# chymaera96/NeuralSampleID

Measured on AMD Instinct MI355X. Metric: audio clips/sec (contrastive step, grafp encoder), higher is better.
Workload: dtype bf16; 1 GPU; B=256 bf16 k=3 hipGraph 2-stream: grafp.yaml GraphEncoder('t') full contrastive step (fwd x2 views + NT-Xent + bwd + clip + Adam), synthetic (64,128) log-mel clip pairs per GPU, random-init weights; global_batch=256, k=3, parallelism=dp1, collectives=none (single process), gemm_arithmetic=bf16 MFMA operands, fp32 accumulate, activation_storage=bf16, views=two HIP streams (parallel graph branches), hipgraph=True

## Files before the change

include/nsid.h:

```cpp
#ifndef NSID_H
#define NSID_H
#include <stddef.h>
#include <stdint.h>

#ifdef __cplusplus
extern "C" {
#endif

#define NSID_OK 0
#define NSID_EINVAL (-1)
#define NSID_ELAUNCH (-2)

#define NSID_ACT_NONE 0
#define NSID_ACT_RELU 1
#define NSID_ACT_LEAKY 2
#define NSID_ACT_ELU 3

#define NSID_ROW_TILE 128

#define NSID_F32 0
#define NSID_BF16 1

#define NSID_GEMM_FP32 0
#define NSID_GEMM_BF16 1

int nsid_version(void);
int nsid_debug_gemm_trace(void* device_buf);
int nsid_debug_knn_trace(void* device_buf);
int nsid_set_gemm_precision(int mode);
int nsid_get_gemm_precision(void);
int nsid_set_tuning(const char* key, long value);
int nsid_get_tuning(const char* key, long* value);
int nsid_reset_tuning(void);
int nsid_tuning_count(void);
const char* nsid_tuning_key(int i);
long nsid_debug_counter(const char* key);
int nsid_debug_counters_reset(void);
int nsid_debug_counter_count(void);
const char* nsid_debug_counter_key(int i);
long nsid_gemm_g256_launches(void);
int nsid_row_tiles(int M);
long nsid_workspace_bytes(const char* op, long rows, long cols);

int nsid_linear_fwd(const void* x, int ldx, const void* w, int w_dtype, const float* bias, void* out, int ldo, int M,
                    int Nout, int K, int groups, const float* in_scale, const float* in_shift, int act_in, int act_out,
                    float* stat, int ksplit, int act_dtype , void* stream);
int nsid_linear_fwd_res(const void* x, int ldx, const void* w, int w_dtype, const float* bias, const void* addend, int ldadd,
                        void* out, int ldo, int M, int Nout, int K, int groups, const float* in_scale,
                        const float* in_shift, int act_in, int act_dtype, void* stream);
int nsid_ffn_fused_fwd(const void* x, const void* w1, const float* b1, const void* w2, const float* b2, void* out, int M, int C,
                       int H, void* stream);
int nsid_mrconv_fused_fwd(const void* y, const int32_t* idx, int B, int N, int C, int k, const void* w, const float* bias, void* out,
                          void* stream);
int nsid_linear_bwd_data(const void* dout, int ldd, const void* w, int w_dtype, const void* addend, int ldadd,
                         void* din, int ldi, int M, int Nout, int K, int groups,
                         int act_dtype , void* stream);
int nsid_linear_bwd_data_bn(const void* dout, int ldd, const void* w, int w_dtype, const void* addend, int ldadd,
                            void* din, int ldi, int M, int Nout, int K, int groups, int act_dtype, const void* bn_r,
                            const float* bn_scale, const float* bn_shift, const float* bn_mean, const float* bn_invstd,
                            int bn_act, float* bn_partial, void* stream);
int nsid_linear_bwd_data_bnapply(const void* dy, const void* r, const float* coef4, int act, void* dr, const void* w, int w_dtype,
                                 const void* addend, int ldadd, void* din, int ldi, int M, int Nout, int K, int groups,
                                 int act_dtype, const void* bn_r, const float* bn_scale, const float* bn_shift,
                                 const float* bn_mean, const float* bn_invstd, int bn_act, float* bn_partial, void* stream);
int nsid_linear_bwd_weight(const void* dout, int ldd, const void* x, int ldx, float* dw, int M, int Nout, int K,
                           int groups, const float* in_scale, const float* in_shift, int act_in,
                           int act_dtype , void* stream);
typedef struct nsid_wgrad_problem {
  const void* dout[2];
  const void* x[2];
  const float* in_scale[2];
  const float* in_shift[2];
  float* dw;
  int ldd, ldx, M, Nout, K, groups, act_in;
  int ds_out_nodes;
} nsid_wgrad_problem;
int nsid_linear_bwd_weight_grouped(const nsid_wgrad_problem* problems, int n, int act_dtype,
                                   int max_workgroups ,
                                   void* stream);
int nsid_colsum_acc(const void* x, int ldx, int M, int C, float* out, int dtype, void* stream);

int nsid_bn_finalize(const float* stat, int tiles, int C, int M, const float* gamma, const float* beta,
                     float* running_mean, float* running_var, int64_t* num_batches_tracked, float momentum,
                     float eps, float* scale, float* shift, float* mean, float* invstd, void* stream);
int nsid_bn_finalize_deferred(const float* stat, int tiles, int C, int M, const float* gamma, const float* beta, float eps,
                              float* scale, float* shift, float* mean, float* invstd, float* uvar, void* stream);
int nsid_bn_running_update(int n, const int* C, float* const* running_mean, float* const* running_var,
                           int64_t* const* num_batches_tracked, const float* const* mean_a, const float* const* uvar_a,
                           const float* const* mean_b, const float* const* uvar_b, float momentum, void* stream);
int nsid_bn_eval_affine(const float* gamma, const float* beta, const float* running_mean, const float* running_var,
                        float eps, int C, float* scale, float* shift, void* stream);
int nsid_bn_apply(const void* r, const float* scale, const float* shift, int act, const void* residual,
                  void* out, int M, int C, int dtype, void* stream);
int nsid_bn_bwd_reduce(const void* dout, const void* r, int M, int C, const float* scale, const float* shift,
                       const float* mean, const float* invstd, int act, float* partial, int dtype, void* stream);
int nsid_bn_bwd_finalize(const float* partial, int tiles, int C, int M, float* dgamma, float* dbeta, float* coef,
                         void* stream);
int nsid_bn_bwd_finalize_fused(const float* partial, int tiles, int C, int M, float* dgamma, float* dbeta, float* coef,
                               const float* scale, const float* shift, const float* mean, const float* invstd, float* coef4,
                               void* stream);
int nsid_bn_bwd_apply(const void* dout, const void* r, int M, int C, const float* scale, const float* shift,
                      const float* mean, const float* invstd, int act, const float* coef, void* dr, int dtype,
                      void* stream);

int nsid_knn_graph(const void* r, int ldr, const float* scale, const float* shift, int B, int N, int C, int k,
                   int dilation, int32_t* idx, int dtype, void* stream);

int nsid_mr_aggregate_fwd(const void* r, int ldr, const float* scale, const float* shift, const int32_t* idx, int B,
                          int N, int C, int k, void* u, uint8_t* argmax, int dtype, void* stream);
int nsid_mr_aggregate_bwd(const void* du, const int32_t* idx, const uint8_t* argmax, int B, int N, int C, int k,
                          void* dy, int dtype, void* stream);
int nsid_mr_aggregate_bwd_bn(const void* du, const int32_t* idx, const uint8_t* argmax, int B, int N, int C, int k, void* dy,
                             const void* bn_r, int bn_ldr, const float* bn_scale, const float* bn_shift, const float* bn_mean,
                             const float* bn_invstd, int bn_act, float* partial, int dtype, void* stream);

int nsid_batched_index_select_fwd(const float* x, const int32_t* idx, int B, int C, int N, int Nq, int k, float* out,
                                  void* stream);
int nsid_batched_index_select_bwd(const float* dout, const int32_t* idx, int B, int C, int N, int Nq, int k,
                                  float* dx , void* stream);

int nsid_downsample3_fwd(const void* x, int B, int N, int C, const void* wp, int w_dtype, const float* bias, void* out,
                         int Cout, float* stat, int act_dtype, void* stream);
int nsid_downsample3_bwd_weight(const void* dout, const void* x, float* dwp , int B, int N, int C, int Cout,
                                int act_dtype, void* stream);
int nsid_downsample3_bwd_data(const void* dout, const void* wp, const void* w_odd, int w_dtype, void* dx, int B, int N,
                              int C, int Cout, int act_dtype, void* stream);
int nsid_pack_ds_weight_bwd(const float* w, int Cout, int Cin, float* w_odd, void* stream);
int nsid_im2col3_fwd(const void* x, int B, int N, int C, void* col, int dtype, void* stream);
int nsid_im2col3_bwd(const void* dcol, int B, int N, int C, void* dx, int dtype, void* stream);
int nsid_pack_ds_weight(const float* w, int Cout, int Cin, float* wp, void* stream);
int nsid_dsact_fwd(const void* x, int B, int N, int C, const float* in_scale, const float* in_shift, int act_in, const float* w,
                   const float* bias, void* out, int Cout, float* stat, const float* out_scale, const float* out_shift, int act_out,
                   int act_dtype, void* stream);
int nsid_dsact_bwd_weight(const void* dout, const void* x, const float* in_scale, const float* in_shift, int act_in,
                          float* dw , int B, int N, int C, int Cout, int act_dtype, void* stream);
int nsid_dsact_bwd_data(const void* dout, const float* w, void* dx, int B, int N, int C, int Cout, const void* r_prev,
                        const float* scale, const float* shift, const float* mean, const float* invstd, int act, float* partial,
                        int act_dtype, void* stream);
int nsid_dsact_part_rows(int B, int N);
int nsid_ds_prepack(int n, const float* const* w, void* const* wp16, void* const* wb16, float* const* dwp, const int* Cout,
                    const int* Cin, void* stream);
int nsid_unpack_ds_wgrad(const float* dwp, int Cout, int Cin, float* dw , void* stream);

int nsid_peak_patchify_fwd(const float* spec, const float* w, const float* bias, int B, int H, int W, int pb, int pf,
                           int F, void* out, int ldo, float* minmax, int out_dtype, void* stream);
int nsid_peak_patchify_bwd(const float* spec, const float* minmax, const void* out, const void* dout, int ldo,
                           int B, int H, int W, int pb, int pf, int F, float* dw , float* dbias ,
                           int out_dtype, void* stream);
int nsid_peak_patchify_bwd_ws(const float* spec, const float* minmax, const void* out, const void* dout, int ldo, int B, int H,
                              int W, int pb, int pf, int F, float* dw, float* dbias, float* ws, int out_dtype, void* stream);

int nsid_node_mean_fwd(const void* x, int B, int N, int C, float* out, int x_dtype, void* stream);
int nsid_node_mean_bwd(const float* dout, int B, int N, int C, void* dx, int dx_dtype, void* stream);
int nsid_elu_bwd(const float* dout, const float* out, long n, float* din, void* stream);
int nsid_l2norm_fwd(const float* p, int B, int d, float eps, float* z, float* norm, void* stream);
int nsid_l2norm_bwd(const float* dz, const float* z, const float* norm, int B, int d, float eps, float* dp,
                    void* stream);

int nsid_reflect_pad(const float* x, long L, int pad, float* out, void* stream);
int nsid_power_mel_db(const float* spec, long ld, int n_freq, const float* fb, const int* band, int n_mels, int T,
                      float* out, void* stream);
int nsid_unfold_segments(const float* logmel, int n_mels, int T, int n_frames, int step, int S, float* out, void* stream);
int nsid_logmel_fft(const float* wave, long in_stride, int B, long L, int n_fft, int hop, const float* window,
                    const float* twiddle, const float* fb, const int* band, int n_mels, float* out, long out_clip_stride,
                    long out_mel_stride, void* stream);

int nsid_f32_to_bf16(const float* src, void* dst, long n, void* stream);

size_t nsid_ntxent_ws_floats(int Bg);
int nsid_ntxent_fwd_bwd(const float* z_i, const float* z_j, int Bg, int d, float tau, int p0, int np, float* ws,
                        float* loss_out, float* dz_i, float* dz_j, void* stream);

int nsid_sumsq_blocks(long n);
int nsid_sumsq_partial(const float* g, long n, float* partial, void* stream);
int nsid_adam_step(float* p, const float* g, float* m, float* v, long n, const float* hyper, int64_t* step,
                   const float* partial, int nblocks, float* gnorm_out, void* stream);

int nsid_fill_zero(void* p, size_t bytes, void* stream);
int nsid_scale_f32(const float* x, const float* scale, long n, float* out, void* stream);

int nsid_bcn_to_rows(const float* x, int B, int C, int N, void* rows, int ld, int rows_dtype, void* stream);
int nsid_rows_to_bcn(const void* rows, int ld, int B, int C, int N, float* x, int rows_dtype, void* stream);

int nsid_row_sqnorm(const float* x, int ldx, int n, int d, float* out, void* stream);
int nsid_flat_l2_topk(const float* q, int ldq, int nq, const float* x, int ldx, int nx, const float* x_sqnorm, const float* q_sqnorm,
                      int d, int k, float* D, int64_t* I, void* ws, size_t ws_bytes, void* stream);
int nsid_seq_scores(const float* q, int ldq, const float* x, int ldx, int nx, int d, const int64_t* I, int k, const int* starts,
                    const int* lens, int npairs, float* out, int ldo, void* stream);

int nsid_clf_node_rows(const float* x, int S, int C, int N, const float* pos, float* rows, void* stream);
int nsid_clf_pair_scores(const float* q, int nq_seg, const float* kp, int nc_seg, int N, const int* groups, const int64_t* out_off,
                         const int* tile_off, int ngroups, int ntiles, const int* cidx, const float* tail, float* out,
                         int64_t out_len, void* stream);
int nsid_clf_pair_scores_c(const float* q, int nq_seg, const float* kp, int nc_seg, int C, int N, const int* groups,
                           const int64_t* out_off, const int* tile_off, int ngroups, int ntiles, const int* cidx, const float* tail,
                           float* out, int64_t out_len, void* stream);
int nsid_clf_node_rows_n(const float* x, int S, int C, int N, const float* pos, float* rows, void* stream);
int nsid_clf_pair_scores_n(const float* q, int nq_seg, const float* kp, int nc_seg, int C, int N, const int* groups,
                           const int64_t* out_off, const int* tile_off, int ngroups, int ntiles, const int* cidx, const float* tail,
                           float* out, int64_t out_len, void* stream);

int nsid_clf_mine_hard_negatives(const float* zq, int nq, const float* za, int na, int d, int k, int64_t* out, void* stream);
int nsid_clf_attn_fwd(const float* q, int nq_seg, const float* kv, int nc_seg, int N, const int* qi, const int* ci, int P, float* obar,
                      float* attn, float* abar, void* stream);
int nsid_clf_head_fwd(const float* hid, const float* keep, const float* w2, const float* b2, int P, float* s, void* stream);
int nsid_clf_head_bwd(const float* ds, const float* s, const float* hid, const float* keep, const float* w2, int P, float* dh, float* dz,
                      float* dw2, float* db2, void* stream);
int nsid_clf_attn_bwd(const float* dobar, const float* attn, const float* q, int nq_seg, const float* kv, int nc_seg, int N,
                      const int* qi, const int* ci, int P, float* dq, float* dk, void* stream);
int nsid_clf_seg_reduce(const float* dq, const float* dk, const float* abar, const float* dobar, const int* qi, const int* ci, int P,
                        int N, int nq_seg, int nc_seg, float* dq_seg, float* dkv_seg, void* stream);
int nsid_clf_attn_fwd_c(const float* q, int nq_seg, const float* kv, int nc_seg, int C, int N, const int* qi, const int* ci, int P,
                        float* obar, float* attn, float* abar, void* stream);
int nsid_clf_attn_bwd_c(const float* dobar, const float* attn, const float* q, int nq_seg, const float* kv, int nc_seg, int C, int N,
                        const int* qi, const int* ci, int P, float* dq, float* dk, void* stream);
int nsid_clf_seg_reduce_c(const float* dq, const float* dk, const float* abar, const float* dobar, const int* qi, const int* ci, int P,
                          int C, int N, int nq_seg, int nc_seg, float* dq_seg, float* dkv_seg, void* stream);

int nsid_conv2d_fwd(const void* x, int B, int H, int W, int C, const void* w, int w_dtype, const float* bias, const void* addend,
                    void* out, int Cout, int ksize, int stride, int act_out, int act_dtype, void* stream);
int nsid_ibn_relu_fwd(const void* x, int B, int HW, int C, const float* in_gamma, const float* in_beta, float eps,
                      const float* bn_scale, const float* bn_shift, void* out, int dtype, void* stream);
int nsid_stem7_pool_fwd(const float* x, int B, int H, int W, const float* w, const float* bias, void* out, int out_dtype,
                        void* stream);
int nsid_gem_pool_fwd(const void* x, int B, int HW, int C, const float* p, float eps, float* out, int x_dtype, void* stream);

#ifdef __cplusplus
}
#endif
#endif
```

neuralsampleid_amd/_lib.py:

```python
import ctypes
import os

import torch

_PKG = os.path.dirname(os.path.abspath(__file__))
LIB_PATH = os.environ.get("NSID_LIB") or os.path.join(_PKG, "libnsid_hip.so")

SIGNATURES = {
    "nsid_set_gemm_precision": "i",
    "nsid_linear_fwd": "pipippiiiiippiipiis",
    "nsid_linear_fwd_res": "pipippipiiiiippiis",
    "nsid_linear_bwd_data": "pipipipiiiiiis",
    "nsid_linear_bwd_data_bn": "pipipipiiiiiipppppips",
    "nsid_linear_bwd_weight": "pipipiiiippiis",
    "nsid_linear_bwd_weight_grouped": "piiis",
    "nsid_colsum_acc": "piiipis",
    "nsid_bn_finalize": "piiipppppffpppps",
    "nsid_bn_finalize_deferred": "piiippfppppps",
    "nsid_bn_running_update": "ippppppppfs",
    "nsid_bn_eval_affine": "ppppfipps",
    "nsid_bn_apply": "pppippiiis",
    "nsid_bn_bwd_reduce": "ppiippppipis",
    "nsid_bn_bwd_finalize": "piiippps",
    "nsid_bn_bwd_apply": "ppiippppippis",
    "nsid_bn_bwd_finalize_fused": "piiipppppppps",
    "nsid_knn_graph": "pippiiiiipis",
    "nsid_mr_aggregate_fwd": "pipppiiiippis",
    "nsid_mr_aggregate_bwd": "pppiiiipis",
    "nsid_im2col3_fwd": "piiipis",
    "nsid_im2col3_bwd": "piiipis",
    "nsid_pack_ds_weight": "piips",
    "nsid_dsact_fwd": "piiippipppipppiis",
    "nsid_dsact_bwd_weight": "ppppipiiiiis",
    "nsid_dsact_bwd_data": "pppiiiipppppipis",
    "nsid_pack_ds_weight_bwd": "piips",
    "nsid_downsample3_fwd": "piiipippipis",
    "nsid_downsample3_bwd_weight": "pppiiiiis",
    "nsid_downsample3_bwd_data": "pppipiiiiis",
    "nsid_unpack_ds_wgrad": "piips",
    "nsid_ds_prepack": "ipppppps",
    "nsid_peak_patchify_fwd": "pppiiiiiipipis",
    "nsid_peak_patchify_bwd": "ppppiiiiiiippis",
    "nsid_peak_patchify_bwd_ws": "ppppiiiiiiipppis",
    "nsid_node_mean_fwd": "piiipis",
    "nsid_node_mean_bwd": "piiipis",
    "nsid_elu_bwd": "pplps",
    "nsid_l2norm_fwd": "piifpps",
    "nsid_l2norm_bwd": "pppiifps",
    "nsid_ntxent_fwd_bwd": "ppiifiipppps",
    "nsid_sumsq_partial": "plps",
    "nsid_adam_step": "pppplpppips",
    "nsid_f32_to_bf16": "ppls",
    "nsid_reflect_pad": "plips",
    "nsid_power_mel_db": "plippiips",
    "nsid_unfold_segments": "piiiiips",
    "nsid_logmel_fft": "pliliippppiplls",
    "nsid_bcn_to_rows": "piiipiis",
    "nsid_rows_to_bcn": "piiiipis",
    "nsid_batched_index_select_fwd": "ppiiiiips",
    "nsid_batched_index_select_bwd": "ppiiiiips",
    "nsid_fill_zero": "pzs",
    "nsid_scale_f32": "pplps",
    "nsid_row_sqnorm": "piiips",
    "nsid_flat_l2_topk": "piipiippiipppzs",
    "nsid_seq_scores": "pipiiipippipis",
    "nsid_clf_node_rows": "piiipps",
    "nsid_clf_pair_scores": "pipiipppiipppls",
    "nsid_clf_pair_scores_c": "pipiiipppiipppls",
    "nsid_clf_node_rows_n": "piiipps",
    "nsid_clf_pair_scores_n": "pipiiipppiipppls",
    "nsid_clf_mine_hard_negatives": "pipiiips",
    "nsid_clf_attn_fwd": "pipiippippps",
    "nsid_clf_head_fwd": "ppppips",
    "nsid_clf_head_bwd": "pppppipppps",
    "nsid_clf_attn_bwd": "pppipiippipps",
    "nsid_clf_seg_reduce": "ppppppiiiipps",
    "nsid_clf_attn_fwd_c": "pipiiippippps",
    "nsid_clf_attn_bwd_c": "pppipiiippipps",
    "nsid_clf_seg_reduce_c": "ppppppiiiiipps",
    "nsid_conv2d_fwd": "piiiipipppiiiiis",
    "nsid_ibn_relu_fwd": "piiippfpppis",
    "nsid_stem7_pool_fwd": "piiipppis",
    "nsid_gem_pool_fwd": "piiipfpis",
}

class WgradProblem(ctypes.Structure):
    _fields_ = [("dout", ctypes.c_void_p * 2), ("x", ctypes.c_void_p * 2), ("in_scale", ctypes.c_void_p * 2),
                ("in_shift", ctypes.c_void_p * 2), ("dw", ctypes.c_void_p), ("ldd", ctypes.c_int), ("ldx", ctypes.c_int),
                ("M", ctypes.c_int), ("Nout", ctypes.c_int), ("K", ctypes.c_int), ("groups", ctypes.c_int), ("act_in", ctypes.c_int),
                ("ds_out_nodes", ctypes.c_int)]


_CT = {"p": ctypes.c_void_p, "i": ctypes.c_int, "l": ctypes.c_long, "f": ctypes.c_float, "s": ctypes.c_void_p,
       "z": ctypes.c_size_t}


def _load():
    if not os.path.exists(LIB_PATH):
        raise ImportError(
            f"{LIB_PATH} is missing: build it with `python -m neuralsampleid_amd.build` "
            "(hipcc --offload-arch=gfx950). There is no CPU fallback for the product path.")
    lib = ctypes.CDLL(LIB_PATH)
    for name, sig in SIGNATURES.items():
        fn = getattr(lib, name)
        fn.argtypes = [_CT[c] for c in sig]
        fn.restype = ctypes.c_int
    lib.nsid_version.restype = ctypes.c_int
    if lib.nsid_version() < 0:
        raise ImportError(f"{LIB_PATH} reports a negative version: not a product build of this tree; rebuild with "
                          "`python -m neuralsampleid_amd.build --force`")
    lib.nsid_debug_gemm_trace.argtypes = [ctypes.c_void_p]
    lib.nsid_debug_gemm_trace.restype = ctypes.c_int
    lib.nsid_debug_knn_trace.argtypes = [ctypes.c_void_p]
    lib.nsid_debug_knn_trace.restype = ctypes.c_int
    lib.nsid_get_gemm_precision.restype = ctypes.c_int
    lib.nsid_gemm_g256_launches.argtypes = []
    lib.nsid_gemm_g256_launches.restype = ctypes.c_long
    lib.nsid_set_tuning.argtypes = [ctypes.c_char_p, ctypes.c_long]
    lib.nsid_set_tuning.restype = ctypes.c_int
    lib.nsid_get_tuning.argtypes = [ctypes.c_char_p, ctypes.POINTER(ctypes.c_long)]
    lib.nsid_get_tuning.restype = ctypes.c_int
    lib.nsid_reset_tuning.argtypes = []
    lib.nsid_reset_tuning.restype = ctypes.c_int
    lib.nsid_workspace_bytes.argtypes = [ctypes.c_char_p, ctypes.c_long, ctypes.c_long]
    lib.nsid_workspace_bytes.restype = ctypes.c_long
    lib.nsid_tuning_count.argtypes = []
    lib.nsid_tuning_count.restype = ctypes.c_int
    lib.nsid_tuning_key.argtypes = [ctypes.c_int]
    lib.nsid_tuning_key.restype = ctypes.c_char_p
    lib.nsid_debug_counter.argtypes = [ctypes.c_char_p]
    lib.nsid_debug_counter.restype = ctypes.c_long
    lib.nsid_debug_counters_reset.argtypes = []
    lib.nsid_debug_counters_reset.restype = ctypes.c_int
    lib.nsid_debug_counter_count.argtypes = []
    lib.nsid_debug_counter_count.restype = ctypes.c_int
    lib.nsid_debug_counter_key.argtypes = [ctypes.c_int]
    lib.nsid_debug_counter_key.restype = ctypes.c_char_p
    lib.nsid_linear_bwd_data_bnapply.argtypes = [_CT[c] for c in "pppippipipiiiiiipppppips"]
    lib.nsid_linear_bwd_data_bnapply.restype = ctypes.c_int
    lib.nsid_mr_aggregate_bwd_bn.argtypes = [_CT[c] for c in "pppiiiippippppipis"]
    lib.nsid_mr_aggregate_bwd_bn.restype = ctypes.c_int
    lib.nsid_ffn_fused_fwd.argtypes = [_CT[c] for c in "ppppppiiis"]
    lib.nsid_ffn_fused_fwd.restype = ctypes.c_int
    lib.nsid_mrconv_fused_fwd.argtypes = [_CT[c] for c in "ppiiiippps"]
    lib.nsid_mrconv_fused_fwd.restype = ctypes.c_int
    lib.nsid_row_tiles.argtypes = [ctypes.c_int]
    lib.nsid_row_tiles.restype = ctypes.c_int
    lib.nsid_dsact_part_rows.argtypes = [ctypes.c_int, ctypes.c_int]
    lib.nsid_dsact_part_rows.restype = ctypes.c_int
    lib.nsid_sumsq_blocks.argtypes = [ctypes.c_long]
    lib.nsid_sumsq_blocks.restype = ctypes.c_int
    lib.nsid_ntxent_ws_floats.argtypes = [ctypes.c_int]
    lib.nsid_ntxent_ws_floats.restype = ctypes.c_size_t
    return lib


lib = _load()
EXPORTS = list(SIGNATURES) + ["nsid_version", "nsid_debug_gemm_trace", "nsid_debug_knn_trace", "nsid_get_gemm_precision", "nsid_gemm_g256_launches", "nsid_linear_bwd_data_bnapply", "nsid_mr_aggregate_bwd_bn", "nsid_ffn_fused_fwd", "nsid_mrconv_fused_fwd", "nsid_debug_counter", "nsid_debug_counters_reset", "nsid_debug_counter_count", "nsid_debug_counter_key", "nsid_set_tuning", "nsid_get_tuning", "nsid_reset_tuning", "nsid_tuning_count", "nsid_tuning_key", "nsid_row_tiles", "nsid_dsact_part_rows", "nsid_sumsq_blocks", "nsid_ntxent_ws_floats", "nsid_workspace_bytes"]

_ERR = {-1: "NSID_EINVAL (unsupported shape, misaligned pointer or bad argument)",
        -2: "NSID_ELAUNCH (HIP runtime refused the launch)"}


def call(name, *args):
    rc = getattr(lib, name)(*args)
    if rc != 0:
        raise RuntimeError(f"{name} failed: {_ERR.get(rc, rc)}")


def set_tuning(key: str, value: int) -> None:
    if lib.nsid_set_tuning(key.encode(), int(value)) != 0:
        raise KeyError(f"unknown tuning key {key!r}; known: {', '.join(tuning_keys())}")


def get_tuning(key: str) -> int:
    v = ctypes.c_long()
    if lib.nsid_get_tuning(key.encode(), ctypes.byref(v)) != 0:
        raise KeyError(f"unknown tuning key {key!r}")
    return int(v.value)


def reset_tuning() -> None:
    lib.nsid_reset_tuning()


def launch_counters(reset: bool = False) -> dict:
    out = {}
    for i in range(lib.nsid_debug_counter_count()):
        k = lib.nsid_debug_counter_key(i)
        out[k.decode()] = int(lib.nsid_debug_counter(k))
    if reset:
        lib.nsid_debug_counters_reset()
    return out


def tuning_keys():
    return [lib.nsid_tuning_key(i).decode() for i in range(lib.nsid_tuning_count())]
```

neuralsampleid_amd/csrc/bn.hip:

```cpp
#include <cstdlib>
#include "nsid_common.h"

namespace {

constexpr int FIN_THREADS = 1024;

template <int FIN_CH>
__device__ __forceinline__ void tile_sums(const float* __restrict__ p0, const float* __restrict__ p1, int tiles,
                                          int C, int c, int tg, bool ok, double* red0, double* red1, double& sum,
                                          double& sq) {
  constexpr int FIN_TG = FIN_THREADS / FIN_CH;
  double a = 0.0, b = 0.0;
  if (ok) {
    constexpr int UB = 8;
    int t = tg;
    for (; t + (UB - 1) * FIN_TG < tiles; t += UB * FIN_TG) {
      float va[UB], vb[UB];
#pragma unroll
      for (int u = 0; u < UB; ++u) {
        va[u] = p0[(long)(t + u * FIN_TG) * C + c];
        vb[u] = p1[(long)(t + u * FIN_TG) * C + c];
      }
#pragma unroll
      for (int u = 0; u < UB; ++u) { a += (double)va[u]; b += (double)vb[u]; }
// ... 172 lines not shown
  if (coef != nullptr) {
    coef[c] = c0;
    coef[C + c] = c1;
  }
  if (coef4 != nullptr) {
    const float sc = scale[c], is = invstd[c];
    coef4[c] = sc;
    coef4[C + c] = shift[c];
    coef4[2 * C + c] = -sc * c1 * is;
    coef4[3 * C + c] = sc * (c1 * is * mean[c] - c0);
  }
}

template <typename T, int U>
__global__ __launch_bounds__(256) void bn_bwd_apply_kernel(const T* __restrict__ dout, const T* __restrict__ r,
                                                           long rows, int CV, const float* __restrict__ scale,
                                                           const float* __restrict__ shift,
                                                           const float* __restrict__ mean,
                                                           const float* __restrict__ invstd, float slope,
                                                           const float* __restrict__ coef, T* __restrict__ dr) {
  constexpr int N = Chunk<T>::N;
  const int C = CV * N;
  const long t = (long)blockIdx.x * blockDim.x + threadIdx.x, total = (long)gridDim.x * blockDim.x;
  const int cq = (int)(t % CV), c = cq * N;
  const long rstep = total / CV;
  float sc[N], sh[N], mu[N], is[N], c0[N], c1[N];
  load_channels<N>(scale, c, sc);
  load_channels<N>(shift, c, sh);
  load_channels<N>(mean, c, mu);
  load_channels<N>(invstd, c, is);
  load_channels<N>(coef, c, c0);
  load_channels<N>(coef + C, c, c1);
  for (long row = t / CV; row < rows; row += U * rstep) {
    float d[U][N], x[U][N];
#pragma unroll
    for (int u = 0; u < U; ++u) {
      const long rr = row + u * rstep;
      if (rr < rows) {
        Chunk<T>::load(dout + (rr * CV + cq) * N, d[u]);
        Chunk<T>::load(r + (rr * CV + cq) * N, x[u]);
      }
    }
#pragma unroll
    for (int u = 0; u < U; ++u) {
      const long rr = row + u * rstep;
      if (rr < rows) {
        float o[N];
#pragma unroll
        for (int e = 0; e < N; ++e) {
          const float g = (sc[e] * x[u][e] + sh[e]) > 0.f ? d[u][e] : d[u][e] * slope;
          const float xh = (x[u][e] - mu[e]) * is[e];
          o[e] = sc[e] * (g - c0[e] - xh * c1[e]);
        }
        Chunk<T>::store(dr + (rr * CV + cq) * N, o);
      }
    }
  }
}

inline float bn_slope(int act) { return act == NSID_ACT_RELU ? 0.f : (act == NSID_ACT_LEAKY ? 0.2f : 1.f); }

inline int stream_grid(long nchunks) {
  long b = (nchunks + 255) / 256;
  const long cap = nsid_tune(NSID_T_stream_max_wg);
  return (int)(b > cap ? cap : (b < 1 ? 1 : b));
}

template <typename T>
__global__ __launch_bounds__(256) void colsum_atomic_kernel(const T* __restrict__ x, long ld, int M, int C,
                                                            float* __restrict__ out) {
  constexpr int N = Chunk<T>::N;
  constexpr int CQ = CR_CH / N, RG = 256 / CQ, ROWS = NSID_ROW_TILE / RG;
  __shared__ float red[RG][CR_CH];
  const int row0 = blockIdx.x * NSID_ROW_TILE;
  const int t = threadIdx.x, q = t % CQ, rgp = t / CQ;
  const int c = blockIdx.y * CR_CH + N * q;
  float s[N];
#pragma unroll
  for (int e = 0; e < N; ++e) s[e] = 0.f;
  if (c < C)
    for (int i = 0; i < ROWS; ++i) {
      const int row = row0 + rgp + RG * i;
      if (row < M) {
        float d[N];
        Chunk<T>::load(x + (long)row * ld + c, d);
#pragma unroll
        for (int e = 0; e < N; ++e) s[e] += d[e];
      }
    }
#pragma unroll
  for (int e = 0; e < N; ++e) red[rgp][N * q + e] = s[e];
  __syncthreads();
  if (t < CR_CH && blockIdx.y * CR_CH + t < C) {
    float a = 0.f;
    for (int g = 0; g < RG; ++g) a += red[g][t];
    atomicAdd(out + blockIdx.y * CR_CH + t, a);
  }
}

inline long chunk_keeping_grid(long nchunks, int CV, int U, long max_wg, bool* capped) {
  int g0 = CV, d256 = 256;
  while (d256 % 2 == 0 && g0 % 2 == 0) { d256 /= 2; g0 /= 2; }
  long want = (nchunks + 256L * U - 1) / (256L * U);
  if (capped) *capped = want > max_wg;
  if (want > max_wg) want = max_wg;
  if (want < 1) want = 1;
  return (want + g0 - 1) / g0 * g0;
}

inline int bn_fin_ch(int tiles) {
  const int t = (int)nsid_tune(NSID_T_bn_fin_tiles);
  return (t > 0 && tiles >= t) ? 16 : 64;
}
#define NSID_FIN_LAUNCH(kernel, tiles, C, stream, ...)                                                                      \
  do {                                                                                                                       \
    if (bn_fin_ch(tiles) == 16)                                                                                              \
      NSID_LAUNCH(kernel<16>, dim3(((C) + 15) / 16), dim3(FIN_THREADS), 0, static_cast<hipStream_t>(stream), __VA_ARGS__);   \
    else                                                                                                                     \
      NSID_LAUNCH(kernel<64>, dim3(((C) + 63) / 64), dim3(FIN_THREADS), 0, static_cast<hipStream_t>(stream), __VA_ARGS__);   \
  } while (0)

}

extern "C" int nsid_bn_finalize(const float* stat, int tiles, int C, int M, const float* gamma, const float* beta,
                                float* running_mean, float* running_var, int64_t* nbt, float momentum, float eps,
                                float* scale, float* shift, float* mean, float* invstd, void* stream) {
  NSID_REQUIRE(stat && gamma && beta && scale && shift && mean && invstd && C > 0 && M > 0);
  NSID_REQUIRE(tiles == nsid_row_tiles(M));
  NSID_REQUIRE((running_mean == nullptr) == (running_var == nullptr));
  NSID_FIN_LAUNCH(bn_finalize_kernel, tiles, C, stream, stat, tiles, C, M, gamma, beta, running_mean, running_var, nbt,
              momentum, eps, scale, shift, mean, invstd, static_cast<float*>(nullptr));
  return nsid_launch_status();
}

extern "C" int nsid_bn_finalize_deferred(const float* stat, int tiles, int C, int M, const float* gamma,
                                         const float* beta, float eps, float* scale, float* shift, float* mean,
                                         float* invstd, float* uvar, void* stream) {
  NSID_REQUIRE(stat && gamma && beta && scale && shift && mean && invstd && uvar && C > 0 && M > 0);
  NSID_REQUIRE(tiles == nsid_row_tiles(M));
  NSID_FIN_LAUNCH(bn_finalize_kernel, tiles, C, stream, stat, tiles, C, M, gamma, beta, static_cast<float*>(nullptr),
              static_cast<float*>(nullptr), static_cast<int64_t*>(nullptr), 0.f, eps, scale, shift, mean, invstd, uvar);
  return nsid_launch_status();
}

namespace {
constexpr int RU_LAYERS = 16;
struct RunUpdArgs {
  float* rm[RU_LAYERS]; float* rv[RU_LAYERS]; int64_t* nbt[RU_LAYERS];
  const float* mean_a[RU_LAYERS]; const float* uvar_a[RU_LAYERS];
  const float* mean_b[RU_LAYERS]; const float* uvar_b[RU_LAYERS];
  int C[RU_LAYERS];
  float momentum;
};
__global__ __launch_bounds__(256) void bn_running_update_kernel(const RunUpdArgs a) {
  const int l = blockIdx.x;
  const float m = a.momentum;
  const bool two = a.mean_b[l] != nullptr;
  if (threadIdx.x == 0 && a.nbt[l] != nullptr) *a.nbt[l] += two ? 2 : 1;
  for (int c = threadIdx.x; c < a.C[l]; c += blockDim.x) {
    float rm = running_blend(a.rm[l][c], a.mean_a[l][c], m);
    float rv = running_blend(a.rv[l][c], a.uvar_a[l][c], m);
    if (two) {
      rm = running_blend(rm, a.mean_b[l][c], m);
      rv = running_blend(rv, a.uvar_b[l][c], m);
    }
    a.rm[l][c] = rm;
    a.rv[l][c] = rv;
  }
}
}

extern "C" int nsid_bn_running_update(int n, const int* C, float* const* running_mean, float* const* running_var,
                                      int64_t* const* num_batches_tracked, const float* const* mean_a,
                                      const float* const* uvar_a, const float* const* mean_b,
                                      const float* const* uvar_b, float momentum, void* stream) {
  NSID_REQUIRE(n > 0 && C && running_mean && running_var && mean_a && uvar_a);
  for (int base = 0; base < n; base += RU_LAYERS) {
    RunUpdArgs a{};
    const int cnt = n - base < RU_LAYERS ? n - base : RU_LAYERS;
    for (int i = 0; i < cnt; ++i) {
      NSID_REQUIRE(C[base + i] > 0 && running_mean[base + i] && running_var[base + i] && mean_a[base + i] && uvar_a[base + i]);
      a.rm[i] = running_mean[base + i]; a.rv[i] = running_var[base + i];
      a.nbt[i] = num_batches_tracked ? num_batches_tracked[base + i] : nullptr;
      a.mean_a[i] = mean_a[base + i]; a.uvar_a[i] = uvar_a[base + i];
      a.mean_b[i] = mean_b ? mean_b[base + i] : nullptr; a.uvar_b[i] = uvar_b ? uvar_b[base + i] : nullptr;
      NSID_REQUIRE((a.mean_b[i] == nullptr) == (a.uvar_b[i] == nullptr));
      a.C[i] = C[base + i];
    }
    a.momentum = momentum;
    NSID_LAUNCH(bn_running_update_kernel, dim3(cnt), dim3(256), 0, static_cast<hipStream_t>(stream), a);
    const int rc = nsid_launch_status();
    if (rc != NSID_OK) return rc;
  }
  return NSID_OK;
}

extern "C" int nsid_bn_eval_affine(const float* gamma, const float* beta, const float* running_mean,
                                   const float* running_var, float eps, int C, float* scale, float* shift,
                                   void* stream) {
  NSID_REQUIRE(gamma && beta && running_mean && running_var && scale && shift && C > 0);
  NSID_LAUNCH(bn_eval_affine_kernel, dim3((C + 127) / 128), dim3(128), 0, static_cast<hipStream_t>(stream), gamma, beta,
              running_mean, running_var, eps, C, scale, shift);
  return nsid_launch_status();
}

extern "C" int nsid_bn_apply(const void* r, const float* scale, const float* shift, int act, const void* residual,
                             void* out, int M, int C, int dtype, void* stream) {
  NSID_REQUIRE(r && scale && shift && out && M > 0 && C > 0 && NSID_DTYPE_OK(dtype));
  NSID_REQUIRE(C % (dtype == NSID_BF16 ? 8 : 4) == 0 && nsid_aligned16(r) && nsid_aligned16(out));
  NSID_DISPATCH_DTYPE(dtype, T, {
    const long nchunks = (long)M * C / Chunk<T>::N;
    NSID_LAUNCH((bn_apply_kernel<T>), dim3(stream_grid(nchunks)), dim3(256), 0, static_cast<hipStream_t>(stream),
                static_cast<const T*>(r), scale, shift, act, static_cast<const T*>(residual), static_cast<T*>(out),
                nchunks, C / Chunk<T>::N);
  });
  return nsid_launch_status();
}

extern "C" int nsid_bn_bwd_reduce(const void* dout, const void* r, int M, int C, const float* scale,
                                  const float* shift, const float* mean, const float* invstd, int act, float* partial,
                                  int dtype, void* stream) {
  NSID_REQUIRE(dout && r && scale && shift && mean && invstd && partial && M > 0 && C > 0 && NSID_DTYPE_OK(dtype));
  NSID_REQUIRE(C % (dtype == NSID_BF16 ? 8 : 4) == 0);
  NSID_REQUIRE(act == NSID_ACT_NONE || act == NSID_ACT_RELU || act == NSID_ACT_LEAKY);
  const int tiles = nsid_row_tiles(M);
  NSID_DISPATCH_DTYPE(dtype, T, {
    NSID_LAUNCH((col_reduce_kernel<1, T>), dim3(tiles, (C + CR_CH - 1) / CR_CH), dim3(256), 0,
                static_cast<hipStream_t>(stream), static_cast<const T*>(dout), static_cast<const T*>(r), (long)C, M, C,
                scale, shift, mean, invstd, bn_slope(act), partial, tiles);
  });
  return nsid_launch_status();
}

extern "C" int nsid_bn_bwd_finalize(const float* partial, int tiles, int C, int M, float* dgamma, float* dbeta,
                                    float* coef, void* stream) {
  NSID_REQUIRE(partial && coef && C > 0 && M > 0 && tiles >= 1);
  NSID_FIN_LAUNCH(bn_bwd_finalize_kernel, tiles, C, stream, partial, tiles, C, M, dgamma, dbeta, coef, static_cast<const float*>(nullptr),
              static_cast<const float*>(nullptr), static_cast<const float*>(nullptr), static_cast<const float*>(nullptr),
              static_cast<float*>(nullptr));
  return nsid_launch_status();
}

extern "C" int nsid_bn_bwd_finalize_fused(const float* partial, int tiles, int C, int M, float* dgamma, float* dbeta,
                                          float* coef, const float* scale, const float* shift, const float* mean,
                                          const float* invstd, float* coef4, void* stream) {
  NSID_REQUIRE(partial && coef && coef4 && scale && shift && mean && invstd && C > 0 && M > 0 && tiles >= 1);
  NSID_FIN_LAUNCH(bn_bwd_finalize_kernel, tiles, C, stream, partial, tiles, C, M, dgamma, dbeta, coef, scale, shift, mean, invstd, coef4);
  return nsid_launch_status();
}

extern "C" int nsid_bn_bwd_apply(const void* dout, const void* r, int M, int C, const float* scale,
                                 const float* shift, const float* mean, const float* invstd, int act,
                                 const float* coef, void* dr, int dtype, void* stream) {
  NSID_REQUIRE(dout && r && scale && shift && mean && invstd && coef && dr && M > 0 && C > 0 && NSID_DTYPE_OK(dtype));
  NSID_REQUIRE(C % (dtype == NSID_BF16 ? 8 : 4) == 0);
  NSID_REQUIRE(act == NSID_ACT_NONE || act == NSID_ACT_RELU || act == NSID_ACT_LEAKY);
  NSID_DISPATCH_DTYPE(dtype, T, {
    constexpr int U = 4;
    const int CV = C / Chunk<T>::N;
    const long nchunks = (long)M * CV;
    int g0 = CV, d256 = 256;
    while (d256 % 2 == 0 && g0 % 2 == 0) { d256 /= 2; g0 /= 2; }
    long want = (nchunks + 256L * U - 1) / (256L * U);
    const long max_wg = nsid_tune(NSID_T_bn_bwd_apply_max_wg);
    nsid_count(NSID_C_bn_bwd_apply);
    if (want > max_wg) { want = max_wg; nsid_count(NSID_C_bn_bwd_apply_capped); }
    const long grid = (want + g0 - 1) / g0 * g0;
    NSID_LAUNCH((bn_bwd_apply_kernel<T, U>), dim3((int)grid), dim3(256), 0, static_cast<hipStream_t>(stream),
                static_cast<const T*>(dout), static_cast<const T*>(r), (long)M, CV, scale, shift, mean,
                invstd, bn_slope(act), coef, static_cast<T*>(dr));
  });
  return nsid_launch_status();
}

extern "C" int nsid_colsum_acc(const void* x, int ldx, int M, int C, float* out, int dtype, void* stream) {
  NSID_REQUIRE(x && out && M > 0 && C > 0 && NSID_DTYPE_OK(dtype) && nsid_aligned16(x));
  NSID_REQUIRE(C % (dtype == NSID_BF16 ? 8 : 4) == 0 && ldx % (dtype == NSID_BF16 ? 8 : 4) == 0);
  NSID_DISPATCH_DTYPE(dtype, T, {
    NSID_LAUNCH((colsum_atomic_kernel<T>), dim3(nsid_row_tiles(M), (C + CR_CH - 1) / CR_CH), dim3(256), 0,
                static_cast<hipStream_t>(stream), static_cast<const T*>(x), (long)ldx, M, C, out);
  });
  return nsid_launch_status();
}
```

neuralsampleid_amd/csrc/misc.hip:

```cpp
#include <algorithm>
#include "nsid_common.h"

namespace {

inline int grid_for(long n, int cap = 2048) {
  long b = (n + 255) / 256;
  return (int)(b > cap ? cap : (b < 1 ? 1 : b));
}

template <typename T>
__global__ __launch_bounds__(256) void im2col3_fwd_kernel(const T* __restrict__ x, int B, int N, int No, int C,
                                                          T* __restrict__ col) {
  constexpr int NV = Chunk<T>::N;
  const int CV = C / NV;
  const long total = (long)B * No * 3 * CV;
  for (long q = (long)blockIdx.x * blockDim.x + threadIdx.x; q < total; q += (long)gridDim.x * blockDim.x) {
    const int cv = (int)(q % CV);
    const int t = (int)((q / CV) % 3);
    const long orow = q / (3L * CV);
    const int b = (int)(orow / No), no = (int)(orow % No);
    const int n = 2 * no - 1 + t;
    float v[NV];
#pragma unroll
    for (int e = 0; e < NV; ++e) v[e] = 0.f;
    if (n >= 0 && n < N) Chunk<T>::load(x + ((long)b * N + n) * C + NV * cv, v);
    Chunk<T>::store(col + orow * (3L * C) + (long)t * C + NV * cv, v);
  }
}

template <typename T>
__global__ __launch_bounds__(256) void im2col3_bwd_kernel(const T* __restrict__ dcol, int B, int N, int No, int C,
                                                          T* __restrict__ dx) {
  constexpr int NV = Chunk<T>::N;
  const int CV = C / NV;
  const long total = (long)B * N * CV;
  for (long q = (long)blockIdx.x * blockDim.x + threadIdx.x; q < total; q += (long)gridDim.x * blockDim.x) {
    const int cv = (int)(q % CV);
    const long row = q / CV;
    const int b = (int)(row / N), n = (int)(row % N);
    float s[NV];
#pragma unroll
    for (int e = 0; e < NV; ++e) s[e] = 0.f;
#pragma unroll
    for (int t = 0; t < 3; ++t) {
      const int m = n + 1 - t;
      if (m >= 0 && (m & 1) == 0 && (m >> 1) < No) {
        float v[NV];
        Chunk<T>::load(dcol + ((long)b * No + (m >> 1)) * (3L * C) + (long)t * C + NV * cv, v);
#pragma unroll
        for (int e = 0; e < NV; ++e) s[e] += v[e];
      }
    }
    Chunk<T>::store(dx + row * C + NV * cv, s);
  }
}

__global__ void pack_ds_weight_kernel(const float* __restrict__ w, int Cout, int Cin, float* __restrict__ wp) {
  const long total = (long)Cout * 3 * Cin;
  for (long q = (long)blockIdx.x * blockDim.x + threadIdx.x; q < total; q += (long)gridDim.x * blockDim.x) {
    const int c = (int)(q % Cin), t = (int)((q / Cin) % 3);
    const long o = q / (3L * Cin);
    wp[q] = w[((o * Cin + c) * 3 + t) * 3 + 1];
  }
}
__global__ void pack_ds_weight_bwd_kernel(const float* __restrict__ w, int Cout, int Cin, float* __restrict__ wb) {
  const long total = 2L * Cout * Cin;
  for (long q = (long)blockIdx.x * blockDim.x + threadIdx.x; q < total; q += (long)gridDim.x * blockDim.x) {
    const int c = (int)(q % Cin);
    const long r = q / Cin;
    const long o = r % Cout;
    const int t = r < Cout ? 2 : 0;
    wb[q] = w[((o * Cin + c) * 3 + t) * 3 + 1];
  }
}
__global__ void unpack_ds_wgrad_kernel(const float* __restrict__ dwp, int Cout, int Cin, float* __restrict__ dw) {
  const long total = (long)Cout * 3 * Cin;
  for (long q = (long)blockIdx.x * blockDim.x + threadIdx.x; q < total; q += (long)gridDim.x * blockDim.x) {
    const int c = (int)(q % Cin), t = (int)((q / Cin) % 3);
    const long o = q / (3L * Cin);
    atomicAdd(dw + ((o * Cin + c) * 3 + t) * 3 + 1, dwp[q]);
  }
}

constexpr int DSP_LAYERS = 8;
#define NSID_DS_SLOTS 2
struct DsPrepArgs {
  const float* w[DSP_LAYERS]; __bf16* wp16[DSP_LAYERS]; __bf16* wb16[DSP_LAYERS]; float* dwp[DSP_LAYERS];
  int Cout[DSP_LAYERS], Cin[DSP_LAYERS];
};
__global__ __launch_bounds__(256) void ds_prepack_kernel(const DsPrepArgs a) {
  const int l = blockIdx.y;
  const float* w = a.w[l];
  const int Cout = a.Cout[l], Cin = a.Cin[l];
  const long total = (long)Cout * 3 * Cin;
  for (long q = (long)blockIdx.x * blockDim.x + threadIdx.x; q < total; q += (long)gridDim.x * blockDim.x) {
    const int c = (int)(q % Cin), t = (int)((q / Cin) % 3);
    const long o = q / (3L * Cin);
    a.wp16[l][q] = (__bf16)w[((o * Cin + c) * 3 + t) * 3 + 1];
    if (a.dwp[l] != nullptr) {
#pragma unroll
      for (int v = 0; v < NSID_DS_SLOTS; ++v) a.dwp[l][v * total + q] = 0.f;
    }
    if (q < 2L * Cout * Cin) {
      const long r = q / Cin, ob = r % Cout;
      const int tb = r < Cout ? 2 : 0;
      a.wb16[l][q] = (__bf16)w[((ob * Cin + c) * 3 + tb) * 3 + 1];
    }
  }
}

__device__ __forceinline__ float add_unfused(float acc, float a, float b) {
#pragma clang fp contract(off)
  const float p = a * b;
  return acc + p;
}
__device__ __forceinline__ float linspace01(int i, int steps) {
  const float step = 1.0f / (float)(steps - 1);
  return (i < steps / 2) ? __fmul_rn((float)i, step) : fmaf(-(float)(steps - 1 - i), step, 1.0f);
}

constexpr int PATCH_PAD = 8;
template <typename T, int MAXPATCH, int PB = 0, int PF = 0>
__global__ __launch_bounds__(256) void patchify_fwd_kernel(const float* __restrict__ spec, const float* __restrict__ w,
                                                           const float* __restrict__ bias, int H, int W, int pb_,
                                                           int pf_, int F, T* __restrict__ out, int ldo,
                                                           float* __restrict__ minmax) {
  constexpr bool FIX = PB > 0;
  const int pb = FIX ? PB : pb_, pf = FIX ? PF : pf_;
  extern __shared__ __attribute__((aligned(16))) float sm[];
  const int b = blockIdx.x, t = threadIdx.x;
  const float* x = spec + (long)b * H * W;
  const int wn = F * 3 * pb * pf, LDW = W + PATCH_PAD;
  float* wl = sm;
  float* red = sm + wn;
  float* xs = red + 8;
  for (int i = t; i < wn; i += blockDim.x) wl[i] = w[i];
  float lo = __builtin_inff(), hi = -__builtin_inff();
  constexpr int XB = 8;
  for (int i0 = t; i0 < H * W / 4; i0 += XB * blockDim.x) {
    f32x4 v[XB];
#pragma unroll
    for (int u = 0; u < XB; ++u) {
      const int i = i0 + u * blockDim.x;
      if (i < H * W / 4) v[u] = *reinterpret_cast<const f32x4*>(x + 4 * i);
    }
#pragma unroll
    for (int u = 0; u < XB; ++u) {
      const int i = i0 + u * blockDim.x;
      if (i < H * W / 4) {
        const int hh = (4 * i) / W, ww = (4 * i) % W;
        *reinterpret_cast<f32x4*>(xs + hh * LDW + ww) = v[u];
        lo = fminf(fminf(lo, v[u][0]), fminf(v[u][1], fminf(v[u][2], v[u][3])));
        hi = fmaxf(fmaxf(hi, v[u][0]), fmaxf(v[u][1], fmaxf(v[u][2], v[u][3])));
      }
    }
  }
  lo = wave_min(lo); hi = wave_max(hi);
  if ((t & 63) == 0) { red[t >> 6] = lo; red[4 + (t >> 6)] = hi; }
  __syncthreads();
  lo = fminf(fminf(red[0], red[1]), fminf(red[2], red[3]));
  hi = fmaxf(fmaxf(red[4], red[5]), fmaxf(red[6], red[7]));
  if (t == 0 && minmax != nullptr) { minmax[2 * b] = lo; minmax[2 * b + 1] = hi; }
  const float range = hi - lo;
  const int Hp = H / pb, Wp = W / pf, NP = Hp * Wp;
  for (int p = t; p < NP; p += blockDim.x) {
    const int ph = p / Wp, pw = p % Wp;
    T* dst = out + ((long)b * NP + p) * ldo;
    constexpr int NLW = FIX ? PF : MAXPATCH, NLH = FIX ? PB : MAXPATCH;
    float sv[MAXPATCH], lw[NLW], lh[NLH];
#pragma unroll
    for (int q = 0; q < MAXPATCH; ++q) {
      if (q < pb * pf) {
        const int i = q / pf, j = q % pf;
        sv[q] = (xs[(ph * pb + i) * LDW + pw * pf + j] - lo) / range;
        if constexpr (!FIX) {
          lw[q] = linspace01(pw * pf + j, W);
          lh[q] = linspace01(ph * pb + i, H);
        }
      }
    }
    if constexpr (FIX) {
#pragma unroll
      for (int j = 0; j < PF; ++j) lw[j] = linspace01(pw * PF + j, W);
#pragma unroll
      for (int i = 0; i < PB; ++i) lh[i] = linspace01(ph * PB + i, H);
    }
    constexpr int NV = Chunk<T>::N;
    for (int f0 = 0; f0 < F; f0 += NV) {
      float res[NV];
#pragma unroll
      for (int ff = 0; ff < NV; ++ff) {
        const int f = f0 + ff;
        res[ff] = 0.f;
        if (f < F) {
          float acc = bias[f];
          const float* wf = (MAXPATCH == 32 ? w : wl) + f * 3 * pb * pf;
#pragma unroll
          for (int q = 0; q < MAXPATCH; ++q) {
            if (q < pb * pf) {
              acc = fmaf(wf[q], lw[FIX ? q % (FIX ? PF : 1) : q], acc);
              acc = add_unfused(acc, wf[pb * pf + q], lh[FIX ? q / (FIX ? PF : 1) : q]);
              acc = add_unfused(acc, wf[2 * pb * pf + q], sv[q]);
            }
          }
          res[ff] = acc < 0.f ? 0.f : acc;
        }
      }
      if (f0 + NV <= F && ldo % NV == 0 && (reinterpret_cast<size_t>(out) & 15) == 0) {
        Chunk<T>::store(dst + f0, res);
      } else {
#pragma unroll
        for (int ff = 0; ff < NV; ++ff)
          if (f0 + ff < F) dst[f0 + ff] = (T)res[ff];
      }
    }
  }
}

template <typename T>
__global__ __launch_bounds__(256) void patchify_bwd_kernel(const float* __restrict__ spec,
                                                           const float* __restrict__ minmax,
                                                           const T* __restrict__ out,
                                                           const T* __restrict__ dout, int ldo, int B, int H,
                                                           int W, int pb, int pf, int F, float* __restrict__ dw,
                                                           float* __restrict__ dbias, int bands) {
  extern __shared__ __attribute__((aligned(16))) float sm[];
  const int t = threadIdx.x;
  const int Hall = H;
  H /= bands;
  const int Hp = H / pb, Wp = W / pf, NP = Hp * Wp;
  const int per_f = 3 * pb * pf, LDW = W + PATCH_PAD;
  float* xs = sm + NP * F;
  float* red = xs + H * LDW;
  constexpr int MAXQ = 4;
  float wacc[MAXQ] = {0.f, 0.f, 0.f, 0.f}, bacc = 0.f;
  constexpr int NV = Chunk<T>::N;
  const bool vec = (F % NV == 0) && (ldo % NV == 0);
  for (int vb = blockIdx.x; vb < B * bands; vb += gridDim.x) {
    const int b = vb / bands, band = vb - b * bands;
    const float* x = spec + ((long)b * bands + band) * H * W;
    const float lo = minmax[2 * b], range = minmax[2 * b + 1] - lo;
    __syncthreads();
    if (vec) {
      const int FC = F / NV;
      for (int q = t; q < NP * FC; q += blockDim.x) {
        const int p = q / FC, f = (q % FC) * NV;
        const long o = ((long)vb * NP + p) * ldo + f;
        float ov[NV], dv[NV];
        Chunk<T>::load(out + o, ov);
        Chunk<T>::load(dout + o, dv);
#pragma unroll
        for (int e = 0; e < NV; ++e) sm[p * F + f + e] = ov[e] > 0.f ? dv[e] : 0.f;
      }
    } else {
      for (int q = t; q < NP * F; q += blockDim.x) {
        const int p = q / F, f = q % F;
        const long o = ((long)vb * NP + p) * ldo + f;
        sm[q] = (float)out[o] > 0.f ? (float)dout[o] : 0.f;
      }
    }
    constexpr int XB = 8;
    for (int i0 = t; i0 < H * W / 4; i0 += XB * blockDim.x) {
// ... 88 lines not shown
      Chunk<T>::load(dout + o, dv); Chunk<T>::load(dout + o + 4, dv + 4);
    }
    f32x4 v[8];
#pragma unroll
    for (int u = 0; u < 8; ++u) v[u] = *reinterpret_cast<const f32x4*>(x + 4 * (t + 256 * u));
#pragma unroll
    for (int e = 0; e < 8; ++e) g[t * F + e] = ov[e] > 0.f ? dv[e] : 0.f;
#pragma unroll
    for (int u = 0; u < 8; ++u) {
      const int i4 = 4 * (t + 256 * u), hh = i4 / W, ww = i4 % W;
      *reinterpret_cast<f32x4*>(xs + hh * LDW + ww) =
          f32x4{(v[u][0] - lo) / range, (v[u][1] - lo) / range, (v[u][2] - lo) / range, (v[u][3] - lo) / range};
    }
  }
  __syncthreads();
  {
    const int f = t % F, k2 = t / F;
    float a = 0.f;
    if (k2 < Wp) { for (int ph = 0; ph < Hp; ++ph) a += g[(ph * Wp + k2) * F + f]; }
    else { for (int pw = 0; pw < Wp; ++pw) a += g[((k2 - Wp) * Wp + pw) * F + f]; }
    red[t] = a;
  }
  __syncthreads();
  const int f = t >> 5, ij = t & 31, i = ij >> 3, j = ij & 7;
  float a_t = 0.f, a_f = 0.f;
#pragma unroll
  for (int q = 0; q < 16; ++q) {
    a_t += red[q * F + f] * linspace01(q * PFk + j, W);
    a_f += red[(Wp + q) * F + f] * linspace01(q * PBk + i, H);
  }
  float part[4] = {0.f, 0.f, 0.f, 0.f};
  for (int ph = 0; ph < Hp; ++ph) {
    const float* srow = g + (ph * Wp) * F + f;
    const float* xrow = xs + (ph * PBk + i) * LDW + j;
#pragma unroll
    for (int pw = 0; pw < Wp; ++pw) part[pw & 3] += srow[pw * F] * xrow[pw * PFk];
  }
  float* wsb = ws + (long)b * PB2_OUT;
  wsb[f * 96 + ij] = a_t;
  wsb[f * 96 + 32 + ij] = a_f;
  wsb[f * 96 + 64 + ij] = (part[0] + part[1]) + (part[2] + part[3]);
  if (t < F) {
    float a = 0.f;
    for (int pw = 0; pw < Wp; ++pw) a += red[pw * F + t];
    wsb[768 + t] = a;
  }
}

__global__ __launch_bounds__(256) void patchify_bwd2_reduce_kernel(const float* __restrict__ ws, int B, float* __restrict__ dw,
                                                                   float* __restrict__ dbias) {
  __shared__ float part[256];
  const int t = threadIdx.x, q = blockIdx.x * 64 + (t & 63), sl = t >> 6;
  float a = 0.f;
  if (q < PB2_OUT)
    for (int b = sl; b < B; b += 4) a += ws[(long)b * PB2_OUT + q];
  part[t] = a;
  __syncthreads();
  if (sl == 0 && q < PB2_OUT) {
    a = (part[t] + part[t + 64]) + (part[t + 128] + part[t + 192]);
    atomicAdd(q < 768 ? dw + q : dbias + (q - 768), a);
  }
}

template <typename T>
__global__ __launch_bounds__(256) void node_mean_fwd_kernel(const T* __restrict__ x, int N, int C,
                                                            float* __restrict__ out) {
  constexpr int NV = Chunk<T>::N;
  const int b = blockIdx.x, CV = C / NV;
  for (int cv = blockIdx.y * blockDim.x + threadIdx.x; cv < CV; cv += gridDim.y * blockDim.x) {
    float s[NV];
#pragma unroll
    for (int e = 0; e < NV; ++e) s[e] = 0.f;
    for (int n = 0; n < N; ++n) {
      float v[NV];
      Chunk<T>::load(x + ((long)b * N + n) * C + NV * cv, v);
#pragma unroll
      for (int e = 0; e < NV; ++e) s[e] += v[e];
    }
#pragma unroll
    for (int e = 0; e < NV; ++e) out[(long)b * C + NV * cv + e] = s[e] / (float)N;
  }
}
template <typename T>
__global__ __launch_bounds__(256) void node_mean_bwd_kernel(const float* __restrict__ dout, int N, int C,
                                                            long nchunks, T* __restrict__ dx) {
  constexpr int NV = Chunk<T>::N;
  const int CV = C / NV;
  for (long q = (long)blockIdx.x * blockDim.x + threadIdx.x; q < nchunks; q += (long)gridDim.x * blockDim.x) {
    const int cv = (int)(q % CV);
    const long b = q / ((long)CV * N);
    float v[NV];
#pragma unroll
    for (int e = 0; e < NV; ++e) v[e] = dout[b * C + NV * cv + e] / (float)N;
    Chunk<T>::store(dx + q * NV, v);
  }
}

__global__ void elu_bwd_kernel(const float* __restrict__ dout, const float* __restrict__ out, long n,
                               float* __restrict__ din) {
  for (long i = (long)blockIdx.x * blockDim.x + threadIdx.x; i < n; i += (long)gridDim.x * blockDim.x) {
    const float o = out[i];
    din[i] = dout[i] * (o > 0.f ? 1.f : o + 1.f);
  }
}

__global__ __launch_bounds__(256) void l2norm_fwd_kernel(const float* __restrict__ p, int B, int d, float eps,
                                                         float* __restrict__ z, float* __restrict__ norm) {
  const int row = blockIdx.x * 4 + (threadIdx.x >> 6), lane = threadIdx.x & 63;
  if (row >= B) return;
  float ss = 0.f;
  for (int c = lane; c < d; c += 64) { const float v = p[(long)row * d + c]; ss += v * v; }
  ss = wave_sum(ss);
  const float nr = sqrtf(ss), den = fmaxf(nr, eps);
  for (int c = lane; c < d; c += 64) z[(long)row * d + c] = p[(long)row * d + c] / den;
  if (lane == 0) norm[row] = nr;
}
__global__ __launch_bounds__(256) void l2norm_bwd_kernel(const float* __restrict__ dz, const float* __restrict__ z,
                                                         const float* __restrict__ norm, int B, int d, float eps,
                                                         float* __restrict__ dp) {
  const int row = blockIdx.x * 4 + (threadIdx.x >> 6), lane = threadIdx.x & 63;
  if (row >= B) return;
  float dot = 0.f;
  for (int c = lane; c < d; c += 64) dot += z[(long)row * d + c] * dz[(long)row * d + c];
  dot = wave_sum(dot);
  const float nr = norm[row];
  for (int c = lane; c < d; c += 64) {
    const long o = (long)row * d + c;
    dp[o] = nr > eps ? (dz[o] - z[o] * dot) / nr : dz[o] / eps;
  }
}

constexpr int SUMSQ_PER_BLOCK = 256 * 4 * 16;
__global__ __launch_bounds__(256) void sumsq_kernel(const float* __restrict__ g, long n, float* __restrict__ partial) {
  __shared__ double red[4];
  const long base = (long)blockIdx.x * SUMSQ_PER_BLOCK;
  double s = 0.0;
  for (int it = 0; it < 16; ++it) {
    const long i = base + ((long)it * 256 + threadIdx.x) * 4;
    if (i + 3 < n) {
      const f32x4 v = *reinterpret_cast<const f32x4*>(g + i);
      s += (double)v[0] * v[0] + (double)v[1] * v[1] + (double)v[2] * v[2] + (double)v[3] * v[3];
    } else {
      for (long j = i; j < n && j < i + 4; ++j) s += (double)g[j] * g[j];
    }
  }
  s = wave_sum_d(s);
  if ((threadIdx.x & 63) == 0) red[threadIdx.x >> 6] = s;
  __syncthreads();
  if (threadIdx.x == 0) partial[blockIdx.x] = (float)(red[0] + red[1] + red[2] + red[3]);
}

__global__ __launch_bounds__(256) void adam_kernel(float* __restrict__ p, const float* __restrict__ g,
                                                   float* __restrict__ m, float* __restrict__ v, long n,
                                                   const float* __restrict__ hyper, const int64_t* __restrict__ step,
                                                   const float* __restrict__ partial, int nblocks,
                                                   float* __restrict__ gnorm_out) {
  __shared__ float coef_s;
  __shared__ int skip_s;
  __shared__ double red[4];
  {
    double s = 0.0;
    for (int i = threadIdx.x; i < nblocks; i += blockDim.x) s += (double)partial[i];
    s = wave_sum_d(s);
    if ((threadIdx.x & 63) == 0) red[threadIdx.x >> 6] = s;
    __syncthreads();
    if (threadIdx.x == 0) {
      const float norm = (float)sqrt(red[0] + red[1] + red[2] + red[3]);
      const float max_norm = hyper[4];
      float c = 1.f;
      if (max_norm > 0.f) { c = max_norm / (norm + 1e-6f); c = c < 1.f ? c : 1.f; }
      coef_s = c;
      skip_s = !isfinite(norm);
      if (blockIdx.x == 0 && gnorm_out != nullptr) gnorm_out[0] = norm;
    }
    __syncthreads();
  }
  if (skip_s) return;
  const float coef = coef_s;
  const float lr = hyper[0], b1 = hyper[1], b2 = hyper[2], eps = hyper[3];
  const double t = (double)(*step + 1);
  const float bc1 = (float)(1.0 - pow((double)b1, t));
  const float bc2_sqrt = (float)sqrt(1.0 - pow((double)b2, t));
  const float step_size = lr / bc1;
  const long n4 = (reinterpret_cast<uintptr_t>(p) | reinterpret_cast<uintptr_t>(g) | reinterpret_cast<uintptr_t>(m) |
                   reinterpret_cast<uintptr_t>(v)) % 16 == 0 ? n / 4 : 0;
  auto upd = [&](float gi_, float& mi_, float& vi_, float& pi_) {
    const float gi = gi_ * coef;
    const float mi = mi_ * b1 + (1.f - b1) * gi;
    const float vi = vi_ * b2 + (1.f - b2) * gi * gi;
    mi_ = mi;
    vi_ = vi;
    const float denom = sqrtf(vi) / bc2_sqrt + eps;
    pi_ -= step_size * (mi / denom);
  };
  for (long i = (long)blockIdx.x * blockDim.x + threadIdx.x; i < n4; i += (long)gridDim.x * blockDim.x) {
    const f32x4 g4 = reinterpret_cast<const f32x4*>(g)[i];
    f32x4 m4 = reinterpret_cast<f32x4*>(m)[i], v4 = reinterpret_cast<f32x4*>(v)[i], p4 = reinterpret_cast<f32x4*>(p)[i];
#pragma unroll
    for (int e = 0; e < 4; ++e) {
      float me = m4[e], ve = v4[e], pe = p4[e];
      upd(g4[e], me, ve, pe);
      m4[e] = me; v4[e] = ve; p4[e] = pe;
    }
    reinterpret_cast<f32x4*>(m)[i] = m4;
    reinterpret_cast<f32x4*>(v)[i] = v4;
    reinterpret_cast<f32x4*>(p)[i] = p4;
  }
  for (long i = 4 * n4 + (long)blockIdx.x * blockDim.x + threadIdx.x; i < n; i += (long)gridDim.x * blockDim.x)
    upd(g[i], m[i], v[i], p[i]);
}
__global__ void adam_tick_kernel(int64_t* step, const float* gnorm) {
  if (gnorm == nullptr || isfinite(gnorm[0])) *step += 1;
}

template <typename TS, typename TD>
__global__ __launch_bounds__(256) void transpose_kernel(const TS* __restrict__ src, long src_batch, long src_ld,
                                                        TD* __restrict__ dst, long dst_batch, long dst_ld,
                                                        int R, int S) {
  __shared__ float tile[32][33];
  const int b = blockIdx.z;
  const int r0 = blockIdx.y * 32, s0 = blockIdx.x * 32;
  const int tx = threadIdx.x & 31, ty = threadIdx.x >> 5;
  for (int i = ty; i < 32; i += 8) {
    const int rr = r0 + i, ss = s0 + tx;
    if (rr < R && ss < S) tile[i][tx] = (float)src[b * src_batch + (long)rr * src_ld + ss];
  }
  __syncthreads();
  for (int i = ty; i < 32; i += 8) {
    const int ss = s0 + i, rr = r0 + tx;
    if (rr < R && ss < S) dst[b * dst_batch + (long)ss * dst_ld + rr] = (TD)tile[tx][i];
  }
}

}

extern "C" int nsid_im2col3_fwd(const void* x, int B, int N, int C, void* col, int dtype, void* stream) {
  NSID_REQUIRE(x && col && B > 0 && N > 0 && C > 0 && NSID_DTYPE_OK(dtype) && nsid_aligned16(x) && nsid_aligned16(col));
  const int nv = dtype == NSID_BF16 ? 8 : 4;
  NSID_REQUIRE(C % nv == 0);
  const int No = (N - 1) / 2 + 1;
  NSID_DISPATCH_DTYPE(dtype, T, {
    NSID_LAUNCH((im2col3_fwd_kernel<T>), dim3(grid_for((long)B * No * 3 * (C / nv))), dim3(256), 0,
                static_cast<hipStream_t>(stream), static_cast<const T*>(x), B, N, No, C, static_cast<T*>(col));
  });
  return nsid_launch_status();
}
extern "C" int nsid_im2col3_bwd(const void* dcol, int B, int N, int C, void* dx, int dtype, void* stream) {
  NSID_REQUIRE(dcol && dx && B > 0 && N > 0 && C > 0 && NSID_DTYPE_OK(dtype) && nsid_aligned16(dcol) && nsid_aligned16(dx));
  const int nv = dtype == NSID_BF16 ? 8 : 4;
  NSID_REQUIRE(C % nv == 0);
  const int No = (N - 1) / 2 + 1;
  NSID_DISPATCH_DTYPE(dtype, T, {
    NSID_LAUNCH((im2col3_bwd_kernel<T>), dim3(grid_for((long)B * N * (C / nv))), dim3(256), 0,
                static_cast<hipStream_t>(stream), static_cast<const T*>(dcol), B, N, No, C, static_cast<T*>(dx));
  });
  return nsid_launch_status();
}
extern "C" int nsid_pack_ds_weight(const float* w, int Cout, int Cin, float* wp, void* stream) {
  NSID_REQUIRE(w && wp && Cout > 0 && Cin > 0);
  NSID_LAUNCH(pack_ds_weight_kernel, dim3(grid_for((long)Cout * 3 * Cin)), dim3(256), 0,
                     static_cast<hipStream_t>(stream), w, Cout, Cin, wp);
  return nsid_launch_status();
}
extern "C" int nsid_pack_ds_weight_bwd(const float* w, int Cout, int Cin, float* wb, void* stream) {
  NSID_REQUIRE(w && wb && Cout > 0 && Cin > 0);
  NSID_LAUNCH(pack_ds_weight_bwd_kernel, dim3(grid_for(2L * Cout * Cin)), dim3(256), 0, static_cast<hipStream_t>(stream),
              w, Cout, Cin, wb);
  return nsid_launch_status();
}
extern "C" int nsid_unpack_ds_wgrad(const float* dwp, int Cout, int Cin, float* dw, void* stream) {
  NSID_REQUIRE(dwp && dw && Cout > 0 && Cin > 0);
  NSID_LAUNCH(unpack_ds_wgrad_kernel, dim3(grid_for((long)Cout * 3 * Cin)), dim3(256), 0,
                     static_cast<hipStream_t>(stream), dwp, Cout, Cin, dw);
  return nsid_launch_status();
}

extern "C" int nsid_ds_prepack(int n, const float* const* w, void* const* wp16, void* const* wb16, float* const* dwp, const int* Cout,
                               const int* Cin, void* stream) {
  NSID_REQUIRE(n > 0 && n <= DSP_LAYERS && w && wp16 && wb16 && Cout && Cin);
  DsPrepArgs a{};
  long most = 0;
  for (int i = 0; i < n; ++i) {
    NSID_REQUIRE(w[i] && wp16[i] && wb16[i] && Cout[i] > 0 && Cin[i] > 0);
    a.w[i] = w[i]; a.wp16[i] = static_cast<__bf16*>(wp16[i]); a.wb16[i] = static_cast<__bf16*>(wb16[i]);
    a.dwp[i] = dwp ? dwp[i] : nullptr; a.Cout[i] = Cout[i]; a.Cin[i] = Cin[i];
    most = std::max(most, (long)Cout[i] * 3 * Cin[i]);
  }
  NSID_LAUNCH(ds_prepack_kernel, dim3(grid_for(most, 256), n), dim3(256), 0, static_cast<hipStream_t>(stream), a);
  return nsid_launch_status();
}
extern "C" int nsid_peak_patchify_fwd(const float* spec, const float* w, const float* bias, int B, int H, int W, int pb,
                                      int pf, int F, void* out, int ldo, float* minmax, int out_dtype, void* stream) {
  NSID_REQUIRE(spec && w && bias && out && B > 0 && H > 1 && W > 1 && pb > 0 && pf > 0 && F > 0);
  NSID_REQUIRE(H % pb == 0 && W % pf == 0 && ldo >= F && NSID_DTYPE_OK(out_dtype));
  const size_t bytes = ((size_t)F * 3 * pb * pf + 8 + (size_t)H * (W + 8)) * sizeof(float);
  NSID_REQUIRE(bytes <= 160 * 1024 && W % 4 == 0 && (F * 3 * pb * pf) % 4 == 0 && nsid_aligned16(spec) && pb * pf <= 64);
  bool attr_ok = true;
  auto big_lds = [&](const void* fn) {
    if (bytes > 64 * 1024 && hipFuncSetAttribute(fn, hipFuncAttributeMaxDynamicSharedMemorySize, 160 * 1024) != hipSuccess) attr_ok = false;
  };
  NSID_DISPATCH_DTYPE(out_dtype, T, {
    if (pb == 4 && pf == 8) {
      big_lds(reinterpret_cast<const void*>(patchify_fwd_kernel<T, 32, 4, 8>));
      if (attr_ok)
        NSID_LAUNCH((patchify_fwd_kernel<T, 32, 4, 8>), dim3(B), dim3(256), bytes, static_cast<hipStream_t>(stream), spec, w,
                    bias, H, W, pb, pf, F, static_cast<T*>(out), ldo, minmax);
    } else if (pb * pf == 32) {
      big_lds(reinterpret_cast<const void*>(patchify_fwd_kernel<T, 32>));
      if (attr_ok)
        NSID_LAUNCH((patchify_fwd_kernel<T, 32>), dim3(B), dim3(256), bytes, static_cast<hipStream_t>(stream), spec, w,
                    bias, H, W, pb, pf, F, static_cast<T*>(out), ldo, minmax);
    } else {
      big_lds(reinterpret_cast<const void*>(patchify_fwd_kernel<T, 64>));
      if (attr_ok)
        NSID_LAUNCH((patchify_fwd_kernel<T, 64>), dim3(B), dim3(256), bytes, static_cast<hipStream_t>(stream), spec, w,
                    bias, H, W, pb, pf, F, static_cast<T*>(out), ldo, minmax);
    }
  });
  if (!attr_ok) return NSID_ELAUNCH;
  return nsid_launch_status();
}
extern "C" int nsid_peak_patchify_bwd(const float* spec, const float* minmax, const void* out, const void* dout,
                                      int ldo, int B, int H, int W, int pb, int pf, int F, float* dw, float* dbias,
                                      int out_dtype, void* stream) {
  NSID_REQUIRE(spec && minmax && out && dout && dw && dbias && B > 0 && H % pb == 0 && W % pf == 0 && ldo >= F);
  NSID_REQUIRE(NSID_DTYPE_OK(out_dtype));
  int bands = 1;
  auto lds_bytes = [&](int nb) {
    const int Hb = H / nb;
    return ((size_t)(Hb / pb) * (W / pf) * F + (size_t)Hb * (W + 8) + (size_t)(Hb / pb + W / pf) * F) * sizeof(float);
  };
  while (lds_bytes(bands) > 64 * 1024 && (H / pb) % (2 * bands) == 0) bands *= 2;
  const size_t bytes = lds_bytes(bands);
  NSID_REQUIRE(bytes <= 64 * 1024 && (long)F * 3 * pb * pf <= 4 * 256 && F <= 256 && W % 4 == 0 && nsid_aligned16(spec));
  NSID_REQUIRE(((H / bands / pb) * (W / pf) * F) % 4 == 0 && (long)B * bands < (1L << 30));
  NSID_DISPATCH_DTYPE(out_dtype, T, {
    NSID_LAUNCH((patchify_bwd_kernel<T>), dim3(B * bands < 256 ? B * bands : 256), dim3(256), bytes, static_cast<hipStream_t>(stream),
                spec, minmax, static_cast<const T*>(out), static_cast<const T*>(dout), ldo, B, H, W, pb, pf, F, dw, dbias, bands);
  });
  return nsid_launch_status();
}

extern "C" int nsid_peak_patchify_bwd_ws(const float* spec, const float* minmax, const void* out, const void* dout, int ldo, int B,
                                         int H, int W, int pb, int pf, int F, float* dw, float* dbias, float* ws, int out_dtype,
                                         void* stream) {
  NSID_REQUIRE(spec && minmax && out && dout && dw && dbias && ws && B > 0 && ldo >= F && NSID_DTYPE_OK(out_dtype));
  NSID_REQUIRE(H == 64 && W == 128 && pb == 4 && pf == 8 && F == 8 && ldo % (out_dtype == NSID_BF16 ? 8 : 4) == 0);
  NSID_REQUIRE(nsid_aligned16(spec) && nsid_aligned16(out) && nsid_aligned16(dout));
  hipStream_t s = static_cast<hipStream_t>(stream);
  NSID_DISPATCH_DTYPE(out_dtype, T, {
    NSID_LAUNCH((patchify_bwd2_kernel<T>), dim3(B), dim3(256), 0, s, spec, minmax, static_cast<const T*>(out),
                static_cast<const T*>(dout), ldo, ws);
  });
  NSID_LAUNCH(patchify_bwd2_reduce_kernel, dim3((PB2_OUT + 63) / 64), dim3(256), 0, s, ws, B, dw, dbias);
  return nsid_launch_status();
}

extern "C" int nsid_node_mean_fwd(const void* x, int B, int N, int C, float* out, int x_dtype, void* stream) {
  NSID_REQUIRE(x && out && B > 0 && N > 0 && C > 0 && NSID_DTYPE_OK(x_dtype) && nsid_aligned16(x));
  const int nv = x_dtype == NSID_BF16 ? 8 : 4;
  NSID_REQUIRE(C % nv == 0);
  NSID_DISPATCH_DTYPE(x_dtype, T, {
    NSID_LAUNCH((node_mean_fwd_kernel<T>), dim3(B, (C / nv + 255) / 256), dim3(256), 0,
                static_cast<hipStream_t>(stream), static_cast<const T*>(x), N, C, out);
  });
  return nsid_launch_status();
}
extern "C" int nsid_node_mean_bwd(const float* dout, int B, int N, int C, void* dx, int dx_dtype, void* stream) {
  NSID_REQUIRE(dout && dx && B > 0 && N > 0 && C > 0 && NSID_DTYPE_OK(dx_dtype) && nsid_aligned16(dx));
  const int nv = dx_dtype == NSID_BF16 ? 8 : 4;
  NSID_REQUIRE(C % nv == 0);
  const long nchunks = (long)B * N * (C / nv);
  NSID_DISPATCH_DTYPE(dx_dtype, T, {
    NSID_LAUNCH((node_mean_bwd_kernel<T>), dim3(grid_for(nchunks)), dim3(256), 0, static_cast<hipStream_t>(stream),
                dout, N, C, nchunks, static_cast<T*>(dx));
  });
  return nsid_launch_status();
}
extern "C" int nsid_elu_bwd(const float* dout, const float* out, long n, float* din, void* stream) {
  NSID_REQUIRE(dout && out && din && n > 0);
  NSID_LAUNCH(elu_bwd_kernel, dim3(grid_for(n)), dim3(256), 0, static_cast<hipStream_t>(stream), dout, out, n,
                     din);
  return nsid_launch_status();
}
extern "C" int nsid_l2norm_fwd(const float* p, int B, int d, float eps, float* z, float* norm, void* stream) {
  NSID_REQUIRE(p && z && norm && B > 0 && d > 0);
  NSID_LAUNCH(l2norm_fwd_kernel, dim3((B + 3) / 4), dim3(256), 0, static_cast<hipStream_t>(stream), p, B, d, eps,
                     z, norm);
  return nsid_launch_status();
}
extern "C" int nsid_l2norm_bwd(const float* dz, const float* z, const float* norm, int B, int d, float eps, float* dp,
                               void* stream) {
  NSID_REQUIRE(dz && z && norm && dp && B > 0 && d > 0);
  NSID_LAUNCH(l2norm_bwd_kernel, dim3((B + 3) / 4), dim3(256), 0, static_cast<hipStream_t>(stream), dz, z, norm,
                     B, d, eps, dp);
  return nsid_launch_status();
}

extern "C" int nsid_sumsq_blocks(long n) { return (int)((n + SUMSQ_PER_BLOCK - 1) / SUMSQ_PER_BLOCK); }
extern "C" int nsid_sumsq_partial(const float* g, long n, float* partial, void* stream) {
  NSID_REQUIRE(g && partial && n > 0 && nsid_aligned16(g));
  NSID_LAUNCH(sumsq_kernel, dim3(nsid_sumsq_blocks(n)), dim3(256), 0, static_cast<hipStream_t>(stream), g, n,
                     partial);
  return nsid_launch_status();
}
extern "C" int nsid_adam_step(float* p, const float* g, float* m, float* v, long n, const float* hyper, int64_t* step,
                              const float* partial, int nblocks, float* gnorm_out, void* stream) {
  NSID_REQUIRE(p && g && m && v && hyper && step && partial && n > 0 && nblocks > 0);
  hipStream_t s = static_cast<hipStream_t>(stream);
  NSID_LAUNCH(adam_kernel, dim3(grid_for(n, 4096)), dim3(256), 0, s, p, g, m, v, n, hyper, step, partial,
                     nblocks, gnorm_out);
  NSID_LAUNCH(adam_tick_kernel, dim3(1), dim3(1), 0, s, step, (const float*)gnorm_out);
  return nsid_launch_status();
}

__global__ void reflect_pad_kernel(const float* __restrict__ x, long L, int pad, float* __restrict__ out) {
  const long n = L + 2L * pad;
  for (long i = (long)blockIdx.x * blockDim.x + threadIdx.x; i < n; i += (long)gridDim.x * blockDim.x) {
    long j = i - pad;
    if (j < 0) j = -j;
    if (j >= L) j = 2 * (L - 1) - j;
    out[i] = x[j];
  }
}

__global__ __launch_bounds__(256) void power_mel_db_kernel(const float* __restrict__ spec, long ld, int n_freq,
                                                           const float* __restrict__ fb, const int* __restrict__ band,
                                                           int n_mels, int T, float* __restrict__ out) {
  extern __shared__ float pw[];
  const int t = blockIdx.x;
  const float* row = spec + (long)t * ld;
  for (int f = threadIdx.x; f < n_freq; f += blockDim.x) {
    const float re = row[f], im = row[n_freq + f];
    pw[f] = re * re + im * im;
  }
  __syncthreads();
  for (int m = threadIdx.x; m < n_mels; m += blockDim.x) {
    float acc = 0.f;
    for (int f = band[2 * m]; f < band[2 * m + 1]; ++f) acc += fb[(long)m * n_freq + f] * pw[f];
    out[(long)m * T + t] = 10.0f * log10f(fmaxf(acc, 1e-10f));
  }
}

__global__ void unfold_segments_kernel(const float* __restrict__ lm, int n_mels, int T, int n_frames, int step, int S,
                                       float* __restrict__ out) {
  const long n = (long)S * n_mels * n_frames;
  for (long i = (long)blockIdx.x * blockDim.x + threadIdx.x; i < n; i += (long)gridDim.x * blockDim.x) {
    const int f = (int)(i % n_frames), m = (int)((i / n_frames) % n_mels);
    const long s = i / ((long)n_frames * n_mels);
    out[i] = lm[(long)m * T + s * step + f];
  }
}

extern "C" int nsid_reflect_pad(const float* x, long L, int pad, float* out, void* stream) {
  NSID_REQUIRE(x && out && L > 1 && pad >= 0 && pad < L);
  NSID_LAUNCH(reflect_pad_kernel, dim3(grid_for(L + 2L * pad)), dim3(256), 0, static_cast<hipStream_t>(stream), x, L, pad,
              out);
  return nsid_launch_status();
}
extern "C" int nsid_power_mel_db(const float* spec, long ld, int n_freq, const float* fb, const int* band, int n_mels,
                                 int T, float* out, void* stream) {
  NSID_REQUIRE(spec && fb && band && out && n_freq > 0 && n_mels > 0 && T > 0 && ld >= 2L * n_freq);
  NSID_REQUIRE((size_t)n_freq * sizeof(float) <= 48 * 1024);
  NSID_LAUNCH(power_mel_db_kernel, dim3(T), dim3(256), (size_t)n_freq * sizeof(float), static_cast<hipStream_t>(stream),
              spec, ld, n_freq, fb, band, n_mels, T, out);
  return nsid_launch_status();
}
extern "C" int nsid_unfold_segments(const float* logmel, int n_mels, int T, int n_frames, int step, int S, float* out,
                                    void* stream) {
  NSID_REQUIRE(logmel && out && n_mels > 0 && n_frames > 0 && step > 0 && S > 0 && (long)(S - 1) * step + n_frames <= T);
  NSID_LAUNCH(unfold_segments_kernel, dim3(grid_for((long)S * n_mels * n_frames)), dim3(256), 0,
              static_cast<hipStream_t>(stream), logmel, n_mels, T, n_frames, step, S, out);
  return nsid_launch_status();
}

__global__ __launch_bounds__(256) void f32_to_bf16_kernel(const float* __restrict__ src, __bf16* __restrict__ dst, long n8) {
  for (long i = (long)blockIdx.x * blockDim.x + threadIdx.x; i < n8; i += (long)gridDim.x * blockDim.x) {
    float v[8];
    Chunk<float>::load(src + 8 * i, v);
    Chunk<float>::load(src + 8 * i + 4, v + 4);
    Chunk<__bf16>::store(dst + 8 * i, v);
  }
}
extern "C" int nsid_f32_to_bf16(const float* src, void* dst, long n, void* stream) {
  NSID_REQUIRE(src && dst && n > 0 && n % 8 == 0 && nsid_aligned16(src) && nsid_aligned16(dst));
  NSID_LAUNCH(f32_to_bf16_kernel, dim3(grid_for(n / 8, 4096)), dim3(256), 0, static_cast<hipStream_t>(stream), src,
              static_cast<__bf16*>(dst), n / 8);
  return nsid_launch_status();
}

extern "C" int nsid_bcn_to_rows(const float* x, int B, int C, int N, void* rows, int ld, int rows_dtype, void* stream) {
  NSID_REQUIRE(x && rows && B > 0 && C > 0 && N > 0 && ld >= C && NSID_DTYPE_OK(rows_dtype));
  NSID_DISPATCH_DTYPE(rows_dtype, T, {
    NSID_LAUNCH((transpose_kernel<float, T>), dim3((N + 31) / 32, (C + 31) / 32, B), dim3(256), 0,
                static_cast<hipStream_t>(stream), x, (long)C * N, (long)N, static_cast<T*>(rows), (long)N * ld, (long)ld,
                C, N);
  });
  return nsid_launch_status();
}
extern "C" int nsid_rows_to_bcn(const void* rows, int ld, int B, int C, int N, float* x, int rows_dtype, void* stream) {
  NSID_REQUIRE(x && rows && B > 0 && C > 0 && N > 0 && ld >= C && NSID_DTYPE_OK(rows_dtype));
  NSID_DISPATCH_DTYPE(rows_dtype, T, {
    NSID_LAUNCH((transpose_kernel<T, float>), dim3((C + 31) / 32, (N + 31) / 32, B), dim3(256), 0,
                static_cast<hipStream_t>(stream), static_cast<const T*>(rows), (long)N * ld, (long)ld, x, (long)C * N,
                (long)N, N, C);
  });
  return nsid_launch_status();
}

__global__ __launch_bounds__(256) void fill_zero_kernel(f32x4* __restrict__ p, long n16) {
  const f32x4 z = {0.f, 0.f, 0.f, 0.f};
  for (long i = (long)blockIdx.x * blockDim.x + threadIdx.x; i < n16; i += (long)gridDim.x * blockDim.x) p[i] = z;
}
__global__ void fill_zero_tail_kernel(unsigned char* __restrict__ p, long n) {
  for (long i = (long)blockIdx.x * blockDim.x + threadIdx.x; i < n; i += (long)gridDim.x * blockDim.x) p[i] = 0;
}
__global__ void scale_f32_kernel(const float* __restrict__ x, const float* __restrict__ s, long n, float* __restrict__ out) {
  const float f = s != nullptr ? s[0] : 1.f;
  for (long i = (long)blockIdx.x * blockDim.x + threadIdx.x; i < n; i += (long)gridDim.x * blockDim.x) out[i] = x[i] * f;
}

extern "C" int nsid_fill_zero(void* p, size_t bytes, void* stream) {
  NSID_REQUIRE(p && bytes > 0 && nsid_aligned16(p));
  const long n16 = (long)(bytes / 16);
  hipStream_t s = static_cast<hipStream_t>(stream);
  if (n16 > 0) {
    NSID_LAUNCH(fill_zero_kernel, dim3(grid_for(n16, 2048)), dim3(256), 0, s, static_cast<f32x4*>(p), n16);
    if (nsid_launch_status() != NSID_OK) return NSID_ELAUNCH;
  }
  if (bytes % 16) {
    NSID_LAUNCH(fill_zero_tail_kernel, dim3(1), dim3(64), 0, s, static_cast<unsigned char*>(p) + 16 * n16,
                (long)(bytes % 16));
    return nsid_launch_status();
  }
  return NSID_OK;
}
extern "C" int nsid_scale_f32(const float* x, const float* scale, long n, float* out, void* stream) {
  NSID_REQUIRE(x && out && n > 0);
  NSID_LAUNCH(scale_f32_kernel, dim3(grid_for(n, 1024)), dim3(256), 0, static_cast<hipStream_t>(stream), x, scale, n, out);
  return nsid_launch_status();
}
```

neuralsampleid_amd/csrc/nsid_common.h:

```cpp
#pragma once
#include <hip/hip_runtime.h>
#include <stdint.h>
#include <stdio.h>

#include "../../include/nsid.h"

typedef float f32x2 __attribute__((ext_vector_type(2)));
typedef float f32x4 __attribute__((ext_vector_type(4)));
typedef uint32_t u32x4 __attribute__((ext_vector_type(4)));
typedef __bf16 bf16x4 __attribute__((ext_vector_type(4)));
typedef __bf16 bf16x8 __attribute__((ext_vector_type(8)));

template <typename T> struct Chunk;
template <> struct Chunk<float> {
  static constexpr int N = 4;
  __device__ static __forceinline__ void load(const float* p, float* v) {
    const f32x4 x = *reinterpret_cast<const f32x4*>(p);
#pragma unroll
    for (int e = 0; e < 4; ++e) v[e] = x[e];
  }
  __device__ static __forceinline__ void store(float* p, const float* v) {
    *reinterpret_cast<f32x4*>(p) = f32x4{v[0], v[1], v[2], v[3]};
  }
};
template <> struct Chunk<__bf16> {
  static constexpr int N = 8;
  __device__ static __forceinline__ void load(const __bf16* p, float* v) {
    const bf16x8 x = *reinterpret_cast<const bf16x8*>(p);
#pragma unroll
    for (int e = 0; e < 8; ++e) v[e] = (float)x[e];
  }
  __device__ static __forceinline__ void store(__bf16* p, const float* v) {
    bf16x8 x;
#pragma unroll
    for (int e = 0; e < 8; ++e) x[e] = (__bf16)v[e];
    *reinterpret_cast<bf16x8*>(p) = x;
  }
};

template <int N>
__device__ __forceinline__ void load_channels(const float* __restrict__ p, int c, float* v) {
#pragma unroll
  for (int e = 0; e < N; e += 4) {
    const f32x4 x = *reinterpret_cast<const f32x4*>(p + c + e);
    v[e] = x[0]; v[e + 1] = x[1]; v[e + 2] = x[2]; v[e + 3] = x[3];
  }
}

#define NSID_DISPATCH_DTYPE(dtype, T, ...)                    \
  do {                                                        \
    if ((dtype) == NSID_BF16) { typedef __bf16 T; __VA_ARGS__; } \
    else { typedef float T; __VA_ARGS__; }                    \
  } while (0)
#define NSID_DTYPE_OK(d) ((d) == NSID_F32 || (d) == NSID_BF16)

#define NSID_WAVE 64

__device__ __forceinline__ float nsid_act(float v, int act) {
  switch (act) {
    case NSID_ACT_RELU: return v < 0.f ? 0.f : v;
    case NSID_ACT_LEAKY: return v > 0.f ? v : 0.2f * v;
    case NSID_ACT_ELU: return v > 0.f ? v : expm1f(v);
    default: return v;
  }
}
__device__ __forceinline__ float nsid_act_grad(float pre, int act) {
  switch (act) {
    case NSID_ACT_RELU: return pre > 0.f ? 1.f : 0.f;
    case NSID_ACT_LEAKY: return pre > 0.f ? 1.f : 0.2f;
    default: return 1.f;
  }
}

__device__ __forceinline__ float wave_sum(float v) {
  v += __builtin_bit_cast(float, __builtin_amdgcn_update_dpp(0, __builtin_bit_cast(int, v), 0xB1, 0xF, 0xF, true));
  v += __builtin_bit_cast(float, __builtin_amdgcn_update_dpp(0, __builtin_bit_cast(int, v), 0x4E, 0xF, 0xF, true));
  v += __builtin_bit_cast(float, __builtin_amdgcn_update_dpp(0, __builtin_bit_cast(int, v), 0x141, 0xF, 0xF, true));
  v += __builtin_bit_cast(float, __builtin_amdgcn_update_dpp(0, __builtin_bit_cast(int, v), 0x140, 0xF, 0xF, true));
  v += __builtin_bit_cast(float, __builtin_amdgcn_update_dpp(0, __builtin_bit_cast(int, v), 0x142, 0xA, 0xF, true));
  v += __builtin_bit_cast(float, __builtin_amdgcn_update_dpp(0, __builtin_bit_cast(int, v), 0x143, 0xC, 0xF, true));
  return __builtin_bit_cast(float, __builtin_amdgcn_readlane(__builtin_bit_cast(int, v), 63));
}
__device__ __forceinline__ double wave_sum_d(double v) {
#pragma unroll
  for (int o = 32; o > 0; o >>= 1) v += __shfl_xor(v, o, 64);
  return v;
}
__device__ __forceinline__ float wave_max(float v) {
#pragma unroll
  for (int o = 32; o > 0; o >>= 1) v = fmaxf(v, __shfl_xor(v, o, 64));
  return v;
}
__device__ __forceinline__ float wave_min(float v) {
#pragma unroll
  for (int o = 32; o > 0; o >>= 1) v = fminf(v, __shfl_xor(v, o, 64));
  return v;
}

__device__ __forceinline__ int lane_id() { return (int)__builtin_amdgcn_mbcnt_hi(~0u, __builtin_amdgcn_mbcnt_lo(~0u, 0u)); }
__device__ __forceinline__ f32x4 ld4(const float* p) { return *reinterpret_cast<const f32x4*>(p); }

template <int VM, int LGKM = 0xF>
__device__ __forceinline__ void nsid_waitcnt() {
  static_assert(VM >= 0 && VM < 64 && LGKM >= 0 && LGKM < 16, "6-bit vmcnt, 4-bit lgkmcnt");
  __builtin_amdgcn_s_waitcnt((VM & 0xF) | ((VM >> 4) << 14) | (7 << 4) | (LGKM << 8));
}
template <int N> __device__ __forceinline__ void wait_vm() { nsid_waitcnt<N>(); }
__device__ __forceinline__ void wait_lgkm0() { nsid_waitcnt<63, 0>(); }

__device__ __forceinline__ void glds16(const char* sbase, unsigned voff, unsigned dst) {
  unsigned keep;
  asm volatile("s_mov_b32 %0, m0\n\ts_mov_b32 m0, %3\n\ts_nop 0\n\tglobal_load_lds_dwordx4 %1, %2\n\ts_mov_b32 m0, %0"
               : "=&s"(keep) : "v"(voff), "s"(sbase), "s"(dst) : "memory");
}

#define NSID_LAUNCH(kernel, grid, block, shmem, stream, ...)                \
  do {                                                                      \
    (void)hipGetLastError();                                                \
    hipLaunchKernelGGL(kernel, grid, block, shmem, stream, __VA_ARGS__);    \
  } while (0)

static inline int nsid_launch_status() {
  hipError_t e = hipGetLastError();
  if (e != hipSuccess) fprintf(stderr, "[nsid] kernel launch failed: %s\n", hipGetErrorString(e));
  return e == hipSuccess ? NSID_OK : NSID_ELAUNCH;
}
static inline bool nsid_aligned16(const void* p) { return (reinterpret_cast<uintptr_t>(p) & 15u) == 0; }

#define NSID_REQUIRE(cond) \
  do {                     \
    if (!(cond)) return NSID_EINVAL; \
  } while (0)

#define NSID_TUNING_TABLE(X)                                                                                                  \
  X(stream_max_wg, 2048)                              \
  X(bn_bwd_apply_max_wg, 384)        \
  X(gemm_deep_ks, 2)                 \
  X(gemm_deep_max_wg, 1024)     \
  X(gemm_deep_kinds, 5)         \
  X(bwd_split_max_tiles, 64)    \
  X(fwd_narrow, -1)                                         \
  X(bwd_narrow, -1)                                                                                                           \
  X(g256_min, 512)                                  \
  X(g256_train, 0)                            \
  X(g256_grid, 0)                                           \
  X(wgrad_wide, 1)                                     \
  X(wgrad_rect, 1)                                                                          \
  X(wgrad_wgs_rect, 256)                         \
  X(wgrad_wgs_sq, 1024)                                                                                                       \
  X(wgrad_rect_min, 256)                                                                                                      \
  X(wgrad_sq_min, 256)                                                                                                        \
  X(w3_wgs, 256)                                                                                                              \
  X(w3_min_tiles, 64)                                                                                                         \
  X(knn_strips, 0)                                            \
  X(knn_pair_min, 512)                 \
  X(knn_raw16, 1)               \
  X(knn_raw_wpe, 6)             \
  X(knn_sel_min_n, 128)               \
  X(mr_grid_stride, 0)                              \
  X(mr_split, 0)                                             \
  X(ffn_regs, 3)                \
  X(mr_key_min_k, 8)            \
  X(mr_bwd_sorted_min_k, 3)     \
  X(ffn_waves, 8)                                                \
  X(ffn256, 1)                  \
  X(mrconv_variant, 7)          \
  X(mrconv_pg_wgs, 768)         \
  X(wgg_rows, 4096)             \
  X(wgg_rows_sq, 1024)          \
  X(wgg_rows_gen, 512)          \
  X(bn_fin_tiles, 0)            \
  X(wgg_w3, 1)                  \
  X(wgrad256, 1)                \
  X(wgg_rows256, 4096)          \
  X(ws_gemm, 7)

enum NsidTuneKey {
#define NSID_TUNE_ENUM(name, def) NSID_T_##name,
  NSID_TUNING_TABLE(NSID_TUNE_ENUM)
#undef NSID_TUNE_ENUM
  NSID_T_COUNT
};
extern long g_nsid_tune[NSID_T_COUNT];
static inline long nsid_tune(NsidTuneKey k) { return g_nsid_tune[k]; }

#define NSID_COUNTER_TABLE(X)                                                                  \
  X(gemm_fwd) X(gemm_bwd_data) X(gemm_bwd_weight)              \
  X(gemm_full)                                    \
  X(gemm_ks2)                                                           \
  X(gemm_bwd_split)          \
  X(gemm_split_major)           \
  X(gemm_affine_load)          \
  X(gemm_relu_load)                                                                             \
  X(gemm_bn_sums)              \
  X(gemm_bn_apply_load)     \
  X(gemm256)                                                                   \
  X(ws_fwd) X(ws_bwd_data) X(ws_bwd_bnapply)                    \
  X(wgrad_rect) X(wgrad_square) X(wgrad3) X(wgrad_grouped) X(wgrad_grouped_w3) X(wgrad_grouped_256)                                                 \
  X(bn_bwd_apply) X(bn_bwd_apply_capped)                                                        \
  X(knn2) X(knn2_pair) X(knn2_raw) X(knn_rank) X(knn_sel) X(knn_strips) X(knn_big)                                                  \
  X(mr_fwd_lds) X(mr_fwd_grid) X(mr_fwd_key) X(mr_bwd_sorted)                                                                  \
  X(ffn_fused)                                 \
  X(mrconv_fused)          \
  X(row_sqnorm) X(flat_l2_topk) X(flat_l2_topk_wide) X(seq_scores)    \
  X(clf_node_rows) X(clf_pair_scores)            \
  X(clf_node_rows_n) X(clf_pair_scores_n)        \
  X(clf_mine) X(clf_attn_fwd) X(clf_head_fwd) X(clf_head_bwd) X(clf_attn_bwd) X(clf_seg_reduce)    \
  X(logmel_fft)            \
  X(conv2d_3x3) X(conv2d_1x1) X(ibn_relu) X(stem7_pool) X(gem_pool)

enum NsidCounterKey {
#define NSID_CNT_ENUM(name) NSID_C_##name,
  NSID_COUNTER_TABLE(NSID_CNT_ENUM)
#undef NSID_CNT_ENUM
  NSID_C_COUNT
};
extern long g_nsid_counter[NSID_C_COUNT];
static inline void nsid_count(NsidCounterKey k) { ++g_nsid_counter[k]; }

constexpr int WGG_MAXP = 28;
struct WgProb {
  const void* A[2];
  const void* B[2];
  const float* bsc[2];
  const float* bsh[2];
  float* C;
  int lda, ldb, I, J, R;
  int groups, rchunk;
  int seg_splits, nsplit;
  int tiles, nwg;
  float slope;
  int pad_period, pad_c1;
};
struct WgGroupArgs {
  int n, pad;
  int wg0[WGG_MAXP + 1];
  WgProb prob[WGG_MAXP];
};
static_assert(sizeof(WgProb) == 128 && sizeof(WgGroupArgs) + 256 <= 4096, "the problem table travels in the kernel arguments");


__device__ __forceinline__ bool wgg_decode(const WgGroupArgs& ga, const int w, int& pi, int& split, int& bid, int& g, int& seg) {
  pi = 0;
  for (int i = 1; i < ga.n; ++i) pi += (w >= ga.wg0[i]) ? 1 : 0;
  pi = __builtin_amdgcn_readfirstlane(pi);
  const WgProb& q = ga.prob[pi];
  const int l = w - ga.wg0[pi];
  if (l >= q.nwg) return false;
  const int S = q.nsplit;
  int rest;
  if (S < 8 && (8 % S) == 0) {
    const int x = l & 7, per = 8 / S;
    split = x % S;
    rest = (l >> 3) * per + x / S;
  } else {
    split = l % S;
    rest = l / S;
  }
  if (rest >= q.tiles * q.groups) return false;
  g = rest / q.tiles;
  bid = rest % q.tiles;
  seg = split >= q.seg_splits ? 1 : 0;
  split -= seg * q.seg_splits;
  return true;
}
int nsid_wgrad3_grouped_launch(const WgGroupArgs& ga, int grid, bool affine, hipStream_t stream);
int nsid_wgrad4_grouped_launch(const WgGroupArgs& ga, int grid, hipStream_t stream);

int nsid_wgrad2_launch(const void* dout, int ldd, const void* x, int ldx, float* dw, int M, int Nout, int K, int groups,
                       const float* in_scale, const float* in_shift, float slope, hipStream_t stream);

int nsid_gemm256_fwd_launch(const void* x, int ldx, const void* w, const float* bias, const void* addend, int ldadd, void* out,
                            int ldo, int M, int Nout, int K, bool relu_out, float* stat, long stat_plane, long stat_ld,
                            hipStream_t stream);
int nsid_ws_fwd_launch(const void* x, int ldx, const void* w, const float* bias, void* out, int ldo, int M, int Nout, int K,
                       int groups, const float* in_scale, const float* in_shift, float in_slope, float* stat, long stat_plane,
                       long stat_ld, hipStream_t stream);
int nsid_ws_bwd_data_launch(const void* dout, int ldd, const void* w, const void* addend, int ldadd, void* din, int ldi, int M, int Nout,
                            int K, int groups, const void* bn_r, long bn_ldr, const float* bn_scale, const float* bn_shift,
                            const float* bn_mean, const float* bn_invstd, float bn_slope, float* bn_partial, long bn_plane, long bn_ld,
                            const void* abn_r, const float* abn_coef, long abn_plane, float abn_slope, void* abn_dr, long abn_lddr,
                            hipStream_t stream);
int nsid_ffn256_fused_launch(const void* x, const void* w1, const float* b1, const void* w2, const float* b2, void* out, int M, int C,
                             int H, hipStream_t stream);
void nsid_l2_plan(long nq, long nx, int* splits, int* chunk);
long nsid_l2_ws_bytes(long nq, long nx, int k);
extern void* g_gemm_trace_host;
```

neuralsampleid_amd/csrc/ntxent.hip:

```cpp
#include "nsid_common.h"

namespace {

constexpr int RB = 16;
constexpr int CBK = 128;

__device__ __forceinline__ const float* zrow(const float* z_i, const float* z_j, int row, int d) {
  return ((row & 1) ? z_j : z_i) + (long)(row >> 1) * d;
}

__device__ __forceinline__ void stage_rows(float* dst, int ld, const float* z_i, const float* z_j, int row0, int nrows,
                                           int M, int d) {
  const int d4 = d >> 2;
  constexpr int UB = 8;
  for (int q0 = threadIdx.x; q0 < nrows * d4; q0 += UB * blockDim.x) {
    f32x4 v[UB];
#pragma unroll
    for (int u = 0; u < UB; ++u) {
      const int q = q0 + u * blockDim.x;
      const int rr = q / d4, c = (q % d4) * 4;
      v[u] = f32x4{0.f, 0.f, 0.f, 0.f};
      if (q < nrows * d4 && row0 + rr < M) v[u] = *reinterpret_cast<const f32x4*>(zrow(z_i, z_j, row0 + rr, d) + c);
    }
#pragma unroll
    for (int u = 0; u < UB; ++u) {
      const int q = q0 + u * blockDim.x;
      const int rr = q / d4, c = (q % d4) * 4;
      if (q < nrows * d4) *reinterpret_cast<f32x4*>(dst + rr * ld + c) = v[u];
    }
  }
}

constexpr int PF_MAX = 16;
struct Prefetch { f32x4 v[PF_MAX]; };

__device__ __forceinline__ void prefetch_rows(Prefetch& pf, const float* z_i, const float* z_j, int row0, int nrows, int M,
                                              int d) {
  const int d4 = d >> 2;
#pragma unroll
  for (int u = 0; u < PF_MAX; ++u) {
    const int q = threadIdx.x + u * 256;
    const int rr = q / d4, c = (q % d4) * 4;
    pf.v[u] = f32x4{0.f, 0.f, 0.f, 0.f};
    if (q < nrows * d4 && row0 + rr < M) pf.v[u] = *reinterpret_cast<const f32x4*>(zrow(z_i, z_j, row0 + rr, d) + c);
  }
}

__device__ __forceinline__ void commit_rows(float* dst, int ld, const Prefetch& pf, int nrows, int d) {
  const int d4 = d >> 2;
#pragma unroll
  for (int u = 0; u < PF_MAX; ++u) {
    const int q = threadIdx.x + u * 256;
    const int rr = q / d4, c = (q % d4) * 4;
    if (q < nrows * d4) *reinterpret_cast<f32x4*>(dst + rr * ld + c) = pf.v[u];
  }
}

template <int NT>
__device__ __forceinline__ void sim_tiles(const float* zi_w, const float* zj_t, int ld, int d, int lr, int rq,
                                          f32x4 (&acc)[NT]) {
#pragma unroll
  for (int u = 0; u < NT; ++u) acc[u] = f32x4{0.f, 0.f, 0.f, 0.f};
  const float* pa = zj_t + lr * ld + 4 * rq;
  const float* pb = zi_w + lr * ld + 4 * rq;
  for (int ch = 0; ch < d; ch += 16) {
    const f32x4 fb = *reinterpret_cast<const f32x4*>(pb + ch);
    f32x4 fa[NT];
#pragma unroll
    for (int u = 0; u < NT; ++u) fa[u] = *reinterpret_cast<const f32x4*>(pa + u * 16 * ld + ch);
#pragma unroll
    for (int e = 0; e < 4; ++e)
#pragma unroll
      for (int u = 0; u < NT; ++u) acc[u] = __builtin_amdgcn_mfma_f32_16x16x4f32(fa[u][e], fb[e], acc[u], 0, 0, 0);
  }
}


__global__ __launch_bounds__(256) void ntxent_lse_kernel(const float* __restrict__ z_i, const float* __restrict__ z_j,
                                                         int M, int d, float tau, int cols_per_group,
                                                         float* __restrict__ lse, float* __restrict__ rowloss,
                                                         float* __restrict__ part_out) {
  extern __shared__ __attribute__((aligned(16))) float sm[];
  const int ld = d + 4;
  float* zi_s = sm;
  float* zj_s = sm + RB * ld;
  float* part = zj_s + CBK * ld;
  const int i0 = blockIdx.x * RB;
  const int lane = threadIdx.x & 63, wave = threadIdx.x >> 6, lr = lane & 15, rq = lane >> 4;
  stage_rows(zi_s, ld, z_i, z_j, i0, RB, M, d);
  const int i = i0 + lr;
  float mrun = -__builtin_inff(), srun = 0.f, pos = 0.f;
  constexpr int TPW = CBK / 16 / 4;
  const bool pipelined = CBK * (d >> 2) <= PF_MAX * 256;
  Prefetch pf;
  const int jbeg = blockIdx.y * cols_per_group, jend = min(M, jbeg + cols_per_group);
  if (pipelined) {
    prefetch_rows(pf, z_i, z_j, jbeg, CBK, M, d);
    __syncthreads();
    commit_rows(zj_s, ld, pf, CBK, d);
  }
  for (int j0 = jbeg; j0 < jend; j0 += CBK) {
    if (pipelined) {
      __syncthreads();
      prefetch_rows(pf, z_i, z_j, j0 + CBK, CBK, M, d);
    } else {
      __syncthreads();
      stage_rows(zj_s, ld, z_i, z_j, j0, CBK, M, d);
      __syncthreads();
    }
    f32x4 acc[TPW];
    sim_tiles<TPW>(zi_s, zj_s + 16 * (wave * TPW) * ld, ld, d, lr, rq, acc);
#pragma unroll
    for (int u = 0; u < TPW; ++u) {
#pragma unroll
      for (int e = 0; e < 4; ++e) {
        const int j = j0 + 16 * (wave * TPW + u) + 4 * rq + e;
        const float a = acc[u][e] / tau;
        if (j < M && j != i) {
          if (j == (i ^ 1)) pos = a;
          const float mn = fmaxf(mrun, a);
          srun = srun * expf(mrun - mn) + expf(a - mn);
          mrun = mn;
        }
      }
    }
    if (pipelined) {
      __syncthreads();
      commit_rows(zj_s, ld, pf, CBK, d);
    }
  }
#pragma unroll
  for (int o = 16; o <= 32; o <<= 1) {
    const float m2 = __shfl_xor(mrun, o, 64), s2 = __shfl_xor(srun, o, 64), p2 = __shfl_xor(pos, o, 64);
    const float mn = fmaxf(mrun, m2);
    const float e1 = mrun == -__builtin_inff() ? 0.f : expf(mrun - mn);
    const float e2 = m2 == -__builtin_inff() ? 0.f : expf(m2 - mn);
    srun = srun * e1 + s2 * e2;
    mrun = mn;
    pos += p2;
  }
  if (rq == 0) { part[(wave * 3 + 0) * 16 + lr] = mrun; part[(wave * 3 + 1) * 16 + lr] = srun; part[(wave * 3 + 2) * 16 + lr] = pos; }
  __syncthreads();
  if (threadIdx.x < 16 && i0 + (int)threadIdx.x < M) {
    float m = -__builtin_inff(), sacc = 0.f, p = 0.f;
#pragma unroll
    for (int w = 0; w < 4; ++w) {
      const float m2 = part[(w * 3 + 0) * 16 + threadIdx.x], s2 = part[(w * 3 + 1) * 16 + threadIdx.x];
      const float mn = fmaxf(m, m2);
      const float e1 = m == -__builtin_inff() ? 0.f : expf(m - mn);
      const float e2 = m2 == -__builtin_inff() ? 0.f : expf(m2 - mn);
      sacc = sacc * e1 + s2 * e2;
      m = mn;
      p += part[(w * 3 + 2) * 16 + threadIdx.x];
    }
    if (gridDim.y > 1) {
      float* po = part_out + (long)blockIdx.y * 3 * M + i0 + threadIdx.x;
      po[0] = m; po[M] = sacc; po[2 * M] = p;
    } else {
      const float l = m + logf(sacc);
      lse[i0 + threadIdx.x] = l;
      rowloss[i0 + threadIdx.x] = l - p;
    }
  }
}

__global__ void ntxent_lse_merge_kernel(const float* __restrict__ part, int groups, int M, float* __restrict__ lse,
                                        float* __restrict__ rowloss) {
  const int i = blockIdx.x * blockDim.x + threadIdx.x;
  if (i >= M) return;
  float m = -__builtin_inff(), sacc = 0.f, p = 0.f;
  for (int g = 0; g < groups; ++g) {
    const float m2 = part[(long)g * 3 * M + i], s2 = part[(long)g * 3 * M + M + i];
    const float mn = fmaxf(m, m2);
    const float e1 = m == -__builtin_inff() ? 0.f : expf(m - mn);
    const float e2 = m2 == -__builtin_inff() ? 0.f : expf(m2 - mn);
    sacc = sacc * e1 + s2 * e2;
    m = mn;
    p += part[(long)g * 3 * M + 2 * M + i];
  }
  const float l = m + logf(sacc);
  lse[i] = l;
  rowloss[i] = l - p;
}

template <int DT>
__global__ __launch_bounds__(256) void ntxent_grad_kernel(const float* __restrict__ z_i, const float* __restrict__ z_j,
                                                          int M, int d, float tau, const float* __restrict__ lse,
                                                          int row0, int nrows, int cols_per_group,
                                                          float* __restrict__ dz_i, float* __restrict__ dz_j) {
  extern __shared__ __attribute__((aligned(16))) float sm[];
  const int ld = d + 4;
  float* zi_s = sm;
  float* zj_s = sm + RB * ld;
  const int i0 = row0 + blockIdx.x * RB;
  const int lane = threadIdx.x & 63, wave = threadIdx.x >> 6, lr = lane & 15, rq = lane >> 4;
  stage_rows(zi_s, ld, z_i, z_j, i0, RB, M, d);
  const int i = i0 + lr;
  const bool iok = i < row0 + nrows && i < M;
  const float lse_i = iok ? lse[i] : 0.f;
  f32x4 out[DT];
#pragma unroll
  for (int c = 0; c < DT; ++c) out[c] = f32x4{0.f, 0.f, 0.f, 0.f};
  constexpr int TPW = CBK / 16 / 4;
  const bool pipelined = CBK * (d >> 2) <= PF_MAX * 256;
  Prefetch pf;
  const int jbeg = blockIdx.y * cols_per_group, jend = min(M, jbeg + cols_per_group);
  if (pipelined) {
    prefetch_rows(pf, z_i, z_j, jbeg, CBK, M, d);
    __syncthreads();
    commit_rows(zj_s, ld, pf, CBK, d);
  }
  for (int j0 = jbeg; j0 < jend; j0 += CBK) {
    if (pipelined) {
      __syncthreads();
      prefetch_rows(pf, z_i, z_j, j0 + CBK, CBK, M, d);
    } else {
      __syncthreads();
      stage_rows(zj_s, ld, z_i, z_j, j0, CBK, M, d);
      __syncthreads();
    }
    f32x4 acc[TPW];
    sim_tiles<TPW>(zi_s, zj_s + 16 * (wave * TPW) * ld, ld, d, lr, rq, acc);
#pragma unroll
    for (int u = 0; u < TPW; ++u) {
      const int jt = wave * TPW + u;
      f32x4 q;
#pragma unroll
      for (int e = 0; e < 4; ++e) {
        const int j = j0 + 16 * jt + 4 * rq + e;
        float v = 0.f;
        if (iok && j < M && j != i) {
          const float a = acc[u][e] / tau;
          v = expf(a - lse_i) + expf(a - lse[j]);
          if (j == (i ^ 1)) v -= 2.f;
        }
        q[e] = v;
      }
      const float* zb = zj_s + (16 * jt + 4 * rq) * ld + lr;
#pragma unroll
      for (int c = 0; c < DT; ++c)
#pragma unroll
        for (int e = 0; e < 4; ++e)
          out[c] = __builtin_amdgcn_mfma_f32_16x16x4f32(q[e], zb[e * ld + 16 * c], out[c], 0, 0, 0);
    }
    if (pipelined) {
      __syncthreads();
      commit_rows(zj_s, ld, pf, CBK, d);
    }
  }
  __syncthreads();
  float* red = zj_s;
#pragma unroll
  for (int e = 0; e < 4; ++e)
#pragma unroll
    for (int c = 0; c < DT; ++c) red[(wave * 16 + 4 * rq + e) * ld + 16 * c + lr] = out[c][e];
  __syncthreads();
  const float sc = 1.f / ((float)M * tau);
  for (int q = threadIdx.x; q < RB * d; q += blockDim.x) {
    const int rr = q / d, c = q % d;
    const int row = i0 + rr;
    if (row < row0 + nrows && row < M) {
      const float v = (red[rr * ld + c] + red[(16 + rr) * ld + c]) + (red[(32 + rr) * ld + c] + red[(48 + rr) * ld + c]);
      float* dst = ((row & 1) ? dz_j : dz_i) + (long)((row >> 1) - (row0 >> 1)) * d;
      if (gridDim.y > 1) atomicAdd(dst + c, v * sc);
      else dst[c] = v * sc;
    }
  }
}

__global__ __launch_bounds__(256) void ntxent_loss_kernel(const float* __restrict__ rowloss, int row0, int nrows, int M,
                                                          float* __restrict__ loss_out) {
  __shared__ double red[4];
  double s = 0.0;
  for (int i = threadIdx.x; i < nrows; i += blockDim.x) s += (double)rowloss[row0 + i];
  s = wave_sum_d(s);
  if ((threadIdx.x & 63) == 0) red[threadIdx.x >> 6] = s;
  __syncthreads();
  if (threadIdx.x == 0) loss_out[0] = (float)((red[0] + red[1] + red[2] + red[3]) / (double)M);
}

template <typename K>
int raise_lds(K kernel, size_t bytes) {
  if (bytes <= 64 * 1024) return NSID_OK;
  return hipFuncSetAttribute(reinterpret_cast<const void*>(kernel), hipFuncAttributeMaxDynamicSharedMemorySize,
                             (int)bytes) == hipSuccess ? NSID_OK : NSID_ELAUNCH;
}

}

constexpr int LSE_MAX_GROUPS = 16;
extern "C" size_t nsid_ntxent_ws_floats(int Bg) { return (size_t)4 * Bg + 8 + (size_t)LSE_MAX_GROUPS * 3 * 2 * Bg; }

extern "C" int nsid_ntxent_fwd_bwd(const float* z_i, const float* z_j, int Bg, int d, float tau, int p0, int np,
                                   float* ws, float* loss_out, float* dz_i, float* dz_j, void* stream) {
  NSID_REQUIRE(z_i && z_j && ws && loss_out && Bg > 0 && np > 0 && p0 >= 0 && p0 + np <= Bg && tau > 0.f);
  NSID_REQUIRE(d % 16 == 0 && d <= 256 && nsid_aligned16(z_i) && nsid_aligned16(z_j));
  NSID_REQUIRE((dz_i == nullptr) == (dz_j == nullptr));
  const int M = 2 * Bg;
  float* lse = ws;
  float* rowloss = ws + M;
  hipStream_t s = static_cast<hipStream_t>(stream);
  const size_t bytes = ((size_t)(RB + CBK) * (d + 4) + 4 * 3 * 16) * sizeof(float);
  if (raise_lds(ntxent_lse_kernel, bytes) != NSID_OK) return NSID_ELAUNCH;
  {
    const int row_tiles = (M + RB - 1) / RB, nblocks = (M + CBK - 1) / CBK;
    int cg = row_tiles >= 512 ? 1 : (512 + row_tiles - 1) / row_tiles;
    if (cg > nblocks) cg = nblocks;
    if (cg > LSE_MAX_GROUPS) cg = LSE_MAX_GROUPS;
    const int cols_per_group = (nblocks + cg - 1) / cg * CBK;
    cg = (M + cols_per_group - 1) / cols_per_group;
    float* part = ws + 2 * M + 8;
    NSID_LAUNCH(ntxent_lse_kernel, dim3(row_tiles, cg), dim3(256), bytes, s, z_i, z_j, M, d, tau, cols_per_group, lse,
                rowloss, part);
    if (cg > 1) NSID_LAUNCH(ntxent_lse_merge_kernel, dim3((M + 255) / 256), dim3(256), 0, s, part, cg, M, lse, rowloss);
  }
  NSID_LAUNCH(ntxent_loss_kernel, dim3(1), dim3(256), 0, s, rowloss, 2 * p0, 2 * np, M, loss_out);
  if (dz_i != nullptr) {
    const int row0 = 2 * p0, nrows = 2 * np;
    const int row_tiles = (nrows + RB - 1) / RB, nblocks = (M + CBK - 1) / CBK;
    int cg = row_tiles >= 128 ? 1 : (256 + row_tiles - 1) / row_tiles;
    if (cg > nblocks) cg = nblocks;
    const int cols_per_group = (nblocks + cg - 1) / cg * CBK;
    cg = (M + cols_per_group - 1) / cols_per_group;
    if (cg > 1) {
      if (hipMemsetAsync(dz_i, 0, (size_t)np * d * sizeof(float), s) != hipSuccess ||
          hipMemsetAsync(dz_j, 0, (size_t)np * d * sizeof(float), s) != hipSuccess)
        return NSID_ELAUNCH;
    }
    dim3 grid(row_tiles, cg);
#define NSID_NTX_CASE(DTV)                                                                                   \
  case DTV:                                                                                                  \
    if (raise_lds(ntxent_grad_kernel<DTV>, bytes) != NSID_OK) return NSID_ELAUNCH;                           \
    NSID_LAUNCH((ntxent_grad_kernel<DTV>), grid, dim3(256), bytes, s, z_i, z_j, M, d, tau, lse, row0, \
                       nrows, cols_per_group, dz_i, dz_j);                                                                   \
    break;
    switch (d / 16) {
      NSID_NTX_CASE(1) NSID_NTX_CASE(2) NSID_NTX_CASE(4) NSID_NTX_CASE(8) NSID_NTX_CASE(16)
      default: return NSID_EINVAL;
    }
#undef NSID_NTX_CASE
  }
  return nsid_launch_status();
}
```

neuralsampleid_amd/ops.py:

```python
import os
from typing import Optional, Tuple

import torch

from ._lib import call, get_tuning, launch_counters, lib, reset_tuning, set_tuning

ACT_NONE, ACT_RELU, ACT_LEAKY, ACT_ELU = 0, 1, 2, 3
ROW_TILE = 128
BN_MOMENTUM = 0.1
BN_EPS = 1e-5


class KernelProfile:

    def __init__(self):
        self.records = []
        self.bracket_ms = self._empty_bracket_ms()

    @staticmethod
    def plug(ms: float = 120.0) -> None:
        torch.cuda._sleep(int(ms * 1e-3 * 2.0e9))

    @staticmethod
    def _empty_bracket_ms(n: int = 64) -> float:
# ... 31 lines not shown
            d = out.setdefault((name,) + shape, [0, 0.0, flops, nbytes])
            d[0] += 1
            d[1] += self._ms(e0, e1)
        rows = []
        for key, (n, ms, flops, nbytes) in out.items():
            us = 1e3 * ms / n
            rows.append({"kernel": key[0], "M": key[1], "Nout": key[2], "K": key[3], "groups": key[4], "launches": n,
                         "avg_us": round(us, 1), "tflops": round(flops / us / 1e6, 1),
                         "alg_GBps": round(nbytes / us / 1e3, 0), "total_ms": round(ms, 3)})
        return sorted(rows, key=lambda r: -r["total_ms"])


PROFILE: Optional[KernelProfile] = None


def _timed(name, flops, nbytes, fn, shape=()):
    if PROFILE is None:
        return fn()
    e0, e1 = torch.cuda.Event(enable_timing=True), torch.cuda.Event(enable_timing=True)
    e0.record()
    fn()
    e1.record()
    PROFILE.records.append((name() if callable(name) else name, flops, nbytes, e0, e1, shape))


def _cnt(key: str) -> int:
    return int(lib.nsid_debug_counter(key.encode())) if PROFILE is not None else 0


def _p(t: Optional[torch.Tensor]):
    return None if t is None else t.data_ptr()


def _stream():
    return torch.cuda.current_stream().cuda_stream


def _chk(*ts):
    for t in ts:
        if t is None:
            continue
        if not t.is_cuda:
            raise RuntimeError("neuralsampleid_amd ops need tensors on the MI355X (cuda) device; there is no CPU path")
        if t.dtype != torch.float32 or not t.is_contiguous():
            raise RuntimeError(f"expected contiguous float32, got {t.dtype} contiguous={t.is_contiguous()}")


F32, BF16 = 0, 1


def _tk(name, nbytes, fn, shape=()):
    return _timed(name, 0.0, float(nbytes), fn, shape)


def _act(*ts) -> int:
    code = None
    for t in ts:
        if t is None:
            continue
        if not t.is_cuda:
            raise RuntimeError("neuralsampleid_amd ops need tensors on the MI355X (cuda) device; there is no CPU path")
        if t.dtype not in (torch.float32, torch.bfloat16) or not t.is_contiguous():
            raise RuntimeError(f"expected contiguous float32/bfloat16, got {t.dtype} contiguous={t.is_contiguous()}")
        c = BF16 if t.dtype == torch.bfloat16 else F32
        if code is not None and c != code:
            raise RuntimeError("activation tensors of one call must share a storage type")
        code = c
    return code


GEMM_FP32, GEMM_BF16 = 0, 1


def set_gemm_precision(mode: str) -> None:
    call("nsid_set_gemm_precision", {"fp32": GEMM_FP32, "bf16": GEMM_BF16}[mode])


def get_gemm_precision() -> str:
    return "bf16" if lib.nsid_get_gemm_precision() == GEMM_BF16 else "fp32"


def row_tiles(M: int) -> int:
    return (M + ROW_TILE - 1) // ROW_TILE


def w2d(w: torch.Tensor) -> torch.Tensor:
    return w.reshape(w.shape[0], -1)


WEIGHT_EPOCH = 0
STATS_EPOCH = 0


def bump_state_epoch(weights: bool = True, stats: bool = True) -> None:
    global WEIGHT_EPOCH, STATS_EPOCH
    if weights:
        WEIGHT_EPOCH += 1
    if stats:
        STATS_EPOCH += 1


class WeightShadows:

    def __init__(self):
        self.entries = {}

    def register(self, w: torch.Tensor, shadow: torch.Tensor, owner: torch.Tensor, fresh: bool = False) -> None:
        import weakref
        self.entries[w.data_ptr()] = [shadow, (w._version, WEIGHT_EPOCH) if fresh else None, w.numel(), weakref.ref(owner)]

    def mark_fresh(self, w: torch.Tensor) -> None:
        e = self.entries.get(w.data_ptr())
        if e is not None:
            e[1] = (w._version, WEIGHT_EPOCH)

    def clear(self) -> None:
        self.entries.clear()

    def purge(self) -> int:
        dead = [k for k, e in self.entries.items() if e[3]() is None]
        for k in dead:
            del self.entries[k]
        return len(dead)

    def operand(self, w: torch.Tensor) -> torch.Tensor:
        e = self.entries.get(w.data_ptr())
        if e is not None and e[3]() is None:
            del self.entries[w.data_ptr()]
            e = None
        if e is None or e[2] != w.numel():
            return f32_to_bf16(w)
        key = (w._version, WEIGHT_EPOCH)
        if e[1] != key:
            f32_to_bf16(w, e[0])
            e[1] = key
        return e[0]


SHADOWS = WeightShadows()


def register_weight_shadows(module) -> int:
    n = 0
    for p in module.parameters():
        if p.is_cuda and p.dim() >= 2 and p.numel() % 8 == 0 and p.data_ptr() not in SHADOWS.entries:
            SHADOWS.register(p.data, torch.empty(p.numel(), device=p.device, dtype=torch.bfloat16), owner=p)
            n += 1
    return n


def f32_to_bf16(src: torch.Tensor, dst: Optional[torch.Tensor] = None) -> torch.Tensor:
    _chk(src)
    n = src.numel()
    if dst is None:
        dst = torch.empty(((n + 7) // 8 * 8,), device=src.device, dtype=torch.bfloat16)
    if n % 8:
        dst[:n].copy_(src.reshape(-1))
        return dst
    _tk("f32_to_bf16_kernel", 6.0 * n, lambda: call("nsid_f32_to_bf16", _p(src), _p(dst), n, _stream()), (n, 1, 0, 1))
    return dst


def _weight(w: torch.Tensor, dt: int, K: int):
    if dt == BF16 and K % 8 == 0 and w.numel() % 8 == 0:
        return SHADOWS.operand(w), BF16
    return w, F32


def linear_fwd(x, w, bias, M, Nout, K, groups=1, in_scale=None, in_shift=None, act_in=ACT_NONE, act_out=ACT_NONE,
               want_stat=False, ksplit=1, out=None, addend=None, in_aff=None) -> Tuple[torch.Tensor, Optional[torch.Tensor]]:
    if in_aff is not None:
        in_scale, in_shift = in_aff.scale, in_aff.shift
    _chk(w, bias, in_scale, in_shift)
    dt = _act(x, out, addend)
    if addend is not None and (want_stat or ksplit != 1 or act_out != ACT_NONE):
        raise ValueError("the residual addend rides with a plain epilogue (no statistics, no split-K, no output activation)")
    ldx = x.shape[-1]
    if out is None:
        out = torch.empty((M, groups * Nout), device=x.device, dtype=x.dtype)
        if ksplit > 1:
            fill_zero(out)
    stat = torch.empty((2, row_tiles(M), groups * Nout), device=x.device, dtype=torch.float32) if want_stat else None
    half = dt == BF16 or lib.nsid_get_gemm_precision() == GEMM_BF16
    narrow = (Nout <= 64 or (Nout <= 128 and K <= 256 and in_scale is None)) if half else Nout <= 64
    if half and row_tiles(M) * ((Nout + 127) // 128) * groups < 128:
        narrow = True
    esz = x.element_size()
    wop, wdt = _weight(w, dt, K)
    name_ = "gemm_kernel<128,%d,true,true>" % (64 if narrow else 128)
    n256 = lib.nsid_gemm_g256_launches() if PROFILE is not None else 0
    nws = _cnt("ws_fwd")
    name = lambda: ("ws_fwd_kernel" if _cnt("ws_fwd") > nws else
                    ("gemm256_fwd_kernel" if lib.nsid_gemm_g256_launches() > n256 else name_))
    if in_scale is None and act_in != ACT_NONE:
        bn_ = 64 if narrow else 128
        bm_ = 128
        if not (act_in == ACT_RELU and dt == BF16 and wdt == BF16 and M % bm_ == 0 and Nout % bn_ == 0 and K % 64 == 0
                and ksplit == 1):
            raise ValueError("activation-on-load without an affine needs ReLU, bf16 storage, bf16 weights and whole tiles")
    if addend is not None:
        _timed(name, 2.0 * M * Nout * K * groups,
               groups * (esz * M * K + float(wop.element_size()) * Nout * K + 2 * esz * M * Nout), lambda: call(
            "nsid_linear_fwd_res", _p(x), ldx, _p(wop), wdt, _p(bias), _p(addend), addend.shape[-1], _p(out),
            out.shape[-1], M, Nout, K, groups, _p(in_scale), _p(in_shift), act_in, dt, _stream()), (M, Nout, K, groups))
        return out, None
    _timed(name, 2.0 * M * Nout * K * groups,
           groups * (esz * M * K + float(wop.element_size()) * Nout * K + esz * M * Nout), lambda: call(
        "nsid_linear_fwd", _p(x), ldx, _p(wop), wdt, _p(bias), _p(out), out.shape[-1], M, Nout, K, groups, _p(in_scale),
        _p(in_shift), act_in, act_out, _p(stat), ksplit, dt, _stream()), (M, Nout, K, groups))
    return out, stat


FUSE_EVAL_FFN = True


def ffn_fused_fwd(x, w1f, b1f, w2f, b2f, M, C, H):
    _chk(w1f, b1f, w2f, b2f)
    if _act(x) != BF16 or x.shape != (M, C) or not FUSE_EVAL_FFN:
        return None
    w1, d1 = _weight(w1f, BF16, C)
    w2, d2 = _weight(w2f, BF16, H)
    if d1 != BF16 or d2 != BF16:
        return None
    out = torch.empty_like(x)
    rc = [0]

    def launch():
        rc[0] = lib.nsid_ffn_fused_fwd(_p(x), _p(w1), _p(b1f), _p(w2), _p(b2f), _p(out), M, C, H, _stream())
    _timed("ffn_fused_kernel", 4.0 * M * C * H, 2.0 * x.element_size() * M * C + 4.0 * C * H, launch, (M, C, H, 1))
    if rc[0] == 1:
        if PROFILE is not None:
            PROFILE.records.pop()
        return None
    if rc[0] != 0:
        raise RuntimeError(f"nsid_ffn_fused_fwd failed: {rc[0]}")
    return out


FUSE_EVAL_MRCONV = True


def mrconv_fused_fwd(y, idx, B, N, C, wf, bf):
    _chk(wf, bf)
    if not FUSE_EVAL_MRCONV or _act(y) != BF16 or y.shape != (B * N, C) or idx.dtype != torch.int32 or not idx.is_contiguous():
        return None
    w, dw = _weight(wf, BF16, C // 2)
    if dw != BF16:
        return None
    k = idx.shape[-1]
    out = torch.empty((B * N, 2 * C), device=y.device, dtype=y.dtype)
    rc = [0]

    def launch():
        rc[0] = lib.nsid_mrconv_fused_fwd(_p(y), _p(idx), B, N, C, k, _p(w), _p(bf), _p(out), _stream())
    _timed("mrconv_fused_kernel", 2.0 * B * N * (C // 2) * (C // 2) * 4, float(B) * N * (3 * C * y.element_size() + k * 4), launch,
           (B * N, C // 2, C // 2, 4))
    if rc[0] == 1:
        if PROFILE is not None:
            PROFILE.records.pop()
        return None
    if rc[0] != 0:
        raise RuntimeError(f"nsid_mrconv_fused_fwd failed: {rc[0]}")
    return out


FUSE_BN_BWD_REDUCE = True


def linear_bwd_data(dout, w, M, Nout, K, groups=1, addend=None, out=None, bn=None):
    _chk(w)
    dt = _act(dout, addend, out)
    if out is None:
        out = torch.empty((M, groups * K), device=dout.device, dtype=dout.dtype)
    half = dt == BF16 or lib.nsid_get_gemm_precision() == GEMM_BF16
    narrow = (K <= 64 or (K <= 128 and Nout <= 256)) if half else K <= 64
    if half and row_tiles(M) * ((K + 127) // 128) * groups < 128:
        narrow = True
    name_ = "gemm_kernel<128,%d,true,false>" % (64 if narrow else 128)
    nws = _cnt("ws_bwd_data")
    name = lambda: "ws_bwd_kernel" if _cnt("ws_bwd_data") > nws else name_
    esz = dout.element_size()
    wop, wdt = _weight(w, dt, K)
    want_pair = bn is not None
    bn = bn or None
    fuse = bn is not None and FUSE_BN_BWD_REDUCE and dt == BF16 and out.shape[-1] == groups * K and (groups * K) % 8 == 0
    if fuse and tuple(bn[0].shape) != (M, groups * K):
        fuse = False
    nbytes = groups * (esz * M * Nout + float(wop.element_size()) * Nout * K
                       + esz * M * K * ((2 if addend is not None else 1) + (1 if fuse else 0)))
    if fuse:
        r, aff, act = bn
        _act(r, out)
        partial = torch.empty((2, row_tiles(M), groups * K), device=dout.device, dtype=torch.float32)
        _timed(name, 2.0 * M * Nout * K * groups, nbytes, lambda: call(
            "nsid_linear_bwd_data_bn", _p(dout), dout.shape[-1], _p(wop), wdt, _p(addend),
            0 if addend is None else addend.shape[-1], _p(out), out.shape[-1], M, Nout, K, groups, dt, _p(r),
            _p(aff.scale), _p(aff.shift), _p(aff.mean), _p(aff.invstd), act, _p(partial), _stream()),
            (M, Nout, K, groups))
        return out, partial
    _timed(name, 2.0 * M * Nout * K * groups, nbytes, lambda: call(
        "nsid_linear_bwd_data", _p(dout), dout.shape[-1], _p(wop), wdt, _p(addend),
        0 if addend is None else addend.shape[-1], _p(out), out.shape[-1], M, Nout, K, groups, dt, _stream()),
        (M, Nout, K, groups))
    return (out, None) if want_pair else out


# ... 295 lines not shown


def bn_backward(dout, r, aff: BNAffine, act, dgamma, dbeta, inplace=False, partial=None) -> torch.Tensor:
    dt = _act(dout, r)
    M, C = r.shape
    tiles = row_tiles(M) if partial is None else partial.shape[1]
    s = _stream()
    coef = torch.empty((2, C), device=r.device, dtype=torch.float32)
    if partial is None:
        partial = torch.empty((2, tiles, C), device=r.device, dtype=torch.float32)
        part_ = partial
        _tk("col_reduce_kernel", 2.0 * r.element_size() * M * C, lambda: call(
            "nsid_bn_bwd_reduce", _p(dout), _p(r), M, C, _p(aff.scale), _p(aff.shift), _p(aff.mean), _p(aff.invstd),
            act, _p(part_), dt, s), (M, C, 0, 1))
    if DIAG_SKIP_FINALIZE & 2:
        coef = _diag_const(C, r.device)[2]
    else:
        _tk("bn_bwd_finalize_kernel", 8.0 * tiles * C + 16.0 * C, lambda: call(
            "nsid_bn_bwd_finalize", _p(partial), tiles, C, M, _p(dgamma), _p(dbeta), _p(coef), s), (M, C, 0, 1))
    dr = dout if inplace else torch.empty_like(dout)
    _tk("bn_bwd_apply_kernel", 3.0 * r.element_size() * M * C, lambda: call(
        "nsid_bn_bwd_apply", _p(dout), _p(r), M, C, _p(aff.scale), _p(aff.shift), _p(aff.mean), _p(aff.invstd),
        act, _p(coef), _p(dr), dt, s), (M, C, 0, 1))
    return dr


def knn_graph(r, B, N, C, k, dilation=1, aff: Optional[BNAffine] = None) -> torch.Tensor:
    dt = _act(r)
    if aff is not None and aff.identity:
        aff = None
    idx = torch.empty((B, N, k), device=r.device, dtype=torch.int32)
    kd = k * dilation
    sel = 8 < kd <= 64 and N >= get_tuning("knn_sel_min_n")
    name_ = "knn2_kernel" if kd <= 8 else ("knn_sel_kernel" if sel else ("knn_rank_kernel" if N <= 128 else "knn_kernel"))
    nraw = _cnt("knn2_raw")
    name = lambda: "knn2_raw_kernel" if _cnt("knn2_raw") > nraw else name_
    _timed(name, 2.0 * B * N * N * C, float(B) * (N * C * r.element_size() + N * k * 4), lambda: call(
        "nsid_knn_graph", _p(r), r.shape[-1], _p(aff.scale) if aff else None, _p(aff.shift) if aff else None,
        B, N, C, k, dilation, _p(idx), dt, _stream()), (B * N, N, C, 1))
    return idx


def mr_aggregate_fwd(r, idx, B, N, C, aff: Optional[BNAffine] = None, want_argmax=True):
    dt = _act(r)
    if aff is not None and aff.identity:
        aff = None
    k = idx.shape[-1]
    u = torch.empty((B * N, 2 * C), device=r.device, dtype=r.dtype)
    amax = torch.empty((B * N, C), device=r.device, dtype=torch.uint8) if want_argmax else None
    nbytes = float(B) * N * (3 * C * r.element_size() + k * 4 + (C if want_argmax else 0))
    _timed("mr_fwd_kernel", 0.0, nbytes, lambda: call(
        "nsid_mr_aggregate_fwd", _p(r), r.shape[-1], _p(aff.scale) if aff else None,
        _p(aff.shift) if aff else None, _p(idx), B, N, C, k, _p(u), _p(amax), dt, _stream()), (B * N, 2 * C, C, 1))
    return u, amax


def mr_bwd_sums_fused(du, N, C, k) -> bool:
    kmin = get_tuning("mr_bwd_sorted_min_k")
    return bool(FUSE_MR_BWD_SUMS and du.dtype == torch.bfloat16 and kmin > 0 and k >= kmin and N * C == 16384 and C & (C - 1) == 0
                and 64 <= C <= 512)


FUSE_MR_BWD_SUMS = True


def mr_aggregate_bwd(du, idx, amax, B, N, C, bn=None):
    dt = _act(du)
    k = idx.shape[-1]
    dy = torch.empty((B * N, C), device=du.device, dtype=du.dtype)
    nbytes = float(B) * N * (3 * C * du.element_size() + k * 4 + C)
    if bn is not None and mr_bwd_sums_fused(du, N, C, k):
        r, aff, act = bn
        _chk(aff.scale, aff.shift, aff.mean, aff.invstd)
        partial = torch.empty((2, B, C), device=du.device, dtype=torch.float32)
        rc = [0]

        def launch():
            rc[0] = lib.nsid_mr_aggregate_bwd_bn(_p(du), _p(idx), _p(amax), B, N, C, k, _p(dy), _p(r), r.shape[-1], _p(aff.scale),
                                                 _p(aff.shift), _p(aff.mean), _p(aff.invstd), act, _p(partial), dt, _stream())
        _timed("mr_bwd_sorted_kernel +bn_sums", 0.0, nbytes + float(B) * N * C * r.element_size(), launch, (B * N, C, 2 * C, 1))
        if rc[0] == 0:
            return dy, partial
        if PROFILE is not None:
            PROFILE.records.pop()
    c0 = _cnt("mr_bwd_sorted")
    _timed(lambda: "mr_bwd_sorted_kernel" if _cnt("mr_bwd_sorted") > c0 else "mr_bwd_kernel", 0.0, nbytes, lambda: call(
        "nsid_mr_aggregate_bwd", _p(du), _p(idx), _p(amax), B, N, C, k, _p(dy), dt, _stream()),
        (B * N, C, 2 * C, 1))
    return (dy, None) if bn is not None else dy


def ds_out_nodes(N: int) -> int:
    return (N - 1) // 2 + 1


def im2col3_fwd(x, B, N, C) -> torch.Tensor:
    dt = _act(x)
    col = torch.empty((B * ds_out_nodes(N), 3 * C), device=x.device, dtype=x.dtype)
    call("nsid_im2col3_fwd", _p(x), B, N, C, _p(col), dt, _stream())
    return col


def im2col3_bwd(dcol, B, N, C) -> torch.Tensor:
    dt = _act(dcol)
    dx = torch.empty((B * N, C), device=dcol.device, dtype=dcol.dtype)
    call("nsid_im2col3_bwd", _p(dcol), B, N, C, _p(dx), dt, _stream())
    return dx


class DsPrep:

    def __init__(self):
        self.entries = {}

    MAX_LAYERS = 8

    def purge(self) -> None:
        for ptr in [k for k, e in self.entries.items() if e["wref"]() is None or e["wref"]().data_ptr() != k]:
            del self.entries[ptr]

    def register(self, w) -> None:
        import weakref
        self.purge()
        if w.data_ptr() in self.entries:
            return
        if len(self.entries) >= self.MAX_LAYERS:
            import warnings
            warnings.warn(f"DsPrep holds {self.MAX_LAYERS} Downsample layers; a further one keeps the per-call pack / convert / zero "
                          "launches (slower, same results)")
            return
        Cout, Cin = w.shape[0], w.shape[1]
        dev = w.device
        self.entries[w.data_ptr()] = dict(wref=weakref.ref(w), Cout=Cout, Cin=Cin, key=None,
                                          wp16=torch.empty((Cout, 3 * Cin), device=dev, dtype=torch.bfloat16),
                                          wb16=torch.empty((2 * Cout, Cin), device=dev, dtype=torch.bfloat16),
                                          dwp=torch.empty((2, Cout, 3 * Cin), device=dev, dtype=torch.float32), slots=0)

    def clear(self) -> None:
        self.entries.clear()

    def _arrays(self, es, *names):
        import ctypes
        n = len(es)
        out = []
        for name in names:
            if name in ("Cout", "Cin"):
                out.append((ctypes.c_int * n)(*[e[name] for e in es]))
            elif name == "w":
                out.append((ctypes.c_void_p * n)(*[e["wref"]().data_ptr() for e in es]))
            else:
                out.append((ctypes.c_void_p * n)(*[e[name].data_ptr() for e in es]))
        return out

    def refresh(self) -> None:
        self.purge()
        es = [e for e in self.entries.values() if e["wref"]().is_cuda] if DS_PREP_ENABLED else []
        if not es:
            return
        w, wp16, wb16, dwp, Cout, Cin = self._arrays(es, "w", "wp16", "wb16", "dwp", "Cout", "Cin")
        _tk("ds_prepack_kernel", sum(4.0 * e["wref"]().numel() / 3 + 2.0 * 5 * e["Cout"] * e["Cin"] + 12.0 * e["Cout"] * e["Cin"] for e in es),
            lambda: call("nsid_ds_prepack", len(es), w, wp16, wb16, dwp, Cout, Cin, _stream()))
        for e in es:
            e["key"], e["slots"] = (e["wref"]()._version, WEIGHT_EPOCH), 0

    def take_slot(self, e):
        if e["slots"] >= e["dwp"].shape[0]:
            return None
        e["slots"] += 1
        return e["dwp"][e["slots"] - 1]

    def get(self, w):
        e = self.entries.get(w.data_ptr())
        if not DS_PREP_ENABLED or e is None or e["key"] != (w._version, WEIGHT_EPOCH):
            return None
        owner = e["wref"]()
        if owner is None or (owner is not w and (owner.data_ptr() != w.data_ptr() or owner.shape != w.shape or
                                                 owner.untyped_storage().data_ptr() != w.untyped_storage().data_ptr())):
            return None
        return e


DS_PREP = DsPrep()
DS_PREP_ENABLED = 1


def downsample3_fwd(x, B, N, C, wp, bias, Cout, want_stat=False, w16=None):
    _chk(wp, bias)
    dt = _act(x)
    No = N // 2
    M = B * No
    out = torch.empty((M, Cout), device=x.device, dtype=x.dtype)
    stat = torch.empty((2, row_tiles(M), Cout), device=x.device, dtype=torch.float32) if want_stat else None
    wop, wdt = (w16, BF16) if (w16 is not None and dt == BF16) else _weight(wp, dt, 3 * C)
    esz = x.element_size()
    _timed("gemm_kernel<128,%d,true,true>" % (64 if Cout <= 64 else 128), 2.0 * M * Cout * 3 * C,
           esz * B * N * C + float(wop.element_size()) * Cout * 3 * C + esz * M * Cout, lambda: call(
        "nsid_downsample3_fwd", _p(x), B, N, C, _p(wop), wdt, _p(bias), _p(out), Cout, _p(stat), dt, _stream()),
        (M, Cout, 3 * C, 1))
    return out, stat


def downsample3_bwd_weight(dout, x, dwp, B, N, C, Cout) -> None:
    _chk(dwp)
    dt = _act(dout, x)
    M = B * (N // 2)
    esz = x.element_size()
    _timed("gemm_kernel<64,64,false,false>", 2.0 * M * Cout * 3 * C, esz * (M * Cout + B * N * C) + 4.0 * Cout * 3 * C,
           lambda: call("nsid_downsample3_bwd_weight", _p(dout), _p(x), _p(dwp), B, N, C, Cout, dt, _stream()),
           (M, Cout, 3 * C, 1))


def downsample3_bwd_data(dout, wp, w_odd, B, N, C, Cout, w16=None) -> torch.Tensor:
    dt = _act(dout)
    dx = torch.empty((B * N, C), device=dout.device, dtype=dout.dtype)
    if w16 is not None and dt == BF16:
        wop, oop, wdt, odt = w16[0], w16[1], BF16, BF16
    else:
        _chk(wp, w_odd)
        wop, wdt = _weight(wp, dt, 3 * C)
        oop, odt = _weight(w_odd, dt, C)
    if odt != wdt:
        wop, wdt, oop, odt = wp, F32, w_odd, F32
    M = B * (N // 2)
    esz = dout.element_size()
    _timed("gemm_kernel<128,%d,true,false>" % (64 if C <= 64 else 128), 2.0 * M * Cout * 3 * C,
           esz * (M * Cout + B * N * C) + float(wop.element_size()) * Cout * 3 * C, lambda: call(
        "nsid_downsample3_bwd_data", _p(dout), _p(wop), _p(oop), wdt, _p(dx), B, N, C, Cout, dt, _stream()),
        (M, Cout, 3 * C, 1))
    return dx


def pack_ds_weight_bwd(w) -> torch.Tensor:
    _chk(w)
    Cout, Cin = w.shape[0], w.shape[1]
    wb = torch.empty((2 * Cout, Cin), device=w.device, dtype=torch.float32)
    call("nsid_pack_ds_weight_bwd", _p(w), Cout, Cin, _p(wb), _stream())
    return wb


def pack_ds_weight(w) -> torch.Tensor:
    _chk(w)
    Cout, Cin = w.shape[0], w.shape[1]
    wp = torch.empty((Cout, 3 * Cin), device=w.device, dtype=torch.float32)
    call("nsid_pack_ds_weight", _p(w), Cout, Cin, _p(wp), _stream())
    return wp


def unpack_ds_wgrad(dwp, dw) -> None:
    _chk(dwp, dw)
    call("nsid_unpack_ds_wgrad", _p(dwp), dw.shape[0], dw.shape[1], _p(dw), _stream())


def dsact_fwd(x, B, N, C, w, bias, Cout, in_aff: Optional["BNAffine"] = None, act_in=ACT_NONE, want_stat=False,
              out_aff: Optional["BNAffine"] = None, act_out=ACT_NONE):
    dt = _act(x)
    _chk(w, bias, *((in_aff.scale, in_aff.shift) if in_aff is not None else ()),
         *((out_aff.scale, out_aff.shift) if out_aff is not None else ()))
    No = ds_out_nodes(N)
    M = B * No
    out = torch.empty((M, Cout), device=x.device, dtype=x.dtype)
    stat = torch.empty((2, row_tiles(M), Cout), device=x.device, dtype=torch.float32) if want_stat else None
    _timed("dsact_fwd_kernel", 2.0 * M * Cout * 3 * C, float(x.element_size()) * (B * N * C + M * Cout), lambda: call(
        "nsid_dsact_fwd", _p(x), B, N, C, _p(in_aff.scale) if in_aff else None, _p(in_aff.shift) if in_aff else None, act_in,
        _p(w), _p(bias), _p(out), Cout, _p(stat), _p(out_aff.scale) if out_aff else None, _p(out_aff.shift) if out_aff else None,
        act_out, dt, _stream()), (M, Cout, 3 * C, 1))
    return out, stat


def dsact_bwd_weight(dout, x, dw, B, N, C, Cout, in_aff: Optional["BNAffine"] = None, act_in=ACT_NONE) -> None:
    dt = _act(dout, x)
    _chk(dw, *((in_aff.scale, in_aff.shift) if in_aff is not None else ()))
    M = dout.shape[0]
    _timed("dsact_wgrad_kernel", 2.0 * M * Cout * 3 * C, float(x.element_size()) * (B * N * C + M * Cout), lambda: call(
        "nsid_dsact_bwd_weight", _p(dout), _p(x), _p(in_aff.scale) if in_aff else None, _p(in_aff.shift) if in_aff else None,
        act_in, _p(dw), B, N, C, Cout, dt, _stream()), (Cout, 3 * C, M, 1))


def dsact_bwd_data(dout, w, B, N, C, Cout, r_prev=None, aff: Optional["BNAffine"] = None, act=ACT_NONE, want_partial=False):
    dt = _act(dout, r_prev)
    _chk(w)
    if r_prev is not None:
        _chk(aff.scale, aff.shift)
    if want_partial:
        _chk(aff.mean, aff.invstd)
    dx = torch.empty((B * N, C), device=dout.device, dtype=dout.dtype)
    partial = torch.empty((2, int(lib.nsid_dsact_part_rows(B, N)), C), device=dout.device, dtype=torch.float32) \
        if want_partial else None
    M = dout.shape[0]
    _timed("dsact_dgrad_kernel", 2.0 * M * Cout * 3 * C, float(dout.element_size()) * (M * Cout + 2 * B * N * C), lambda: call(
        "nsid_dsact_bwd_data", _p(dout), _p(w), _p(dx), B, N, C, Cout, _p(r_prev), _p(aff.scale) if aff else None,
        _p(aff.shift) if aff else None, _p(aff.mean) if want_partial else None, _p(aff.invstd) if want_partial else None, act,
        _p(partial), dt, _stream()), (B * N, C, 3 * Cout, 1))
    return dx, partial


def peak_patchify_fwd(spec, w, bias, pb, pf, out_dtype=torch.float32):
    _chk(spec, w, bias)
    B, H, W = spec.shape
    F = w.shape[0]
    n = (H // pb) * (W // pf)
    out = torch.empty((B * n, F), device=spec.device, dtype=out_dtype)
    minmax = torch.empty((B, 2), device=spec.device, dtype=torch.float32)
    _tk("patchify_fwd_kernel", 4.0 * B * H * W + float(out.element_size()) * B * n * F, lambda: call(
        "nsid_peak_patchify_fwd", _p(spec), _p(w), _p(bias), B, H, W, pb, pf, F, _p(out), F, _p(minmax), _act(out),
        _stream()), (B * n, F, pb * pf * 3, 1))
    return out, minmax


PATCHIFY_BWD_WS = True


def peak_patchify_bwd(spec, minmax, out, dout, pb, pf, dw, dbias) -> None:
    _chk(spec, minmax, dw, dbias)
    B, H, W = spec.shape
    F = out.shape[-1]
    nbytes = 4.0 * B * H * W + 2.0 * out.element_size() * out.numel()
    if PATCHIFY_BWD_WS and (H, W, pb, pf, F) == (64, 128, 4, 8, 8) and out.is_contiguous() and dout.is_contiguous():
        ws = torch.empty((B, 776), device=spec.device, dtype=torch.float32)
        _tk("patchify_bwd2_kernel", nbytes + 8.0 * ws.numel(), lambda: call(
            "nsid_peak_patchify_bwd_ws", _p(spec), _p(minmax), _p(out), _p(dout), F, B, H, W, pb, pf, F, _p(dw), _p(dbias), _p(ws),
            _act(out, dout), _stream()), (out.shape[0], out.shape[1], pb * pf * 3, 1))
        return
    _tk("patchify_bwd_kernel", nbytes, lambda: call(
        "nsid_peak_patchify_bwd", _p(spec), _p(minmax), _p(out), _p(dout), out.shape[-1], B, H, W, pb, pf,
        out.shape[-1], _p(dw), _p(dbias), _act(out, dout), _stream()), (out.shape[0], out.shape[1], pb * pf * 3, 1))


def node_mean_fwd(x, B, N, C) -> torch.Tensor:
    out = torch.empty((B, C), device=x.device, dtype=torch.float32)
    _tk("node_mean_fwd_kernel", float(x.element_size()) * B * N * C, lambda: call(
        "nsid_node_mean_fwd", _p(x), B, N, C, _p(out), _act(x), _stream()), (B * N, C, 0, 1))
    return out


def node_mean_bwd(dout, B, N, C, dtype=torch.float32) -> torch.Tensor:
    _chk(dout)
    dx = torch.empty((B * N, C), device=dout.device, dtype=dtype)
    _tk("node_mean_bwd_kernel", float(dx.element_size()) * B * N * C, lambda: call(
        "nsid_node_mean_bwd", _p(dout), B, N, C, _p(dx), _act(dx), _stream()), (B * N, C, 0, 1))
    return dx


def elu_bwd(dout, out) -> torch.Tensor:
    _chk(dout, out)
    din = torch.empty_like(dout)
    call("nsid_elu_bwd", _p(dout), _p(out), out.numel(), _p(din), _stream())
    return din


def l2norm_fwd(p, eps):
    _chk(p)
    B, d = p.shape
    z = torch.empty_like(p)
    norm = torch.empty((B,), device=p.device, dtype=torch.float32)
    call("nsid_l2norm_fwd", _p(p), B, d, eps, _p(z), _p(norm), _stream())
    return z, norm


def l2norm_bwd(dz, z, norm, eps) -> torch.Tensor:
    _chk(dz, z, norm)
    B, d = z.shape
    dp = torch.empty_like(z)
    call("nsid_l2norm_bwd", _p(dz), _p(z), _p(norm), B, d, eps, _p(dp), _stream())
    return dp


def ntxent_fwd_bwd(z_i, z_j, tau, p0=0, npairs=None, want_grad=True):
    _chk(z_i, z_j)
    Bg, d = z_i.shape
    npairs = Bg if npairs is None else npairs
    ws = torch.empty((lib.nsid_ntxent_ws_floats(Bg),), device=z_i.device, dtype=torch.float32)
    loss = torch.empty((1,), device=z_i.device, dtype=torch.float32)
    dzi = torch.empty((npairs, d), device=z_i.device, dtype=torch.float32) if want_grad else None
    dzj = torch.empty((npairs, d), device=z_i.device, dtype=torch.float32) if want_grad else None
    _timed("ntxent_kernels", 2.0 * (2 * Bg) * (2 * npairs) * d * (2 if want_grad else 1), 4.0 * d * (2 * Bg + 2 * npairs), lambda: call(
        "nsid_ntxent_fwd_bwd", _p(z_i), _p(z_j), Bg, d, float(tau), p0, npairs, _p(ws), _p(loss), _p(dzi), _p(dzj),
        _stream()), (2 * npairs, 2 * Bg, d, 1))
    return loss, dzi, dzj


def fill_zero(t: torch.Tensor) -> torch.Tensor:
    if not (t.is_cuda and t.is_contiguous()):
        raise RuntimeError("fill_zero needs a contiguous device tensor")
    _tk("fill_zero_kernel", float(t.numel() * t.element_size()), lambda: call(
        "nsid_fill_zero", _p(t), t.numel() * t.element_size(), _stream()), (t.numel(), 1, 0, 1))
    return t


def zeros(shape, device, dtype=torch.float32) -> torch.Tensor:
    return fill_zero(torch.empty(shape, device=device, dtype=dtype))


def scale_f32(x: torch.Tensor, scale: Optional[torch.Tensor] = None, out: Optional[torch.Tensor] = None) -> torch.Tensor:
    _chk(x, out)
    if scale is not None:
        scale = scale.reshape(-1)
        _chk(scale)
    if out is None:
        out = torch.empty_like(x)
    call("nsid_scale_f32", _p(x), _p(scale), x.numel(), _p(out), _stream())
    return out


def logmel_fft(waves: torch.Tensor, n_fft: int, hop: int, window: torch.Tensor, twiddle: torch.Tensor, fb: torch.Tensor,
               band: torch.Tensor) -> torch.Tensor:
    _chk(window, twiddle, fb)
    if waves.dim() != 2 or not waves.is_cuda or waves.dtype != torch.float32 or waves.stride(1) != 1:
        raise RuntimeError("logmel_fft takes (B, L) float32 waveforms on the MI355X device with a contiguous last dimension")
    B, L = waves.shape
    if L <= n_fft // 2:
        raise RuntimeError(f"waveforms of {L} samples are too short for reflect padding by n_fft/2 = {n_fft // 2}")
    n_mels, T = fb.shape[0], 1 + L // hop
    out = torch.empty((B, n_mels, T), device=waves.device, dtype=torch.float32)
    call("nsid_logmel_fft", _p(waves), waves.stride(0) if B > 1 else L, B, L, n_fft, hop, _p(window), _p(twiddle), _p(fb),
         _p(band), n_mels, _p(out), n_mels * T, T, _stream())
    return out


def batched_index_select_fwd(x: torch.Tensor, idx: torch.Tensor) -> torch.Tensor:
    _chk(x)
    B, C, N = x.shape
    _, Nq, k = idx.shape
    out = torch.empty((B, C, Nq, k), device=x.device, dtype=torch.float32)
    call("nsid_batched_index_select_fwd", _p(x), _p(idx), B, C, N, Nq, k, _p(out), _stream())
    return out


def batched_index_select_bwd(dout: torch.Tensor, idx: torch.Tensor, N: int) -> torch.Tensor:
    _chk(dout)
    B, C, Nq, k = dout.shape
    dx = zeros((B, C, N), dout.device)
    call("nsid_batched_index_select_bwd", _p(dout), _p(idx), B, C, N, Nq, k, _p(dx), _stream())
    return dx


def sumsq_partial(g_flat) -> torch.Tensor:
    _chk(g_flat)
    n = g_flat.numel()
    partial = torch.empty((lib.nsid_sumsq_blocks(n),), device=g_flat.device, dtype=torch.float32)
    _tk("sumsq_kernel", 4.0 * n, lambda: call("nsid_sumsq_partial", _p(g_flat), n, _p(partial), _stream()), (n, 1, 0, 1))
    return partial


def adam_step(p, g, m, v, hyper, step, partial, gnorm_out) -> None:
    _chk(p, g, m, v, hyper, partial, gnorm_out)
    _tk("adam_kernel", 28.0 * p.numel(), lambda: call(
        "nsid_adam_step", _p(p), _p(g), _p(m), _p(v), p.numel(), _p(hyper), _p(step), _p(partial), partial.numel(),
        _p(gnorm_out), _stream()), (p.numel(), 1, 0, 1))


def bcn_to_rows(x, dtype=torch.float32) -> torch.Tensor:
    _chk(x)
    B, C, N = x.shape[0], x.shape[1], x.shape[2]
    rows = torch.empty((B * N, C), device=x.device, dtype=dtype)
    call("nsid_bcn_to_rows", _p(x), B, C, N, _p(rows), C, _act(rows), _stream())
    return rows


def rows_to_bcn(rows, B, N) -> torch.Tensor:
    C = rows.shape[-1]
    x = torch.empty((B, C, N), device=rows.device, dtype=torch.float32)
    call("nsid_rows_to_bcn", _p(rows), C, B, C, N, _p(x), _act(rows), _stream())
    return x


SEARCH_MAX_K = 64
SEARCH_D_LIMITS = "d % 16 == 0 and 16 <= d <= 256, or d % 64 == 0 and 256 < d <= 2048"


def search_d_ok(d) -> bool:
    return (d % 16 == 0 and 16 <= d <= 256) or (d % 64 == 0 and 256 < d <= 2048)


def _search_rows(t, name):
    if not t.is_cuda:
        raise RuntimeError("neuralsampleid_amd ops need tensors on the MI355X (cuda) device; there is no CPU path")
    if t.dtype != torch.float32 or t.dim() != 2 or t.stride(1) != 1 or t.stride(0) % 4 or t.data_ptr() % 16:
        raise RuntimeError(f"{name}: expected a (rows, d) float32 matrix with unit column stride and 16-byte aligned rows")
    d = t.shape[1]
    if not search_d_ok(d):
        raise ValueError(f"{name}: d = {d} is outside the search kernels' limits ({SEARCH_D_LIMITS})")
    return max(t.stride(0), d)


def row_sqnorm(x) -> torch.Tensor:
    ldx = _search_rows(x, "row_sqnorm")
    n, d = x.shape
    out = torch.empty((n,), device=x.device, dtype=torch.float32)
    _tk("row_sqnorm_kernel", 4.0 * n * (d + 1), lambda: call("nsid_row_sqnorm", _p(x), ldx, n, d, _p(out), _stream()), (n, d, 0, 1))
    return out


def flat_l2_topk(q, x, x_sqnorm, k, q_sqnorm=None) -> Tuple[torch.Tensor, torch.Tensor]:
    k = int(k)
    if not 1 <= k <= SEARCH_MAX_K:
        raise ValueError(f"flat_l2_topk: k = {k} is outside [1, {SEARCH_MAX_K}]")
    ldq, ldx = _search_rows(q, "flat_l2_topk q"), _search_rows(x, "flat_l2_topk x")
    if q.shape[1] != x.shape[1]:
        raise ValueError(f"flat_l2_topk: query d = {q.shape[1]} != database d = {x.shape[1]}")
    _chk(x_sqnorm)
    nq, d = q.shape
    nx = x.shape[0]
    if x_sqnorm.numel() != nx:
        raise ValueError("flat_l2_topk: x_sqnorm must hold one norm per database row")
    if q_sqnorm is None:
        q_sqnorm = row_sqnorm(q)
    D = torch.empty((nq, k), device=q.device, dtype=torch.float32)
    I = torch.empty((nq, k), device=q.device, dtype=torch.int64)
    if nq == 0:
        return D, I
    wsb = int(lib.nsid_workspace_bytes(b"flat_l2_topk", nq, nx))
    ws = torch.empty((max(wsb, 16),), device=q.device, dtype=torch.uint8)
    _timed("flat_l2_topk", 2.0 * nq * nx * d, 4.0 * nx * d + 4.0 * nq * d + 12.0 * nq * k, lambda: call(
        "nsid_flat_l2_topk", _p(q), ldq, nq, _p(x) if nx else None, ldx, nx, _p(x_sqnorm) if nx else None, _p(q_sqnorm), d, k,
        _p(D), _p(I), _p(ws), ws.numel(), _stream()), (nq, nx, d, k))
    return D, I


def seq_scores(q, x, I, starts, lens, ldo) -> torch.Tensor:
    import numpy as np
    ldq, ldx = _search_rows(q, "seq_scores q"), _search_rows(x, "seq_scores x")
    if q.shape[1] != x.shape[1]:
        raise ValueError("seq_scores: query and database d differ")
    if I.dtype != torch.int64 or I.dim() != 2 or not I.is_contiguous() or not I.is_cuda:
        raise RuntimeError("seq_scores: I must be a contiguous (rows, k) int64 tensor on the GPU")
    k = I.shape[1]
    if not 1 <= k <= SEARCH_MAX_K:
        raise ValueError(f"seq_scores: k = {k} is outside [1, {SEARCH_MAX_K}]")
    starts = np.asarray(starts, dtype=np.int64).reshape(-1)
    lens = np.asarray(lens, dtype=np.int64).reshape(-1)
    if starts.shape != lens.shape:
        raise ValueError("seq_scores: starts and lens differ in length")
    ldo = int(ldo)
    npairs = starts.size
    if npairs and (starts.min() < 0 or lens.min() < 1 or (starts + lens).max() > min(q.shape[0], I.shape[0])):
        raise ValueError("seq_scores: every pair needs 0 <= start, 1 <= length and start + length <= the rows of q and I")
    if not 0 <= ldo <= 4 * 65535:
        raise ValueError(f"seq_scores: ldo = {ldo} is outside [0, 262140]")
    out = torch.empty((npairs, ldo), device=q.device, dtype=torch.float32)
    if npairs == 0 or ldo == 0:
        return out
    st = torch.from_numpy(starts.astype(np.int32)).to(q.device)
    ln = torch.from_numpy(lens.astype(np.int32)).to(q.device)
    nx, d = x.shape
    _tk("seq_scores_kernel", 8.0 * float(lens.sum()) * k * d, lambda: call(
        "nsid_seq_scores", _p(q), ldq, _p(x), ldx, nx, d, _p(I), k, _p(st), _p(ln), npairs, _p(out), ldo, _stream()),
        (npairs, ldo, d, 1))
    return out


CLF_C, CLF_KP, CLF_MAX_N, CLF_QCHUNK = 512, 1024, 32, 64
CLF_WIDTHS = (512, 640, 768, 1024)
CLF_PW = 512
CLF_MAX_N_EVAL = 128


def _clf_width(C, name) -> int:
    C = int(C)
    if C not in CLF_WIDTHS:
        raise ValueError(f"{name}: width C = {C} is not one of {CLF_WIDTHS}")
    return C


def clf_node_rows(x, pos=None) -> torch.Tensor:
    _chk(x, pos)
    if x.dim() != 3:
        raise ValueError(f"clf_node_rows: expected (S, C, N) node matrices, got {tuple(x.shape)}")
    S, C, N = x.shape
    if C % 32 or not 1 <= N <= CLF_MAX_N_EVAL:
        raise ValueError(f"clf_node_rows: C = {C}, N = {N} outside C % 32 == 0, 1 <= N <= {CLF_MAX_N_EVAL}")
    if N > CLF_MAX_N:
        _clf_width(C, "clf_node_rows (N > 32)")
    if pos is not None and tuple(pos.shape) != (N, C):
        raise ValueError(f"clf_node_rows: pos must be ({N}, {C}), got {tuple(pos.shape)}")
    rows = torch.empty((S * N, C), device=x.device, dtype=torch.float32)
    if N > CLF_MAX_N:
        _tk("clf_node_rows_kernel<128>", 8.0 * S * C * N,
            lambda: call("nsid_clf_node_rows_n", _p(x), S, C, N, _p(pos), _p(rows), _stream()), (S, C, N, 1))
        return rows
    _tk("clf_node_rows_kernel", 8.0 * S * C * N, lambda: call("nsid_clf_node_rows", _p(x), S, C, N, _p(pos), _p(rows), _stream()),
        (S, C, N, 1))
    return rows


def clf_pair_scores(q, kp, N, tail, q_start, q_count, cand_idx, cand_off, cand_count):
    import numpy as np
    _chk(q, kp, tail)
    N = int(N)
    if not 1 <= N <= CLF_MAX_N_EVAL:
        raise ValueError(f"clf_pair_scores: N = {N} is outside [1, {CLF_MAX_N_EVAL}]")
    if q.dim() != 2 or kp.dim() != 2:
        raise ValueError(f"clf_pair_scores: expected q (S N, C) and kp (S N, C + {CLF_PW}), got {tuple(q.shape)}, {tuple(kp.shape)}")
    C = _clf_width(q.shape[1], "clf_pair_scores")
    if q.shape[0] % N or kp.shape[1] != C + CLF_PW or kp.shape[0] % N:
        raise ValueError(f"clf_pair_scores: expected q (S N, {C}) and kp (S N, {C + CLF_PW}), got {tuple(q.shape)}, {tuple(kp.shape)}")
    if tail.numel() != 257:
        raise ValueError("clf_pair_scores: tail must hold g (128), w2 (128) and b2")
    nq_seg, nc_seg = q.shape[0] // N, kp.shape[0] // N
# ... 235 lines not shown
```

neuralsampleid_amd/optim.py:

```python
from typing import Iterable, List

import torch

from . import ops


class FusedClipAdam:
    def __init__(self, params: Iterable[torch.nn.Parameter], lr: float = 8e-5, betas=(0.9, 0.999), eps: float = 1e-8,
                 max_norm: float = 1.0, direct_grads: bool = True):
        self.params: List[torch.nn.Parameter] = [p for p in params if p.requires_grad]
        if not self.params:
            raise ValueError("no trainable parameters")
        dev = self.params[0].device
        if dev.type != "cuda":
            raise RuntimeError("FusedClipAdam needs parameters on the MI355X (cuda) device")
        self.offsets, total = [], 0
        for p in self.params:
            self.offsets.append(total)
            total += (p.numel() + 7) // 8 * 8
        self.numel = total
        self.flat_p = torch.zeros(total, device=dev)
        self.flat_g = torch.zeros(total, device=dev)
        self.exp_avg = torch.zeros(total, device=dev)
        self.exp_avg_sq = torch.zeros(total, device=dev)
        for p, off in zip(self.params, self.offsets):
            view = self.flat_p[off:off + p.numel()].view_as(p)
            view.copy_(p.data)
            p.data = view
            p.grad = self.flat_g[off:off + p.numel()].view_as(p)
        self.flat_p16 = torch.zeros(total, device=dev, dtype=torch.bfloat16)
        ops.SHADOWS.purge()
        for p, off in zip(self.params, self.offsets):
            if p.numel() % 8 == 0:
                ops.SHADOWS.register(p.data, self.flat_p16[off:off + p.numel()], owner=self.flat_p)
        for p in self.params:
            if p.dim() == 4 and tuple(p.shape[2:]) == (3, 3):
                ops.DS_PREP.register(p)
        self.hyper = torch.tensor([lr, betas[0], betas[1], eps, max_norm if max_norm else 0.0], device=dev)
        self.step_count = torch.zeros((), dtype=torch.int64, device=dev)
        self.grad_norm = torch.zeros(1, device=dev)
        if direct_grads:
            from . import functional
            functional.DIRECT_GRADS = True

    def zero_grad(self, set_to_none: bool = False):
        from . import functional
        functional.DEFERRED.reset()
        functional.join_side_streams()
        ops.fill_zero(self.flat_g)
        if functional.ACT_DTYPE == torch.bfloat16:
            self.sync_shadow()
            ops.DS_PREP.refresh()

    def sync_shadow(self):
        n8 = self.numel
        ops.f32_to_bf16(self.flat_p[:n8], self.flat_p16)
        for p in self.params:
            ops.SHADOWS.mark_fresh(p)

    def set_lr(self, lr: float):
        self.hyper[0:1].fill_(lr)

    @property
    def lr(self) -> float:
        return float(self.hyper[0])

    def step(self):
        from . import functional
        functional.join_side_streams()
        partial = ops.sumsq_partial(self.flat_g)
        ops.bump_state_epoch(stats=False)
        ops.adam_step(self.flat_p, self.flat_g, self.exp_avg, self.exp_avg_sq, self.hyper, self.step_count, partial,
                      self.grad_norm)
```

Baseline: 35330 clips/s.

## Fuse step prologue kernels and fold Adam/NT-Xent tails via atomic tickets

Merges grad zero-fill, the fp32-to-bf16 shadow copy and the depthwise weight prepack into one multi-role launch at zero_grad. The Adam step-counter increment moves into the last finishing block through an atomic ticket, which removes the separate tick kernel. The NT-Xent forward and backward use a ticket-based fused path. A wider BN running-stat update packs up to 64 layers per launch using variance offsets. The aim is fewer graph nodes and fewer launch gaps per step, at the cost of grid-wide atomic counters that must reset correctly on every replay.

```diff
diff --git a/include/nsid.h b/include/nsid.h
--- a/include/nsid.h
+++ b/include/nsid.h
@@ -170,13 +170,19 @@
 size_t nsid_ntxent_ws_floats(int Bg);
 int nsid_ntxent_fwd_bwd(const float* z_i, const float* z_j, int Bg, int d, float tau, int p0, int np, float* ws,
                         float* loss_out, float* dz_i, float* dz_j, void* stream);
+int nsid_ntxent_fwd_bwd_fused(const float* z_i, const float* z_j, int Bg, int d, float tau, int p0, int np, float* ws,
+                              void* ticket, float* loss_out, float* dz_i, float* dz_j, void* stream);
 
 int nsid_sumsq_blocks(long n);
 int nsid_sumsq_partial(const float* g, long n, float* partial, void* stream);
 int nsid_adam_step(float* p, const float* g, float* m, float* v, long n, const float* hyper, int64_t* step,
                    const float* partial, int nblocks, float* gnorm_out, void* stream);
+int nsid_adam_step_ticket(float* p, const float* g, float* m, float* v, long n, const float* hyper, int64_t* step,
+                          const float* partial, int nblocks, float* gnorm_out, void* ticket, void* stream);
 
 int nsid_fill_zero(void* p, size_t bytes, void* stream);
+int nsid_step_prologue(float* grad, const float* p, void* p16, long n, int nds, const float* const* w, void* const* wp16,
+                       void* const* wb16, float* const* dwp, const int* Cout, const int* Cin, void* stream);
 int nsid_scale_f32(const float* x, const float* scale, long n, float* out, void* stream);
 
 int nsid_bcn_to_rows(const float* x, int B, int C, int N, void* rows, int ld, int rows_dtype, void* stream);
diff --git a/neuralsampleid_amd/_lib.py b/neuralsampleid_amd/_lib.py
--- a/neuralsampleid_amd/_lib.py
+++ b/neuralsampleid_amd/_lib.py
@@ -48,8 +48,10 @@
     "nsid_l2norm_fwd": "piifpps",
     "nsid_l2norm_bwd": "pppiifps",
     "nsid_ntxent_fwd_bwd": "ppiifiipppps",
+    "nsid_ntxent_fwd_bwd_fused": "ppiifiippppps",
     "nsid_sumsq_partial": "plps",
     "nsid_adam_step": "pppplpppips",
+    "nsid_adam_step_ticket": "pppplpppipps",
     "nsid_f32_to_bf16": "ppls",
     "nsid_reflect_pad": "plips",
     "nsid_power_mel_db": "plippiips",
@@ -60,6 +62,7 @@
     "nsid_batched_index_select_fwd": "ppiiiiips",
     "nsid_batched_index_select_bwd": "ppiiiiips",
     "nsid_fill_zero": "pzs",
+    "nsid_step_prologue": "ppplipppppps",
     "nsid_scale_f32": "pplps",
     "nsid_row_sqnorm": "piiips",
     "nsid_flat_l2_topk": "piipiippiipppzs",
diff --git a/neuralsampleid_amd/csrc/bn.hip b/neuralsampleid_amd/csrc/bn.hip
--- a/neuralsampleid_amd/csrc/bn.hip
+++ b/neuralsampleid_amd/csrc/bn.hip
@@ -348,21 +348,45 @@
   int C[RU_LAYERS];
   float momentum;
 };
+__device__ __forceinline__ void running_update_layer(float* rm_p, float* rv_p, int64_t* nbt, const float* mean_a, const float* uvar_a,
+                                                     const float* mean_b, const float* uvar_b, int C, float m) {
+  const bool two = mean_b != nullptr;
+  if (threadIdx.x == 0 && nbt != nullptr) *nbt += two ? 2 : 1;
+  for (int c = threadIdx.x; c < C; c += blockDim.x) {
+    float rm = running_blend(rm_p[c], mean_a[c], m);
+    float rv = running_blend(rv_p[c], uvar_a[c], m);
+    if (two) {
+      rm = running_blend(rm, mean_b[c], m);
+      rv = running_blend(rv, uvar_b[c], m);
+    }
+    rm_p[c] = rm;
+    rv_p[c] = rv;
+  }
+}
 __global__ __launch_bounds__(256) void bn_running_update_kernel(const RunUpdArgs a) {
   const int l = blockIdx.x;
-  const float m = a.momentum;
-  const bool two = a.mean_b[l] != nullptr;
-  if (threadIdx.x == 0 && a.nbt[l] != nullptr) *a.nbt[l] += two ? 2 : 1;
-  for (int c = threadIdx.x; c < a.C[l]; c += blockDim.x) {
-    float rm = running_blend(a.rm[l][c], a.mean_a[l][c], m);
-    float rv = running_blend(a.rv[l][c], a.uvar_a[l][c], m);
-    if (two) {
-      rm = running_blend(rm, a.mean_b[l][c], m);
-      rv = running_blend(rv, a.uvar_b[l][c], m);
-    }
-    a.rm[l][c] = rm;
-    a.rv[l][c] = rv;
-  }
+  running_update_layer(a.rm[l], a.rv[l], a.nbt[l], a.mean_a[l], a.uvar_a[l], a.mean_b[l], a.uvar_b[l], a.C[l], a.momentum);
+}
+constexpr int RUW_LAYERS = 64;
+struct RunUpdWideArgs {
+  float* rm[RUW_LAYERS]; float* rv[RUW_LAYERS]; int64_t* nbt[RUW_LAYERS];
+  const float* mean_a[RUW_LAYERS]; const float* mean_b[RUW_LAYERS];
+  int uvar_a_off[RUW_LAYERS], uvar_b_off[RUW_LAYERS];
+  int C[RUW_LAYERS];
+  float momentum;
+};
+static_assert(sizeof(RunUpdWideArgs) + 256 <= 4096, "kernel arguments (explicit + hidden) must fit the 4 KB segment");
+__global__ __launch_bounds__(256) void bn_running_update_wide_kernel(const RunUpdWideArgs a) {
+  const int l = blockIdx.x;
+  const float* mb = a.mean_b[l];
+  running_update_layer(a.rm[l], a.rv[l], a.nbt[l], a.mean_a[l], a.mean_a[l] + a.uvar_a_off[l], mb,
+                       mb != nullptr ? mb + a.uvar_b_off[l] : nullptr, a.C[l], a.momentum);
+}
+inline bool float_offset(const float* p, const float* q, int* off) {
+  const ptrdiff_t d = reinterpret_cast<const char*>(q) - reinterpret_cast<const char*>(p);
+  if (d % (ptrdiff_t)sizeof(float) != 0 || d / 4 > INT32_MAX || d / 4 < INT32_MIN) return false;
+  *off = (int)(d / 4);
+  return true;
 }
 }
 
@@ -371,20 +395,47 @@
                                       const float* const* uvar_a, const float* const* mean_b,
                                       const float* const* uvar_b, float momentum, void* stream) {
   NSID_REQUIRE(n > 0 && C && running_mean && running_var && mean_a && uvar_a);
+  for (int i = 0; i < n; ++i) {
+    NSID_REQUIRE(C[i] > 0 && running_mean[i] && running_var[i] && mean_a[i] && uvar_a[i]);
+    NSID_REQUIRE(((mean_b ? mean_b[i] : nullptr) == nullptr) == ((uvar_b ? uvar_b[i] : nullptr) == nullptr));
+  }
+  bool wide = nsid_tune(NSID_T_bn_run_wide) != 0;
+  for (int i = 0, off; wide && i < n; ++i)
+    wide = float_offset(mean_a[i], uvar_a[i], &off) && (!(mean_b && mean_b[i]) || float_offset(mean_b[i], uvar_b[i], &off));
+  if (wide) {
+    for (int base = 0; base < n; base += RUW_LAYERS) {
+      RunUpdWideArgs a{};
+      const int cnt = n - base < RUW_LAYERS ? n - base : RUW_LAYERS;
+      for (int i = 0; i < cnt; ++i) {
+        const int k = base + i;
+        a.rm[i] = running_mean[k]; a.rv[i] = running_var[k];
+        a.nbt[i] = num_batches_tracked ? num_batches_tracked[k] : nullptr;
+        a.mean_a[i] = mean_a[k]; a.mean_b[i] = mean_b ? mean_b[k] : nullptr;
+        float_offset(mean_a[k], uvar_a[k], &a.uvar_a_off[i]);
+        if (a.mean_b[i] != nullptr) float_offset(mean_b[k], uvar_b[k], &a.uvar_b_off[i]);
+        a.C[i] = C[k];
+      }
+      a.momentum = momentum;
+      NSID_LAUNCH(bn_running_update_wide_kernel, dim3(cnt), dim3(256), 0, static_cast<hipStream_t>(stream), a);
+      nsid_count(NSID_C_bn_running_update);
+      const int rc = nsid_launch_status();
+      if (rc != NSID_OK) return rc;
+    }
+    return NSID_OK;
+  }
   for (int base = 0; base < n; base += RU_LAYERS) {
     RunUpdArgs a{};
     const int cnt = n - base < RU_LAYERS ? n - base : RU_LAYERS;
     for (int i = 0; i < cnt; ++i) {
-      NSID_REQUIRE(C[base + i] > 0 && running_mean[base + i] && running_var[base + i] && mean_a[base + i] && uvar_a[base + i]);
       a.rm[i] = running_mean[base + i]; a.rv[i] = running_var[base + i];
       a.nbt[i] = num_batches_tracked ? num_batches_tracked[base + i] : nullptr;
       a.mean_a[i] = mean_a[base + i]; a.uvar_a[i] = uvar_a[base + i];
       a.mean_b[i] = mean_b ? mean_b[base + i] : nullptr; a.uvar_b[i] = uvar_b ? uvar_b[base + i] : nullptr;
-      NSID_REQUIRE((a.mean_b[i] == nullptr) == (a.uvar_b[i] == nullptr));
       a.C[i] = C[base + i];
     }
     a.momentum = momentum;
     NSID_LAUNCH(bn_running_update_kernel, dim3(cnt), dim3(256), 0, static_cast<hipStream_t>(stream), a);
+    nsid_count(NSID_C_bn_running_update);
     const int rc = nsid_launch_status();
     if (rc != NSID_OK) return rc;
   }
diff --git a/neuralsampleid_amd/csrc/misc.hip b/neuralsampleid_amd/csrc/misc.hip
--- a/neuralsampleid_amd/csrc/misc.hip
+++ b/neuralsampleid_amd/csrc/misc.hip
@@ -88,12 +88,11 @@
   const float* w[DSP_LAYERS]; __bf16* wp16[DSP_LAYERS]; __bf16* wb16[DSP_LAYERS]; float* dwp[DSP_LAYERS];
   int Cout[DSP_LAYERS], Cin[DSP_LAYERS];
 };
-__global__ __launch_bounds__(256) void ds_prepack_kernel(const DsPrepArgs a) {
-  const int l = blockIdx.y;
+__device__ __forceinline__ void ds_prepack_layer(const DsPrepArgs& a, int l, int bx, int nbx) {
   const float* w = a.w[l];
   const int Cout = a.Cout[l], Cin = a.Cin[l];
   const long total = (long)Cout * 3 * Cin;
-  for (long q = (long)blockIdx.x * blockDim.x + threadIdx.x; q < total; q += (long)gridDim.x * blockDim.x) {
+  for (long q = (long)bx * blockDim.x + threadIdx.x; q < total; q += (long)nbx * blockDim.x) {
     const int c = (int)(q % Cin), t = (int)((q / Cin) % 3);
     const long o = q / (3L * Cin);
     a.wp16[l][q] = (__bf16)w[((o * Cin + c) * 3 + t) * 3 + 1];
@@ -108,6 +107,7 @@
     }
   }
 }
+__global__ __launch_bounds__(256) void ds_prepack_kernel(const DsPrepArgs a) { ds_prepack_layer(a, blockIdx.y, blockIdx.x, gridDim.x); }
 
 __device__ __forceinline__ float add_unfused(float acc, float a, float b) {
 #pragma clang fp contract(off)
@@ -502,9 +502,18 @@
 
 __global__ __launch_bounds__(256) void adam_kernel(float* __restrict__ p, const float* __restrict__ g,
                                                    float* __restrict__ m, float* __restrict__ v, long n,
-                                                   const float* __restrict__ hyper, const int64_t* __restrict__ step,
+                                                   const float* __restrict__ hyper, int64_t* step,
                                                    const float* __restrict__ partial, int nblocks,
-                                                   float* __restrict__ gnorm_out) {
+                                                   float* __restrict__ gnorm_out, unsigned* ticket) {
+  auto done = [&](bool finite) {
+    if (ticket == nullptr) return;
+    __syncthreads();
+    if (threadIdx.x == 0 &&
+        __hip_atomic_fetch_add(ticket, 1u, __ATOMIC_RELAXED, __HIP_MEMORY_SCOPE_AGENT) == gridDim.x - 1) {
+      __hip_atomic_store(ticket, 0u, __ATOMIC_RELAXED, __HIP_MEMORY_SCOPE_AGENT);
+      if (finite) *step += 1;
+    }
+  };
   __shared__ float coef_s;
   __shared__ int skip_s;
   __shared__ double red[4];
@@ -525,7 +534,7 @@
     }
     __syncthreads();
   }
-  if (skip_s) return;
+  if (skip_s) { done(false); return; }
   const float coef = coef_s;
   const float lr = hyper[0], b1 = hyper[1], b2 = hyper[2], eps = hyper[3];
   const double t = (double)(*step + 1);
@@ -558,6 +567,7 @@
   }
   for (long i = 4 * n4 + (long)blockIdx.x * blockDim.x + threadIdx.x; i < n; i += (long)gridDim.x * blockDim.x)
     upd(g[i], m[i], v[i], p[i]);
+  done(true);
 }
 __global__ void adam_tick_kernel(int64_t* step, const float* gnorm) {
   if (gnorm == nullptr || isfinite(gnorm[0])) *step += 1;
@@ -637,6 +647,7 @@
     most = std::max(most, (long)Cout[i] * 3 * Cin[i]);
   }
   NSID_LAUNCH(ds_prepack_kernel, dim3(grid_for(most, 256), n), dim3(256), 0, static_cast<hipStream_t>(stream), a);
+  nsid_count(NSID_C_ds_prepack);
   return nsid_launch_status();
 }
 extern "C" int nsid_peak_patchify_fwd(const float* spec, const float* w, const float* bias, int B, int H, int W, int pb,
@@ -759,8 +770,17 @@
   NSID_REQUIRE(p && g && m && v && hyper && step && partial && n > 0 && nblocks > 0);
   hipStream_t s = static_cast<hipStream_t>(stream);
   NSID_LAUNCH(adam_kernel, dim3(grid_for(n, 4096)), dim3(256), 0, s, p, g, m, v, n, hyper, step, partial,
-                     nblocks, gnorm_out);
+                     nblocks, gnorm_out, static_cast<unsigned*>(nullptr));
   NSID_LAUNCH(adam_tick_kernel, dim3(1), dim3(1), 0, s, step, (const float*)gnorm_out);
+  nsid_count(NSID_C_adam_tick);
+  return nsid_launch_status();
+}
+extern "C" int nsid_adam_step_ticket(float* p, const float* g, float* m, float* v, long n, const float* hyper, int64_t* step,
+                                     const float* partial, int nblocks, float* gnorm_out, void* ticket, void* stream) {
+  NSID_REQUIRE(p && g && m && v && hyper && step && partial && ticket && n > 0 && nblocks > 0);
+  NSID_REQUIRE((reinterpret_cast<uintptr_t>(ticket) & 3u) == 0);
+  NSID_LAUNCH(adam_kernel, dim3(grid_for(n, 4096)), dim3(256), 0, static_cast<hipStream_t>(stream), p, g, m, v, n, hyper, step,
+              partial, nblocks, gnorm_out, static_cast<unsigned*>(ticket));
   return nsid_launch_status();
 }
 
@@ -824,18 +844,22 @@
   return nsid_launch_status();
 }
 
-__global__ __launch_bounds__(256) void f32_to_bf16_kernel(const float* __restrict__ src, __bf16* __restrict__ dst, long n8) {
-  for (long i = (long)blockIdx.x * blockDim.x + threadIdx.x; i < n8; i += (long)gridDim.x * blockDim.x) {
+__device__ __forceinline__ void f32_to_bf16_blocks(const float* __restrict__ src, __bf16* __restrict__ dst, long n8, int bx, int nbx) {
+  for (long i = (long)bx * blockDim.x + threadIdx.x; i < n8; i += (long)nbx * blockDim.x) {
     float v[8];
     Chunk<float>::load(src + 8 * i, v);
     Chunk<float>::load(src + 8 * i + 4, v + 4);
     Chunk<__bf16>::store(dst + 8 * i, v);
   }
 }
+__global__ __launch_bounds__(256) void f32_to_bf16_kernel(const float* __restrict__ src, __bf16* __restrict__ dst, long n8) {
+  f32_to_bf16_blocks(src, dst, n8, blockIdx.x, gridDim.x);
+}
 extern "C" int nsid_f32_to_bf16(const float* src, void* dst, long n, void* stream) {
   NSID_REQUIRE(src && dst && n > 0 && n % 8 == 0 && nsid_aligned16(src) && nsid_aligned16(dst));
   NSID_LAUNCH(f32_to_bf16_kernel, dim3(grid_for(n / 8, 4096)), dim3(256), 0, static_cast<hipStream_t>(stream), src,
               static_cast<__bf16*>(dst), n / 8);
+  nsid_count(NSID_C_f32_to_bf16);
   return nsid_launch_status();
 }
 
@@ -858,9 +882,22 @@
   return nsid_launch_status();
 }
 
+__device__ __forceinline__ void fill_zero_blocks(f32x4* __restrict__ p, long n16, int bx, int nbx) {
+  const f32x4 z = {0.f, 0.f, 0.f, 0.f};
+  for (long i = (long)bx * blockDim.x + threadIdx.x; i < n16; i += (long)nbx * blockDim.x) p[i] = z;
+}
 __global__ __launch_bounds__(256) void fill_zero_kernel(f32x4* __restrict__ p, long n16) {
-  const f32x4 z = {0.f, 0.f, 0.f, 0.f};
-  for (long i = (long)blockIdx.x * blockDim.x + threadIdx.x; i < n16; i += (long)gridDim.x * blockDim.x) p[i] = z;
+  fill_zero_blocks(p, n16, blockIdx.x, gridDim.x);
+}
+__global__ __launch_bounds__(256) void step_prologue_kernel(f32x4* __restrict__ grad, long n16, const float* __restrict__ p,
+                                                            __bf16* __restrict__ p16, long n8, int bz, int bc, int bd,
+                                                            const DsPrepArgs a) {
+  int b = blockIdx.x;
+  if (b < bz) { fill_zero_blocks(grad, n16, b, bz); return; }
+  b -= bz;
+  if (b < bc) { f32_to_bf16_blocks(p, p16, n8, b, bc); return; }
+  b -= bc;
+  ds_prepack_layer(a, b / bd, b % bd, bd);
 }
 __global__ void fill_zero_tail_kernel(unsigned char* __restrict__ p, long n) {
   for (long i = (long)blockIdx.x * blockDim.x + threadIdx.x; i < n; i += (long)gridDim.x * blockDim.x) p[i] = 0;
@@ -876,6 +913,7 @@
   hipStream_t s = static_cast<hipStream_t>(stream);
   if (n16 > 0) {
     NSID_LAUNCH(fill_zero_kernel, dim3(grid_for(n16, 2048)), dim3(256), 0, s, static_cast<f32x4*>(p), n16);
+    nsid_count(NSID_C_fill_zero);
     if (nsid_launch_status() != NSID_OK) return NSID_ELAUNCH;
   }
   if (bytes % 16) {
@@ -885,6 +923,24 @@
   }
   return NSID_OK;
 }
+extern "C" int nsid_step_prologue(float* grad, const float* p, void* p16, long n, int nds, const float* const* w, void* const* wp16,
+                                  void* const* wb16, float* const* dwp, const int* Cout, const int* Cin, void* stream) {
+  NSID_REQUIRE(grad && p && p16 && n > 0 && n % 8 == 0 && nsid_aligned16(grad) && nsid_aligned16(p) && nsid_aligned16(p16));
+  NSID_REQUIRE(nds >= 0 && nds <= DSP_LAYERS && (nds == 0 || (w && wp16 && wb16 && Cout && Cin)));
+  DsPrepArgs a{};
+  long most = 0;
+  for (int i = 0; i < nds; ++i) {
+    NSID_REQUIRE(w[i] && wp16[i] && wb16[i] && Cout[i] > 0 && Cin[i] > 0);
+    a.w[i] = w[i]; a.wp16[i] = static_cast<__bf16*>(wp16[i]); a.wb16[i] = static_cast<__bf16*>(wb16[i]);
+    a.dwp[i] = dwp ? dwp[i] : nullptr; a.Cout[i] = Cout[i]; a.Cin[i] = Cin[i];
+    most = std::max(most, (long)Cout[i] * 3 * Cin[i]);
+  }
+  const int bz = grid_for(n / 4, 2048), bc = grid_for(n / 8, 4096), bd = nds > 0 ? grid_for(most, 256) : 1;
+  NSID_LAUNCH(step_prologue_kernel, dim3(bz + bc + bd * nds), dim3(256), 0, static_cast<hipStream_t>(stream),
+              reinterpret_cast<f32x4*>(grad), n / 4, p, static_cast<__bf16*>(p16), n / 8, bz, bc, bd, a);
+  nsid_count(NSID_C_step_prologue);
+  return nsid_launch_status();
+}
 extern "C" int nsid_scale_f32(const float* x, const float* scale, long n, float* out, void* stream) {
   NSID_REQUIRE(x && out && n > 0);
   NSID_LAUNCH(scale_f32_kernel, dim3(grid_for(n, 1024)), dim3(256), 0, static_cast<hipStream_t>(stream), x, scale, n, out);
diff --git a/neuralsampleid_amd/csrc/nsid_common.h b/neuralsampleid_amd/csrc/nsid_common.h
--- a/neuralsampleid_amd/csrc/nsid_common.h
+++ b/neuralsampleid_amd/csrc/nsid_common.h
@@ -173,6 +173,7 @@
   X(wgg_w3, 1)                  \
   X(wgrad256, 1)                \
   X(wgg_rows256, 4096)          \
+  X(bn_run_wide, 1)             \
   X(ws_gemm, 7)
 
 enum NsidTuneKey {
@@ -207,7 +208,11 @@
   X(clf_node_rows_n) X(clf_pair_scores_n)        \
   X(clf_mine) X(clf_attn_fwd) X(clf_head_fwd) X(clf_head_bwd) X(clf_attn_bwd) X(clf_seg_reduce)    \
   X(logmel_fft)            \
-  X(conv2d_3x3) X(conv2d_1x1) X(ibn_relu) X(stem7_pool) X(gem_pool)
+  X(conv2d_3x3) X(conv2d_1x1) X(ibn_relu) X(stem7_pool) X(gem_pool)    \
+  X(step_prologue) X(fill_zero) X(f32_to_bf16) X(ds_prepack)           \
+  X(bn_running_update)     \
+  X(ntxent_lse) X(ntxent_merge) X(ntxent_loss) X(ntxent_memset) X(ntxent_grad)    \
+  X(adam_tick)
 
 enum NsidCounterKey {
 #define NSID_CNT_ENUM(name) NSID_C_##name,
diff --git a/neuralsampleid_amd/csrc/ntxent.hip b/neuralsampleid_amd/csrc/ntxent.hip
--- a/neuralsampleid_amd/csrc/ntxent.hip
+++ b/neuralsampleid_amd/csrc/ntxent.hip
@@ -76,12 +76,47 @@
 }
 
 
+__device__ __forceinline__ void merge_row(const float* part, int groups, int M, int i, float* lse, float* rowloss) {
+  float m = -__builtin_inff(), sacc = 0.f, p = 0.f;
+  for (int g = 0; g < groups; ++g) {
+    const float m2 = part[(long)g * 3 * M + i], s2 = part[(long)g * 3 * M + M + i];
+    const float mn = fmaxf(m, m2);
+    const float e1 = m == -__builtin_inff() ? 0.f : expf(m - mn);
+    const float e2 = m2 == -__builtin_inff() ? 0.f : expf(m2 - mn);
+    sacc = sacc * e1 + s2 * e2;
+    m = mn;
+    p += part[(long)g * 3 * M + 2 * M + i];
+  }
+  const float l = m + logf(sacc);
+  lse[i] = l;
+  rowloss[i] = l - p;
+}
+__device__ __forceinline__ void loss_sum(const float* rowloss, int row0, int nrows, int M, double* red, float* loss_out) {
+  double s = 0.0;
+  for (int i = threadIdx.x; i < nrows; i += blockDim.x) s += (double)rowloss[row0 + i];
+  s = wave_sum_d(s);
+  if ((threadIdx.x & 63) == 0) red[threadIdx.x >> 6] = s;
+  __syncthreads();
+  if (threadIdx.x == 0) loss_out[0] = (float)((red[0] + red[1] + red[2] + red[3]) / (double)M);
+}
+
+struct LseFinish {
+  unsigned* ticket;
+  float* loss_out;
+  int row0, nrows;
+  f32x4* dz_i; f32x4* dz_j; long dz16;
+};
+
 __global__ __launch_bounds__(256) void ntxent_lse_kernel(const float* __restrict__ z_i, const float* __restrict__ z_j,
                                                          int M, int d, float tau, int cols_per_group,
-                                                         float* __restrict__ lse, float* __restrict__ rowloss,
-                                                         float* __restrict__ part_out) {
+                                                         float* lse, float* rowloss, float* part_out, const LseFinish fin) {
   extern __shared__ __attribute__((aligned(16))) float sm[];
   const int ld = d + 4;
+  if (fin.ticket != nullptr && fin.dz16 > 0) {
+    const f32x4 z = {0.f, 0.f, 0.f, 0.f};
+    const long wg = (long)blockIdx.y * gridDim.x + blockIdx.x, nwg = (long)gridDim.x * gridDim.y;
+    for (long q = wg * blockDim.x + threadIdx.x; q < fin.dz16; q += nwg * blockDim.x) { fin.dz_i[q] = z; fin.dz_j[q] = z; }
+  }
   float* zi_s = sm;
   float* zj_s = sm + RB * ld;
   float* part = zj_s + CBK * ld;
@@ -162,25 +197,36 @@
       rowloss[i0 + threadIdx.x] = l - p;
     }
   }
+  if (fin.ticket == nullptr) return;
+  int* last_s = reinterpret_cast<int*>(part);
+  asm volatile("s_waitcnt vmcnt(0)" ::: "memory");
+  __syncthreads();
+  if (threadIdx.x == 0) {
+    __builtin_amdgcn_fence(__ATOMIC_RELEASE, "agent");
+    asm volatile("s_waitcnt vmcnt(0)" ::: "memory");
+    const unsigned total = gridDim.x * gridDim.y;
+    const bool last = __hip_atomic_fetch_add(fin.ticket, 1u, __ATOMIC_RELAXED, __HIP_MEMORY_SCOPE_AGENT) == total - 1;
+    if (last) {
+      __builtin_amdgcn_fence(__ATOMIC_ACQUIRE, "agent");
+      asm volatile("s_waitcnt vmcnt(0)" ::: "memory");
+      __hip_atomic_store(fin.ticket, 0u, __ATOMIC_RELAXED, __HIP_MEMORY_SCOPE_AGENT);
+    }
+    *last_s = last;
+  }
+  __syncthreads();
+  if (!*last_s) return;
+  if (gridDim.y > 1) {
+    for (int r = threadIdx.x; r < M; r += blockDim.x) merge_row(part_out, gridDim.y, M, r, lse, rowloss);
+    __syncthreads();
+  }
+  loss_sum(rowloss, fin.row0, fin.nrows, M, reinterpret_cast<double*>(sm), fin.loss_out);
 }
 
 __global__ void ntxent_lse_merge_kernel(const float* __restrict__ part, int groups, int M, float* __restrict__ lse,
                                         float* __restrict__ rowloss) {
   const int i = blockIdx.x * blockDim.x + threadIdx.x;
   if (i >= M) return;
-  float m = -__builtin_inff(), sacc = 0.f, p = 0.f;
-  for (int g = 0; g < groups; ++g) {
-    const float m2 = part[(long)g * 3 * M + i], s2 = part[(long)g * 3 * M + M + i];
-    const float mn = fmaxf(m, m2);
-    const float e1 = m == -__builtin_inff() ? 0.f : expf(m - mn);
-    const float e2 = m2 == -__builtin_inff() ? 0.f : expf(m2 - mn);
-    sacc = sacc * e1 + s2 * e2;
-    m = mn;
-    p += part[(long)g * 3 * M + 2 * M + i];
-  }
-  const float l = m + logf(sacc);
-  lse[i] = l;
-  rowloss[i] = l - p;
+  merge_row(part, groups, M, i, lse, rowloss);
 }
 
 template <int DT>
@@ -271,12 +317,7 @@
 __global__ __launch_bounds__(256) void ntxent_loss_kernel(const float* __restrict__ rowloss, int row0, int nrows, int M,
                                                           float* __restrict__ loss_out) {
   __shared__ double red[4];
-  double s = 0.0;
-  for (int i = threadIdx.x; i < nrows; i += blockDim.x) s += (double)rowloss[row0 + i];
-  s = wave_sum_d(s);
-  if ((threadIdx.x & 63) == 0) red[threadIdx.x >> 6] = s;
-  __syncthreads();
-  if (threadIdx.x == 0) loss_out[0] = (float)((red[0] + red[1] + red[2] + red[3]) / (double)M);
+  loss_sum(rowloss, row0, nrows, M, red, loss_out);
 }
 
 template <typename K>
@@ -291,19 +332,32 @@
 constexpr int LSE_MAX_GROUPS = 16;
 extern "C" size_t nsid_ntxent_ws_floats(int Bg) { return (size_t)4 * Bg + 8 + (size_t)LSE_MAX_GROUPS * 3 * 2 * Bg; }
 
-extern "C" int nsid_ntxent_fwd_bwd(const float* z_i, const float* z_j, int Bg, int d, float tau, int p0, int np,
-                                   float* ws, float* loss_out, float* dz_i, float* dz_j, void* stream) {
+namespace {
+int ntxent_launch(const float* z_i, const float* z_j, int Bg, int d, float tau, int p0, int np, float* ws, unsigned* ticket,
+                  float* loss_out, float* dz_i, float* dz_j, hipStream_t s) {
   NSID_REQUIRE(z_i && z_j && ws && loss_out && Bg > 0 && np > 0 && p0 >= 0 && p0 + np <= Bg && tau > 0.f);
   NSID_REQUIRE(d % 16 == 0 && d <= 256 && nsid_aligned16(z_i) && nsid_aligned16(z_j));
   NSID_REQUIRE((dz_i == nullptr) == (dz_j == nullptr));
   const int M = 2 * Bg;
   float* lse = ws;
   float* rowloss = ws + M;
-  hipStream_t s = static_cast<hipStream_t>(stream);
   const size_t bytes = ((size_t)(RB + CBK) * (d + 4) + 4 * 3 * 16) * sizeof(float);
   if (raise_lds(ntxent_lse_kernel, bytes) != NSID_OK) return NSID_ELAUNCH;
+  const int row0 = 2 * p0, nrows = 2 * np, nblocks = (M + CBK - 1) / CBK;
+  const int grow_tiles = (nrows + RB - 1) / RB;
+  int gcg = grow_tiles >= 128 ? 1 : (256 + grow_tiles - 1) / grow_tiles;
+  if (gcg > nblocks) gcg = nblocks;
+  const int gcols = (nblocks + gcg - 1) / gcg * CBK;
+  gcg = (M + gcols - 1) / gcols;
+  LseFinish fin{};
+  if (ticket != nullptr) {
+    NSID_REQUIRE(dz_i != nullptr && nsid_aligned16(dz_i) && nsid_aligned16(dz_j) && (reinterpret_cast<uintptr_t>(ticket) & 3u) == 0);
+    fin.ticket = ticket; fin.loss_out = loss_out; fin.row0 = row0; fin.nrows = nrows;
+    fin.dz_i = reinterpret_cast<f32x4*>(dz_i); fin.dz_j = reinterpret_cast<f32x4*>(dz_j);
+    fin.dz16 = gcg > 1 ? (long)np * d / 4 : 0;
+  }
   {
-    const int row_tiles = (M + RB - 1) / RB, nblocks = (M + CBK - 1) / CBK;
+    const int row_tiles = (M + RB - 1) / RB;
     int cg = row_tiles >= 512 ? 1 : (512 + row_tiles - 1) / row_tiles;
     if (cg > nblocks) cg = nblocks;
     if (cg > LSE_MAX_GROUPS) cg = LSE_MAX_GROUPS;
@@ -311,34 +365,50 @@
     cg = (M + cols_per_group - 1) / cols_per_group;
     float* part = ws + 2 * M + 8;
     NSID_LAUNCH(ntxent_lse_kernel, dim3(row_tiles, cg), dim3(256), bytes, s, z_i, z_j, M, d, tau, cols_per_group, lse,
-                rowloss, part);
-    if (cg > 1) NSID_LAUNCH(ntxent_lse_merge_kernel, dim3((M + 255) / 256), dim3(256), 0, s, part, cg, M, lse, rowloss);
-  }
-  NSID_LAUNCH(ntxent_loss_kernel, dim3(1), dim3(256), 0, s, rowloss, 2 * p0, 2 * np, M, loss_out);
+                rowloss, part, fin);
+    nsid_count(NSID_C_ntxent_lse);
+    if (cg > 1 && ticket == nullptr) {
+      NSID_LAUNCH(ntxent_lse_merge_kernel, dim3((M + 255) / 256), dim3(256), 0, s, part, cg, M, lse, rowloss);
+      nsid_count(NSID_C_ntxent_merge);
+    }
+  }
+  if (ticket == nullptr) {
+    NSID_LAUNCH(ntxent_loss_kernel, dim3(1), dim3(256), 0, s, rowloss, 2 * p0, 2 * np, M, loss_out);
+    nsid_count(NSID_C_ntxent_loss);
+  }
   if (dz_i != nullptr) {
-    const int row0 = 2 * p0, nrows = 2 * np;
-    const int row_tiles = (nrows + RB - 1) / RB, nblocks = (M + CBK - 1) / CBK;
-    int cg = row_tiles >= 128 ? 1 : (256 + row_tiles - 1) / row_tiles;
-    if (cg > nblocks) cg = nblocks;
-    const int cols_per_group = (nblocks + cg - 1) / cg * CBK;
-    cg = (M + cols_per_group - 1) / cols_per_group;
-    if (cg > 1) {
+    if (gcg > 1 && ticket == nullptr) {
       if (hipMemsetAsync(dz_i, 0, (size_t)np * d * sizeof(float), s) != hipSuccess ||
           hipMemsetAsync(dz_j, 0, (size_t)np * d * sizeof(float), s) != hipSuccess)
         return NSID_ELAUNCH;
-    }
-    dim3 grid(row_tiles, cg);
+      nsid_count(NSID_C_ntxent_memset);
+      nsid_count(NSID_C_ntxent_memset);
+    }
+    dim3 grid(grow_tiles, gcg);
 #define NSID_NTX_CASE(DTV)                                                                                   \
   case DTV:                                                                                                  \
     if (raise_lds(ntxent_grad_kernel<DTV>, bytes) != NSID_OK) return NSID_ELAUNCH;                           \
     NSID_LAUNCH((ntxent_grad_kernel<DTV>), grid, dim3(256), bytes, s, z_i, z_j, M, d, tau, lse, row0, \
-                       nrows, cols_per_group, dz_i, dz_j);                                                                   \
+                       nrows, gcols, dz_i, dz_j);                                                                   \
     break;
     switch (d / 16) {
       NSID_NTX_CASE(1) NSID_NTX_CASE(2) NSID_NTX_CASE(4) NSID_NTX_CASE(8) NSID_NTX_CASE(16)
       default: return NSID_EINVAL;
     }
 #undef NSID_NTX_CASE
+    nsid_count(NSID_C_ntxent_grad);
   }
   return nsid_launch_status();
 }
+}
+
+extern "C" int nsid_ntxent_fwd_bwd(const float* z_i, const float* z_j, int Bg, int d, float tau, int p0, int np,
+                                   float* ws, float* loss_out, float* dz_i, float* dz_j, void* stream) {
+  return ntxent_launch(z_i, z_j, Bg, d, tau, p0, np, ws, nullptr, loss_out, dz_i, dz_j, static_cast<hipStream_t>(stream));
+}
+extern "C" int nsid_ntxent_fwd_bwd_fused(const float* z_i, const float* z_j, int Bg, int d, float tau, int p0, int np,
+                                         float* ws, void* ticket, float* loss_out, float* dz_i, float* dz_j, void* stream) {
+  NSID_REQUIRE(ticket && dz_i && dz_j);
+  return ntxent_launch(z_i, z_j, Bg, d, tau, p0, np, ws, static_cast<unsigned*>(ticket), loss_out, dz_i, dz_j,
+                       static_cast<hipStream_t>(stream));
+}
diff --git a/neuralsampleid_amd/ops.py b/neuralsampleid_amd/ops.py
--- a/neuralsampleid_amd/ops.py
+++ b/neuralsampleid_amd/ops.py
@@ -207,6 +207,9 @@
 def f32_to_bf16(src: torch.Tensor, dst: Optional[torch.Tensor] = None) -> torch.Tensor:
     _chk(src)
     n = src.numel()
+    if _PROLOGUE_FILL is not None:
+        _prologue_launch(_PROLOGUE_FILL, src, dst)
+        return dst
     if dst is None:
         dst = torch.empty(((n + 7) // 8 * 8,), device=src.device, dtype=torch.bfloat16)
     if n % 8:
@@ -808,16 +811,25 @@
                 out.append((ctypes.c_void_p * n)(*[e[name].data_ptr() for e in es]))
         return out
 
+    def live(self):
+        self.purge()
+        return [e for e in self.entries.values() if e["wref"]().is_cuda] if DS_PREP_ENABLED else []
+
+    @staticmethod
+    def _bytes(es) -> float:
+        return sum(4.0 * e["wref"]().numel() / 3 + 2.0 * 5 * e["Cout"] * e["Cin"] + 12.0 * e["Cout"] * e["Cin"] for e in es)
+
+    def mark_refreshed(self, es) -> None:
+        for e in es:
+            e["key"], e["slots"] = (e["wref"]()._version, WEIGHT_EPOCH), 0
+
     def refresh(self) -> None:
-        self.purge()
-        es = [e for e in self.entries.values() if e["wref"]().is_cuda] if DS_PREP_ENABLED else []
+        es = self.live()
         if not es:
             return
         w, wp16, wb16, dwp, Cout, Cin = self._arrays(es, "w", "wp16", "wb16", "dwp", "Cout", "Cin")
-        _tk("ds_prepack_kernel", sum(4.0 * e["wref"]().numel() / 3 + 2.0 * 5 * e["Cout"] * e["Cin"] + 12.0 * e["Cout"] * e["Cin"] for e in es),
-            lambda: call("nsid_ds_prepack", len(es), w, wp16, wb16, dwp, Cout, Cin, _stream()))
-        for e in es:
-            e["key"], e["slots"] = (e["wref"]()._version, WEIGHT_EPOCH), 0
+        _tk("ds_prepack_kernel", self._bytes(es), lambda: call("nsid_ds_prepack", len(es), w, wp16, wb16, dwp, Cout, Cin, _stream()))
+        self.mark_refreshed(es)
 
     def take_slot(self, e):
         if e["slots"] >= e["dwp"].shape[0]:
@@ -1021,6 +1033,18 @@
     return dp
 
 
+NTXENT_FUSED = 1
+_NTX_TICKET = {}
+
+
+def ntxent_ticket(device) -> torch.Tensor:
+    dev = torch.device(device)
+    idx = dev.index if dev.index is not None else torch.cuda.current_device()
+    if idx not in _NTX_TICKET:
+        _NTX_TICKET[idx] = torch.zeros(1, device=dev, dtype=torch.int32)
+    return _NTX_TICKET[idx]
+
+
 def ntxent_fwd_bwd(z_i, z_j, tau, p0=0, npairs=None, want_grad=True):
     _chk(z_i, z_j)
     Bg, d = z_i.shape
@@ -1029,9 +1053,15 @@
     loss = torch.empty((1,), device=z_i.device, dtype=torch.float32)
     dzi = torch.empty((npairs, d), device=z_i.device, dtype=torch.float32) if want_grad else None
     dzj = torch.empty((npairs, d), device=z_i.device, dtype=torch.float32) if want_grad else None
-    _timed("ntxent_kernels", 2.0 * (2 * Bg) * (2 * npairs) * d * (2 if want_grad else 1), 4.0 * d * (2 * Bg + 2 * npairs), lambda: call(
-        "nsid_ntxent_fwd_bwd", _p(z_i), _p(z_j), Bg, d, float(tau), p0, npairs, _p(ws), _p(loss), _p(dzi), _p(dzj),
-        _stream()), (2 * npairs, 2 * Bg, d, 1))
+    if want_grad and NTXENT_FUSED:
+        ticket = ntxent_ticket(z_i.device)
+        launch = lambda: call("nsid_ntxent_fwd_bwd_fused", _p(z_i), _p(z_j), Bg, d, float(tau), p0, npairs, _p(ws), _p(ticket),
+                              _p(loss), _p(dzi), _p(dzj), _stream())
+    else:
+        launch = lambda: call("nsid_ntxent_fwd_bwd", _p(z_i), _p(z_j), Bg, d, float(tau), p0, npairs, _p(ws), _p(loss), _p(dzi),
+                              _p(dzj), _stream())
+    _timed("ntxent_kernels", 2.0 * (2 * Bg) * (2 * npairs) * d * (2 if want_grad else 1), 4.0 * d * (2 * Bg + 2 * npairs), launch,
+           (2 * npairs, 2 * Bg, d, 1))
     return loss, dzi, dzj
 
 
@@ -1045,6 +1075,32 @@
 
 def zeros(shape, device, dtype=torch.float32) -> torch.Tensor:
     return fill_zero(torch.empty(shape, device=device, dtype=dtype))
+
+
+STEP_PROLOGUE = 1
+_PROLOGUE_FILL = None
+
+
+def step_prologue(flat_g: torch.Tensor, flat_p: torch.Tensor, flat_p16: torch.Tensor) -> None:
+    global _PROLOGUE_FILL
+    _chk(flat_g, flat_p)
+    n = flat_p.numel()
+    if flat_g.numel() != n or flat_p16.numel() != n or n % 8 or flat_p16.dtype != torch.bfloat16 or not flat_p16.is_contiguous():
+        raise RuntimeError("step_prologue takes the three flat buffers of one optimiser")
+    _PROLOGUE_FILL = flat_g
+    try:
+        f32_to_bf16(flat_p, flat_p16)
+    finally:
+        _PROLOGUE_FILL = None
+
+
+def _prologue_launch(flat_g, flat_p, flat_p16) -> None:
+    n = flat_p.numel()
+    es = DS_PREP.live()
+    arrays = DS_PREP._arrays(es, "w", "wp16", "wb16", "dwp", "Cout", "Cin") if es else [None] * 6
+    _tk("step_prologue_kernel", 10.0 * n + DsPrep._bytes(es), lambda: call(
+        "nsid_step_prologue", _p(flat_g), _p(flat_p), _p(flat_p16), n, len(es), *arrays, _stream()), (n, 1, 0, 1))
+    DS_PREP.mark_refreshed(es)
 
 
 def scale_f32(x: torch.Tensor, scale: Optional[torch.Tensor] = None, out: Optional[torch.Tensor] = None) -> torch.Tensor:
@@ -1098,8 +1154,16 @@
     return partial
 
 
-def adam_step(p, g, m, v, hyper, step, partial, gnorm_out) -> None:
+ADAM_TICKET = 1
+
+
+def adam_step(p, g, m, v, hyper, step, partial, gnorm_out, ticket=None) -> None:
     _chk(p, g, m, v, hyper, partial, gnorm_out)
+    if ticket is not None and ADAM_TICKET:
+        _tk("adam_kernel", 28.0 * p.numel(), lambda: call(
+            "nsid_adam_step_ticket", _p(p), _p(g), _p(m), _p(v), p.numel(), _p(hyper), _p(step), _p(partial), partial.numel(),
+            _p(gnorm_out), _p(ticket), _stream()), (p.numel(), 1, 0, 1))
+        return
     _tk("adam_kernel", 28.0 * p.numel(), lambda: call(
         "nsid_adam_step", _p(p), _p(g), _p(m), _p(v), p.numel(), _p(hyper), _p(step), _p(partial), partial.numel(),
         _p(gnorm_out), _stream()), (p.numel(), 1, 0, 1))
diff --git a/neuralsampleid_amd/optim.py b/neuralsampleid_amd/optim.py
--- a/neuralsampleid_amd/optim.py
+++ b/neuralsampleid_amd/optim.py
@@ -39,6 +39,8 @@
         self.hyper = torch.tensor([lr, betas[0], betas[1], eps, max_norm if max_norm else 0.0], device=dev)
         self.step_count = torch.zeros((), dtype=torch.int64, device=dev)
         self.grad_norm = torch.zeros(1, device=dev)
+        self.ticket = torch.zeros(1, dtype=torch.int32, device=dev)
+        ops.ntxent_ticket(dev)
         if direct_grads:
             from . import functional
             functional.DIRECT_GRADS = True
@@ -47,6 +49,10 @@
         from . import functional
         functional.DEFERRED.reset()
         functional.join_side_streams()
+        if functional.ACT_DTYPE == torch.bfloat16 and ops.STEP_PROLOGUE:
+            ops.step_prologue(self.flat_g, self.flat_p, self.flat_p16)
+            self._shadows_fresh()
+            return
         ops.fill_zero(self.flat_g)
         if functional.ACT_DTYPE == torch.bfloat16:
             self.sync_shadow()
@@ -55,6 +61,9 @@
     def sync_shadow(self):
         n8 = self.numel
         ops.f32_to_bf16(self.flat_p[:n8], self.flat_p16)
+        self._shadows_fresh()
+
+    def _shadows_fresh(self):
         for p in self.params:
             ops.SHADOWS.mark_fresh(p)
 
@@ -71,4 +80,4 @@
         partial = ops.sumsq_partial(self.flat_g)
         ops.bump_state_epoch(stats=False)
         ops.adam_step(self.flat_p, self.flat_g, self.exp_avg, self.exp_avg_sq, self.hyper, self.step_count, partial,
-                      self.grad_norm)
+                      self.grad_norm, ticket=self.ticket)
```

After: 35440 clips/s (median of 6 runs). About the same (+0.3%).
